# jaggedsoft/mythril

Measured on AMD Instinct MI355X. Metric: constraint-node evals/sec, higher is better.
Workload: dtype u32x8 (256-bit bit-vectors)

## Files before the change

### include/mythcc.h

```cpp
#ifndef MYTHCC_H
#define MYTHCC_H

#include <stdint.h>

#ifdef __cplusplus
extern "C" {
#endif

#define MGC_OK 0
#define MGC_UNSUPPORTED 1
#define MGC_ERROR 2

#define MGC_MAX_SOURCE_WIDTH 65536

#define MGC_SORT_BV 0
#define MGC_SORT_BOOL 1
#define MGC_SORT_ARRAY 2

#define MGC_REMAT_SPILL 0
#define MGC_REMAT_SCRATCH 1
#define MGC_REMAT_ALWAYS 2

typedef struct mgc_input {
    int32_t n_nodes;
    const int32_t* op;
    const int32_t* sort;
    const int32_t* width;
    const int32_t* dom;
    const int64_t* id;
    const int32_t* arg_off;
    const int32_t* args;
    const int64_t* p0;
    const int64_t* p1;
    const int32_t* str;
    const int32_t* cval_off;
    const uint32_t* cval;
    const char* strings;
    int32_t n_strings;
    int32_t n_cons;
    const int32_t* cons;
    int32_t n_probes;
    const int32_t* probes;
    int32_t n_tables;
    const int32_t* table_name;
    const int32_t* table_size;
    int32_t default_entries;
    int32_t nreg;
    int32_t n_extra;
    const uint32_t* extra;
    int32_t leaf_pools;
    int32_t const_keys;
    int32_t solve;
    int32_t remat_mode;
    int32_t remat_k;
    int32_t keep_clean;
    int32_t search_hints;
    int32_t abi_presets;
    int32_t n_cval;
    int32_t n_string_bytes;
} mgc_input;

typedef struct mgc_result mgc_result;

const char* mgc_source_ops(void);

int mgc_compile(const mgc_input* in, mgc_result** out);

const char* mgc_error(const mgc_result* r);
const uint32_t* mgc_code(const mgc_result* r, int32_t* n_ins);
const uint32_t* mgc_table(const mgc_result* r, int32_t* n_rows, int32_t* n_const_values);
const char* mgc_meta(const mgc_result* r);
void mgc_free(mgc_result* r);

#ifdef __cplusplus
}
#endif

#endif
```

### mythril_amd/ccompile.py

```python

from __future__ import annotations

import collections.abc as _abc
import ctypes
import json
import os
import threading
from array import array
from typing import Dict, List, Optional, Sequence

import numpy as np

from . import irdefs as I
from .smt.node import ARRAY, BOOL, topo_order

_lib = None
_lock = threading.Lock()
_OPS: Dict[str, int] = {}
_OTHER = 0

MGC_OK, MGC_UNSUPPORTED = 0, 1
_SORT = {"bv": 0, BOOL: 1, ARRAY: 2}
_REMAT = {"spill": 0, "always": 2}


class _Input(ctypes.Structure):
    _fields_ = [("n_nodes", ctypes.c_int32)] + \
        [(n, ctypes.c_void_p) for n in ("op", "sort", "width", "dom", "id", "arg_off", "args", "p0",
                                         "p1", "str", "cval_off", "cval")] + \
        [("strings", ctypes.c_char_p), ("n_strings", ctypes.c_int32),
         ("n_cons", ctypes.c_int32), ("cons", ctypes.c_void_p),
         ("n_probes", ctypes.c_int32), ("probes", ctypes.c_void_p),
         ("n_tables", ctypes.c_int32), ("table_name", ctypes.c_void_p),
         ("table_size", ctypes.c_void_p),
         ("default_entries", ctypes.c_int32), ("nreg", ctypes.c_int32),
         ("n_extra", ctypes.c_int32), ("extra", ctypes.c_void_p),
         ("leaf_pools", ctypes.c_int32), ("const_keys", ctypes.c_int32), ("solve", ctypes.c_int32),
         ("remat_mode", ctypes.c_int32), ("remat_k", ctypes.c_int32),
         ("keep_clean", ctypes.c_int32), ("search_hints", ctypes.c_int32),
         ("abi_presets", ctypes.c_int32), ("n_cval", ctypes.c_int32),
         ("n_string_bytes", ctypes.c_int32)]


def load():
    global _lib, _OTHER
    if _lib is not None:
        return _lib
    with _lock:
        if _lib is not None:
            return _lib
        from .build import build_compiler
        path = build_compiler()
        lib = ctypes.CDLL(path)
        lib.mgc_source_ops.restype = ctypes.c_char_p
        lib.mgc_compile.argtypes = [ctypes.POINTER(_Input), ctypes.POINTER(ctypes.c_void_p)]
        lib.mgc_compile.restype = ctypes.c_int
        lib.mgc_error.argtypes = [ctypes.c_void_p]
        lib.mgc_error.restype = ctypes.c_char_p
        lib.mgc_code.argtypes = [ctypes.c_void_p, ctypes.POINTER(ctypes.c_int32)]
        lib.mgc_code.restype = ctypes.c_void_p
        lib.mgc_table.argtypes = [ctypes.c_void_p, ctypes.POINTER(ctypes.c_int32),
                                  ctypes.POINTER(ctypes.c_int32)]
        lib.mgc_table.restype = ctypes.c_void_p
        lib.mgc_meta.argtypes = [ctypes.c_void_p]
        lib.mgc_meta.restype = ctypes.c_char_p
        lib.mgc_free.argtypes = [ctypes.c_void_p]
        names = lib.mgc_source_ops().decode().split("\n")
        _OPS.update({n: i for i, n in enumerate(names)})
        _OTHER = _OPS["?"]
        _lib = lib
    return _lib


def _ptr(a):
    return ctypes.addressof(ctypes.c_char.from_buffer(a)) if len(a) else None


_ext = None


def _load_ext():
    global _ext
    if _ext is None:
        import importlib.util
        from .build import cc_ext_path
        load()
        spec = importlib.util.spec_from_file_location("_mythcc", cc_ext_path())
        mod = importlib.util.module_from_spec(spec)
        spec.loader.exec_module(mod)
        _ext = mod
    return _ext


def compile_native(constraints: Sequence, probes: Sequence = (),
                   table_sizes: Optional[Dict[str, int]] = None, default_entries: int = 2,
                   nreg: int = I.NREG, extra_consts: Sequence[int] = (), leaf_pools: bool = False,
                   const_keys: bool = False, solve: bool = False, leaf_remat: Optional[str] = None,
                   keep_clean: Optional[bool] = None, search_hints: bool = False,
                   abi_presets: bool = False):
    from . import ir
    ext = _load_ext()
    M = (1 << 256) - 1
    extra = b"".join((v & M).to_bytes(32, "little") for v in extra_consts)
    remat = leaf_remat or ir.LEAF_REMAT
    mode = _REMAT.get(remat, 1)
    k = int(remat[7:]) if mode == 1 and remat[7:].isdigit() else 0
    rc, err, code_b, raw, ncv, meta = ext.compile(
        list(constraints), list(probes), _OPS, list((table_sizes or {}).items()), default_entries,
        nreg, extra, int(leaf_pools), int(const_keys), int(solve), mode, k,
        int(ir.KEEP_CLEAN if keep_clean is None else keep_clean), int(search_hints),
        int(abi_presets))
    if rc != MGC_OK:
        if rc == MGC_UNSUPPORTED:
            raise ir.Unsupported(err)
        raise RuntimeError("native compiler: " + err)
    prog = _program(np.frombuffer(code_b, dtype=np.uint32).reshape(-1, 4).copy(), raw, ncv,
                    json.loads(meta))
    prog.nreg = nreg
    return prog


def buckets(constraints: Sequence):
    return _load_ext().buckets(list(constraints))


def flatten(constraints: Sequence, probes: Sequence = (),
            table_sizes: Optional[Dict[str, int]] = None, extra_consts: Sequence[int] = ()):
    load()
    constraints, probes = list(constraints), list(probes)
    nodes = topo_order(constraints + probes)
    index = {n.id: i for i, n in enumerate(nodes)}
    ops, OTHER = _OPS, _OTHER
    f = {k: array("i") for k in ("op", "sort", "width", "dom", "str", "cval_off", "args")}
    f.update({k: array("q") for k in ("id", "p0", "p1")})
    f["arg_off"] = array("i", [0])
    cval = bytearray()
    strings: List[str] = []
    sidx: Dict[str, int] = {}

    def intern(s: str) -> int:
        k = sidx.get(s)
        if k is None:
            k = sidx[s] = len(strings)
            strings.append(s)
        return k
    for n in nodes:
        op = n.op
        code = ops.get(op, OTHER)
        f["op"].append(code)
        f["sort"].append(_SORT[n.sort])
        f["width"].append(n.width)
        f["dom"].append(n.dom or 0)
        f["id"].append(n.id)
        for a in n.args:
            f["args"].append(index[a.id])
        f["arg_off"].append(len(f["args"]))
        p0 = p1 = 0
        s = -1
        c = -1
        pr = n.params
        if op == "bvnum":
            c = len(cval) // 4
            cval += pr[0].to_bytes(4 * ((n.width + 31) // 32), "little")
        elif op in ("var", "array"):
            s = intern(pr[0])
        elif op == "apply":
            s = intern(pr[0])
            p0 = pr[1]
        elif op == "extract":
            p0, p1 = pr
        elif op in ("zero_extend", "sign_extend"):
            p0 = pr[0]
        elif code == OTHER:
            s = intern(op)
        f["p0"].append(p0)
        f["p1"].append(p1)
        f["str"].append(s)
        f["cval_off"].append(c)
    f["cons"] = array("i", [index[c.id] for c in constraints])
    f["probes"] = array("i", [index[p.id] for p in probes])
    tsz = table_sizes or {}
    f["table_name"] = array("i", [intern(k) for k in tsz])
    f["table_size"] = array("i", list(tsz.values()))
    M = (1 << 256) - 1
    f["extra"] = bytearray(b"".join((v & M).to_bytes(32, "little") for v in extra_consts))
    f["cval"] = bytearray(cval)
    f["strings"] = b"".join(s.encode() + b"\0" for s in strings)
    f["n_nodes"], f["n_strings"] = len(nodes), len(strings)
    return f


def compile_native_ctypes(constraints: Sequence, probes: Sequence = (),
                          table_sizes: Optional[Dict[str, int]] = None, default_entries: int = 2,
                          nreg: int = I.NREG, extra_consts: Sequence[int] = (),
                          leaf_pools: bool = False, const_keys: bool = False, solve: bool = False,
                          leaf_remat: Optional[str] = None, keep_clean: Optional[bool] = None,
                          search_hints: bool = False, abi_presets: bool = False):
    from . import ir
    lib = load()
    f = flatten(constraints, probes, table_sizes, extra_consts)
    remat = leaf_remat or ir.LEAF_REMAT
    mode = _REMAT.get(remat, 1)
    k = int(remat[7:]) if mode == 1 and remat[7:].isdigit() else 0
    P = {n: _ptr(f[n]) for n in ("op", "sort", "width", "dom", "id", "arg_off", "args", "p0", "p1",
                                  "str", "cval_off", "cval", "cons", "probes", "table_name",
                                  "table_size", "extra")}
    inp = _Input(f["n_nodes"], P["op"], P["sort"], P["width"], P["dom"], P["id"], P["arg_off"],
                 P["args"], P["p0"], P["p1"], P["str"], P["cval_off"], P["cval"], f["strings"],
                 f["n_strings"], len(f["cons"]), P["cons"], len(f["probes"]), P["probes"],
                 len(f["table_name"]), P["table_name"], P["table_size"], default_entries, nreg,
                 len(f["extra"]) // 32, P["extra"], int(leaf_pools), int(const_keys), int(solve),
                 mode, k, int(ir.KEEP_CLEAN if keep_clean is None else keep_clean),
                 int(search_hints), int(abi_presets), len(f["cval"]) // 4, len(f["strings"]))
    res = ctypes.c_void_p()
    rc = lib.mgc_compile(ctypes.byref(inp), ctypes.byref(res))
    try:
        if rc != MGC_OK:
            msg = lib.mgc_error(res).decode()
            if rc == MGC_UNSUPPORTED:
                raise ir.Unsupported(msg)
            raise RuntimeError("native compiler: " + msg)
        n = ctypes.c_int32()
        p = lib.mgc_code(res, ctypes.byref(n))
        code = np.frombuffer(ctypes.string_at(p, 16 * n.value), dtype=np.uint32).reshape(-1, 4).copy()
        rows, ncv = ctypes.c_int32(), ctypes.c_int32()
        p = lib.mgc_table(res, ctypes.byref(rows), ctypes.byref(ncv))
        raw = ctypes.string_at(p, 32 * rows.value) if rows.value else b""
        meta = json.loads(lib.mgc_meta(res))
    finally:
        lib.mgc_free(res)
    prog = _program(code, raw, ncv.value, meta)
    prog.nreg = nreg
    return prog


class LeafRecords(_abc.Sequence):

    __slots__ = ("_rs", "_items", "widths")

    def __init__(self, rs: str, widths: Sequence[int]):
        self._rs = rs
        self._items = None
        self.widths = list(widths)

    def _decode(self):
        from .ir import Leaf
        items = []
        if self.widths:
            for line in self._rs.split("\n"):
                name, w, kind, source, chunk, entry = line.split("\t")
                items.append(Leaf(name, int(w), kind, source, int(chunk), int(entry)))
        self._items = items
        self._rs = None
        return items

    def __len__(self):
        return len(self.widths)

    def __getitem__(self, i):
        return (self._items if self._items is not None else self._decode())[i]

    def __iter__(self):
        return iter(self._items if self._items is not None else self._decode())

    def __eq__(self, other):
        return list(self) == list(other)

    def __repr__(self):
        return repr(list(self))

    def __reduce__(self):
        return (list, (list(self),))


def _program(code, raw: bytes, ncv: int, meta):
    from . import ir
    consts = np.frombuffer(raw, dtype="<u4").reshape(-1, 8).astype(np.uint32)
    const_values = [int.from_bytes(raw[32 * i:32 * i + 32], "little") for i in range(ncv)]
    Leaf = ir.Leaf
    if meta.get("leaves_rs") is not None:
        leaves = LeafRecords(meta["leaves_rs"], meta["leaf_widths"])
    else:
        leaves = [Leaf(*row) for row in meta["leaves"]]
    hist_counts = dict(meta["hist"])
    stats = {"lnodes": meta["lnodes"], "n_ins": int(code.shape[0]), "spills": meta["spills"],
             "reloads": meta["reloads"],
             "hist": {I.OPNAME[op]: hist_counts[op] for op in meta["hist_order"]}}
    prog = ir.Program(code, consts, const_values, leaves, meta["n_lds"], meta["n_probes"],
                      meta["n_roots"], dict(meta["table_sizes"]), dict(meta["table_kinds"]),
                      {k: [int(h, 16) for h in v] for k, v in meta["table_ckeys"]}, stats,
                      [tuple(r) for r in meta["pool_ranges"]], dict(meta["derived"]),
                      {k: v for k, v in meta["entry_keys"]}, meta["n_user_probes"])
    prog.compile_us = meta.get("t_us")
    pre = meta.get("presets")
    if pre is not None:
        from .abi import Plan
        prog.presets = Plan(vars={k: int(v, 16) for k, v in pre["vars"]},
                            arrays={k: dict(cells) for k, cells in pre["arrays"]})
    return prog
```

### mythril_amd/csrc/mg_compile.cpp

```cpp

#include "mythcc.h"
#include "mythgpu_ir.h"

#include <algorithm>
#include <memory>
#include <cstdint>
#include <cstdio>
#include <cstring>
#include <chrono>
#include <stdexcept>
#include <string>
#include <unordered_map>
#include <unordered_set>
#include <tuple>
#include <utility>
#include <vector>

namespace {

struct U {
    static const int N = 6;
    uint64_t w[N];
    U() { std::memset(w, 0, sizeof w); }
    static U of(uint64_t x) { U r; r.w[0] = x; return r; }
    bool zero() const {
        for (int i = 0; i < N; i++) if (w[i]) return false;
        return true;
    }
    bool neg() const { return w[N - 1] >> 63; }
    int bitlen() const {
        for (int i = N - 1; i >= 0; i--)
            if (w[i]) return 64 * i + 64 - __builtin_clzll(w[i]);
        return 0;
    }
    int popcount() const {
        int c = 0;
        for (int i = 0; i < N; i++) c += __builtin_popcountll(w[i]);
        return c;
    }
    bool bit(int k) const { return k < 64 * N && ((w[k >> 6] >> (k & 63)) & 1); }
};

static U operator+(const U& a, const U& b) {
    U r; unsigned __int128 c = 0;
    for (int i = 0; i < U::N; i++) { c += (unsigned __int128)a.w[i] + b.w[i]; r.w[i] = (uint64_t)c; c >>= 64; }
    return r;
}
static U operator~(const U& a) { U r; for (int i = 0; i < U::N; i++) r.w[i] = ~a.w[i]; return r; }
static U operator-(const U& a, const U& b) { return a + ~b + U::of(1); }
static U operator&(const U& a, const U& b) { U r; for (int i = 0; i < U::N; i++) r.w[i] = a.w[i] & b.w[i]; return r; }
static U operator|(const U& a, const U& b) { U r; for (int i = 0; i < U::N; i++) r.w[i] = a.w[i] | b.w[i]; return r; }
static U operator^(const U& a, const U& b) { U r; for (int i = 0; i < U::N; i++) r.w[i] = a.w[i] ^ b.w[i]; return r; }
static U operator*(const U& a, const U& b) {
    U r;
    for (int i = 0; i < U::N; i++) {
        unsigned __int128 c = 0;
        for (int j = 0; i + j < U::N; j++) {
            c += (unsigned __int128)a.w[i] * b.w[j] + r.w[i + j];
            r.w[i + j] = (uint64_t)c; c >>= 64;
        }
    }
    return r;
}
struct BadShift : std::runtime_error { BadShift() : std::runtime_error("negative shift") {} };
static U shl(const U& a, int k) {
    if (k < 0) throw BadShift();
    U r; if (k >= 64 * U::N) return r;
    int q = k >> 6, s = k & 63;
    for (int i = U::N - 1; i >= q; i--) {
        uint64_t v = a.w[i - q] << s;
        if (s && i - q - 1 >= 0) v |= a.w[i - q - 1] >> (64 - s);
        r.w[i] = v;
    }
    return r;
}
static U shr(const U& a, int k) {
    if (k < 0) throw BadShift();
    U r; if (k >= 64 * U::N) return r;
    int q = k >> 6, s = k & 63;
    for (int i = 0; i + q < U::N; i++) {
        uint64_t v = a.w[i + q] >> s;
        if (s && i + q + 1 < U::N) v |= a.w[i + q + 1] << (64 - s);
        r.w[i] = v;
    }
    return r;
}
static U sar(const U& a, int k) {
    if (!a.neg()) return shr(a, k);
    return ~shr(~a, k);
}
static bool operator==(const U& a, const U& b) { return std::memcmp(a.w, b.w, sizeof a.w) == 0; }
static bool operator!=(const U& a, const U& b) { return !(a == b); }
static bool operator<(const U& a, const U& b) {
    for (int i = U::N - 1; i >= 0; i--) if (a.w[i] != b.w[i]) return a.w[i] < b.w[i];
    return false;
}
static bool operator>(const U& a, const U& b) { return b < a; }
static bool operator<=(const U& a, const U& b) { return !(b < a); }
static bool operator>=(const U& a, const U& b) { return !(a < b); }
static U umin(const U& a, const U& b) { return b < a ? b : a; }
static U umax(const U& a, const U& b) { return a < b ? b : a; }
static U mask_slow(int w) { return shl(U::of(1), w) - U::of(1); }
static const U* mask_table() {
    static const std::vector<U> t = [] {
        std::vector<U> v(64 * U::N + 1);
        for (int w = 0; w <= 64 * U::N; w++) v[w] = mask_slow(w);
        return v;
    }();
    return t.data();
}
static const U* const MASKS = mask_table();
static inline const U& mask(int w) { return MASKS[w < 0 ? 0 : (w > 64 * U::N ? 64 * U::N : w)]; }
static U U1(int k) { return shl(U::of(1), k); }
static bool nz(const U& a) { return !a.zero(); }

static std::string hex(const U& a) {
    char buf[8];
    std::string s;
    bool started = false;
    for (int i = U::N - 1; i >= 0; i--) {
        for (int nib = 15; nib >= 0; nib--) {
            int d = (a.w[i] >> (4 * nib)) & 15;
            if (!started && !d) continue;
            started = true;
            std::snprintf(buf, sizeof buf, "%x", d);
            s += buf;
        }
    }
    return started ? s : "0";
}

struct Big {
    std::vector<uint32_t> l;
    void norm() { while (!l.empty() && !l.back()) l.pop_back(); }
    bool operator==(const Big& o) const { return l == o.l; }
    bool operator<(const Big& o) const {
        if (l.size() != o.l.size()) return l.size() < o.l.size();
        for (size_t i = l.size(); i-- > 0;) if (l[i] != o.l[i]) return l[i] < o.l[i];
        return false;
    }
    U chunk(int k) const {
        U r;
        for (int j = 0; j < 8; j++) {
            size_t idx = (size_t)8 * k + j;
            if (idx < l.size()) r.w[j / 2] |= (uint64_t)l[idx] << (32 * (j & 1));
        }
        return r;
    }
    U low384() const {
        U r;
        for (size_t j = 0; j < l.size() && j < 12; j++) r.w[j / 2] |= (uint64_t)l[j] << (32 * (j & 1));
        return r;
    }
    std::string hexs() const {
        if (l.empty()) return "0";
        char buf[16];
        std::string s;
        std::snprintf(buf, sizeof buf, "%x", l.back());
        s += buf;
        for (size_t i = l.size() - 1; i-- > 0;) { std::snprintf(buf, sizeof buf, "%08x", l[i]); s += buf; }
        return s;
    }
};

static Big big_of(const U& u) {
    Big b;
    for (int j = 0; j < 2 * U::N; j++) b.l.push_back((uint32_t)(u.w[j / 2] >> (32 * (j & 1))));
    b.norm();
    return b;
}

struct Bits {
    std::vector<uint64_t> w;
    void set(int k) { if ((size_t)(k >> 6) >= w.size()) w.resize((k >> 6) + 1, 0); w[k >> 6] |= 1ull << (k & 63); }
    void orw(const Bits& o) { if (o.w.size() > w.size()) w.resize(o.w.size(), 0); for (size_t i = 0; i < o.w.size(); i++) w[i] |= o.w[i]; }
    bool meets(const Bits& o) const {
        size_t n = std::min(w.size(), o.w.size());
        for (size_t i = 0; i < n; i++) if (w[i] & o.w[i]) return true;
        return false;
    }
    bool any() const { for (auto x : w) if (x) return true; return false; }
    int count() const { int c = 0; for (auto x : w) c += __builtin_popcountll(x); return c; }
    template <class F> void each(F f) const {
        for (size_t i = 0; i < w.size(); i++) {
            uint64_t x = w[i];
            while (x) { int b = __builtin_ctzll(x); f((int)(64 * i + b)); x &= x - 1; }
        }
    }
    bool any_minus(const Bits& o) const {
        for (size_t i = 0; i < w.size(); i++) if (w[i] & ~(i < o.w.size() ? o.w[i] : 0)) return true;
        return false;
    }
    Bits minus(const Bits& o) const {
        Bits r; r.w = w;
        for (size_t i = 0; i < r.w.size() && i < o.w.size(); i++) r.w[i] &= ~o.w[i];
        return r;
    }
};

struct Unsupported : std::runtime_error { using std::runtime_error::runtime_error; };
struct MemoMiss {};

template <class K, class V, class H = std::hash<K>>
struct OMap {
    std::vector<std::pair<K, V>> items;
    std::unordered_map<K, size_t, H> idx;
    V* find(const K& k) { auto it = idx.find(k); return it == idx.end() ? nullptr : &items[it->second].second; }
    const V* find(const K& k) const { auto it = idx.find(k); return it == idx.end() ? nullptr : &items[it->second].second; }
    bool has(const K& k) const { return idx.count(k) != 0; }
    V& setdefault(const K& k, const V& d) {
        auto it = idx.find(k);
        if (it != idx.end()) return items[it->second].second;
        idx.emplace(k, items.size());
        items.emplace_back(k, d);
        return items.back().second;
    }
    void put(const K& k, const V& v) { setdefault(k, v) = v; }
    size_t size() const { return items.size(); }
    void truncate(size_t n) {
        while (items.size() > n) { idx.erase(items.back().first); items.pop_back(); }
    }
};

enum SOp {
    S_BVNUM, S_TRUE, S_FALSE, S_VAR, S_BVSUB, S_BVUDIV, S_BVUREM, S_BVSDIV, S_BVSREM, S_BVSMOD,
    S_BVSHL, S_BVLSHR, S_BVASHR, S_BVADD, S_BVMUL, S_BVAND, S_BVOR, S_BVXOR, S_AND, S_OR,
    S_BVNEG, S_BVNOT, S_NOT, S_XOR, S_IMPLIES, S_BVULT, S_BVULE, S_BVUGT, S_BVUGE, S_BVSLT,
    S_BVSLE, S_BVSGT, S_BVSGE, S_UMULNO, S_EQ, S_DISTINCT, S_ITE, S_CONCAT, S_EXTRACT, S_ZEXT,
    S_SEXT, S_SELECT, S_APPLY, S_STORE, S_K, S_ARRAY, S_OTHER
};
static const char* const SOP_NAMES =
    "bvnum\ntrue\nfalse\nvar\nbvsub\nbvudiv\nbvurem\nbvsdiv\nbvsrem\nbvsmod\n"
    "bvshl\nbvlshr\nbvashr\nbvadd\nbvmul\nbvand\nbvor\nbvxor\nand\nor\n"
    "bvneg\nbvnot\nnot\nxor\n=>\nbvult\nbvule\nbvugt\nbvuge\nbvslt\n"
    "bvsle\nbvsgt\nbvsge\nbvumul_noovfl\n=\ndistinct\nite\nconcat\nextract\nzero_extend\n"
    "sign_extend\nselect\napply\nstore\nK\narray\n?";

struct Src {
    int op, sort, width, dom;
    int64_t id;
    std::vector<int> args;
    int64_t p0, p1;
    std::string str;
    Big val;
    bool is_array() const { return sort == MGC_SORT_ARRAY; }
    bool is_bool() const { return sort == MGC_SORT_BOOL; }
};

static const int CHUNK = 256;
static const int MAX_SPILL = MG_MAX_LDS + MG_MAX_PSLOTS;
static const int LDS_TIER = 6;
static const int POOL_CAP = 128;
static const int ARG_ENTRIES_CAP = 64;

static std::vector<int> topo(const std::vector<Src>& S, const std::vector<int>& roots) {
    std::vector<char> seen(S.size(), 0);
    std::vector<int> out;
    std::vector<std::pair<int, bool>> stack;
    for (int r : roots) {
        if (seen[r]) continue;
        stack.assign(1, {r, false});
        while (!stack.empty()) {
            auto [n, done] = stack.back();
            stack.pop_back();
            if (done) { out.push_back(n); continue; }
            if (seen[n]) continue;
            seen[n] = 1;
            stack.push_back({n, true});
            const auto& a = S[n].args;
            for (size_t i = a.size(); i-- > 0;)
                if (!seen[a[i]]) stack.push_back({a[i], false});
        }
    }
    return out;
}

struct Args {
    int n = 0;
    int a[3] = {0, 0, 0};
    std::vector<int> more;
    Args() {}
    Args(std::initializer_list<int> il) { assign(il.begin(), il.end()); }
    Args(const std::vector<int>& v) { assign(v.data(), v.data() + v.size()); }
    template <class It> void assign(It b, It e) {
        n = (int)(e - b);
        if (n <= 3) { std::copy(b, e, a); more.clear(); }
        else more.assign(b, e);
    }
    const int* begin() const { return n <= 3 ? a : more.data(); }
    const int* end() const { return begin() + n; }
    int* begin() { return n <= 3 ? a : more.data(); }
    int* end() { return begin() + n; }
    size_t size() const { return (size_t)n; }
    bool empty() const { return n == 0; }
    int operator[](size_t i) const { return begin()[i]; }
    int& operator[](size_t i) { return begin()[i]; }
    int back() const { return begin()[n - 1]; }
    bool operator==(const Args& o) const { return n == o.n && std::equal(begin(), end(), o.begin()); }
    bool operator!=(const Args& o) const { return !(*this == o); }
};

struct LN {
    int op, width;
    Args args;
    bool has_imm;
    U imm;
    int64_t birth;
};

enum LeafKind { K_VAR, K_KEY, K_VAL, K_ELSE, K_CVAL, K_AUX };
static const char* KIND_NAMES[] = {"var", "key", "val", "else", "cval", "aux"};

struct Leaf {
    std::string name;
    int width;
    int kind;
    std::string source;
    int chunk, entry;
};

static bool is_pred(int op) {
    return op == MG_EQ || op == MG_ULT || op == MG_ULE || op == MG_SLT || op == MG_SLE || op == MG_UMULNO;
}
static bool is_cmp(int op) {
    return op == MG_EQ || op == MG_ULT || op == MG_ULE || op == MG_SLT || op == MG_SLE;
}
static bool is_order(int op) { return op == MG_ULT || op == MG_ULE || op == MG_SLT || op == MG_SLE; }

typedef std::vector<int> Chunks;


struct Lowerer {
    const std::vector<Src>& S;
    std::vector<LN> ln;
    std::vector<int> slot_id;
    std::vector<uint64_t> slot_hash;
    size_t n_slots_used = 0;
    std::vector<Leaf> leaves;
    std::unordered_map<std::string, int> leaf_ids;
    std::vector<Chunks> memo;
    std::vector<char> has_memo;
    std::unordered_map<std::string, Chunks> sel_memo;
    OMap<std::string, int> table_sizes;
    OMap<std::string, std::string> table_kinds;
    int default_entries;
    int64_t birth = 0;
    OMap<std::string, std::vector<Big>> table_ckeys;
    bool solve = false;
    std::unordered_set<std::string> solve_tables;
    OMap<std::string, std::vector<std::pair<Chunks, Chunks>>> arg_entries;

    Lowerer(const std::vector<Src>& s, int de) : S(s), default_entries(de) {
        memo.resize(S.size());
        has_memo.assign(S.size(), 0);
    }

    static uint64_t key_hash(int op, int width, const Args& args, bool has_imm, const U& imm) {
        uint64_t h = (uint64_t)op * 0x9E3779B97F4A7C15ull ^ (uint64_t)width * 0xC2B2AE3D27D4EB4Full;
        for (int a : args) h = (h ^ (uint64_t)(uint32_t)a) * 0x100000001B3ull;
        if (has_imm) for (int i = 0; i < U::N; i++) h = (h ^ imm.w[i]) * 0x100000001B3ull;
        h ^= h >> 29;
        return h | 1;
    }
    void rehash(size_t n) {
        std::vector<int> ids(n, -1);
        std::vector<uint64_t> hs(n, 0);
        for (size_t i = 0; i < slot_id.size(); i++) {
            if (slot_id[i] < 0) continue;
            size_t j = slot_hash[i] & (n - 1);
            while (ids[j] >= 0) j = (j + 1) & (n - 1);
            ids[j] = slot_id[i];
            hs[j] = slot_hash[i];
        }
        slot_id.swap(ids);
        slot_hash.swap(hs);
    }
    int mk(int op, int width, Args args, bool has_imm = false, const U& imm = U()) {
        if (op == MG_CONCAT && width == MG_MAX_WIDTH && ln[args[0]].op == MG_EXTRACT &&
            ln[args[0]].imm.zero() && ln[ln[args[0]].args[0]].width == MG_MAX_WIDTH)
            args[0] = ln[args[0]].args[0];
        const U key_imm = has_imm ? imm : U();
        if (2 * (n_slots_used + 1) > slot_id.size()) rehash(slot_id.empty() ? 4096 : 2 * slot_id.size());
        uint64_t h = key_hash(op, width, args, has_imm, key_imm);
        size_t j = h & (slot_id.size() - 1);
        while (slot_id[j] >= 0) {
            if (slot_hash[j] == h) {
                const LN& o = ln[slot_id[j]];
                if (o.op == op && o.width == width && o.has_imm == has_imm && o.args == args &&
                    (!has_imm || o.imm == key_imm))
                    return slot_id[j];
            }
            j = (j + 1) & (slot_id.size() - 1);
        }
        int64_t b = birth;
        for (int a : args) if (ln[a].birth > b) b = ln[a].birth;
        int id = (int)ln.size();
        ln.push_back(LN{op, width, std::move(args), has_imm, key_imm, b});
        slot_id[j] = id;
        slot_hash[j] = h;
        n_slots_used++;
        return id;
    }
    int mki(int op, int width, Args args, int64_t imm) { return mk(op, width, std::move(args), true, U::of((uint64_t)imm)); }
    int cnst(const U& value, int width) { return mk(MG_CONST, width, {}, true, value & mask(width)); }
    int cnst(uint64_t value, int width) { return cnst(U::of(value), width); }
    int leaf(const std::string& name, int width, int kind, const std::string& source, int chunk = 0, int entry = 0) {
        auto it = leaf_ids.find(name);
        int idx;
        if (it == leaf_ids.end()) {
            idx = (int)leaves.size();
            leaf_ids.emplace(name, idx);
            leaves.push_back(Leaf{name, width, kind, source, chunk, entry});
        } else {
            idx = it->second;
        }
        return mki(MG_LEAF, width, {}, idx);
    }

    static int nchunks(int w) { return (w + CHUNK - 1) / CHUNK; }
    static int chunk_width(int w, int i) { return std::min(CHUNK, w - CHUNK * i); }

    int bits(const Chunks& chunks, int w, int lo, int hi) {
        int ci = lo / CHUNK, cj = hi / CHUNK;
        if (ci == cj) {
            int c = chunks.at(ci);
            int cw = chunk_width(w, ci);
            int l0 = lo - CHUNK * ci, h0 = hi - CHUNK * ci;
            if (l0 == 0 && h0 == cw - 1) return c;
            return mki(MG_EXTRACT, h0 - l0 + 1, {c}, l0);
        }
        int low_w = CHUNK * (ci + 1) - lo;
        int low = bits(chunks, w, lo, CHUNK * (ci + 1) - 1);
        int high = bits(chunks, w, CHUNK * cj, hi);
        return mki(MG_CONCAT, hi - lo + 1, {high, low}, low_w);
    }

    Chunks assemble(const std::vector<std::pair<Chunks, int>>& pieces) {
        int total = 0;
        for (auto& p : pieces) total += p.second;
        struct Seg { const Chunks* ch; int w, off; };
        std::vector<Seg> segs;
        int off = 0;
        for (size_t i = pieces.size(); i-- > 0;) {
            segs.push_back({&pieces[i].first, pieces[i].second, off});
            off += pieces[i].second;
        }
        Chunks out;
        for (int k = 0; k < nchunks(total); k++) {
            int lo_k = CHUNK * k, hi_k = std::min(total, CHUNK * (k + 1)) - 1;
            int acc = -1, acc_w = 0;
            for (auto& s : segs) {
                int a = std::max(lo_k, s.off), b = std::min(hi_k, s.off + s.w - 1);
                if (a > b) continue;
                int part = bits(*s.ch, s.w, a - s.off, b - s.off);
                int pw = b - a + 1;
                if (acc < 0) { acc = part; acc_w = pw; }
                else { acc = mki(MG_CONCAT, acc_w + pw, {part, acc}, acc_w); acc_w += pw; }
            }
            out.push_back(acc);
        }
        return out;
    }

    const Chunks& M(int s) {
        if (!has_memo[s]) throw MemoMiss();
        return memo[s];
    }

    std::vector<char> pend_seen_;
    std::vector<int> pending(int n) {
        if (pend_seen_.size() < S.size()) pend_seen_.assign(S.size(), 0);
        std::vector<int> out, touched;
        std::vector<std::pair<int, bool>> stack{{n, false}};
        while (!stack.empty()) {
            auto [m, done] = stack.back();
            stack.pop_back();
            if (done) { out.push_back(m); continue; }
            if (pend_seen_[m] || has_memo[m]) continue;
            pend_seen_[m] = 1;
            touched.push_back(m);
            stack.push_back({m, true});
            const auto& a = S[m].args;
            for (size_t i = a.size(); i-- > 0;)
                if (!pend_seen_[a[i]] && !has_memo[a[i]]) stack.push_back({a[i], false});
        }
        for (int m : touched) pend_seen_[m] = 0;
        return out;
    }

    const Chunks& lower(int n) {
        if (has_memo[n]) return memo[n];
        std::vector<int> nodes = pending(n);
        std::unordered_set<int> skip;
        for (int m : nodes)
            if (S[m].op == S_EXTRACT && is_carry(m)) {
                int s = S[m].args[0];
                skip.insert(s); skip.insert(S[s].args[0]); skip.insert(S[s].args[1]);
            }
        int64_t saved = birth;
        for (int m : nodes) {
            if (has_memo[m] || S[m].is_array() || (skip.count(m) && m != n)) continue;
            birth = S[m].id;
            try {
                Chunks r = lower_one(m);
                memo[m] = std::move(r);
                has_memo[m] = 1;
            } catch (MemoMiss&) {
                throw Unsupported("operand lowered only as part of a pattern");
            }
            birth = S[m].id;
        }
        birth = saved ? std::max(saved, birth) : birth;
        if (!has_memo[n]) throw Unsupported("operand lowered only as part of a pattern");
        return memo[n];
    }

    int narrow(int s) {
        const Chunks& ch = M(s);
        if (ch.size() != 1)
            throw Unsupported(opname(s) + " on a " + std::to_string(S[s].width) + "-bit value");
        return ch[0];
    }

    std::string opname(int s) {
        static const std::vector<std::string> names = [] {
            std::vector<std::string> v;
            std::string all(SOP_NAMES);
            size_t p = 0;
            while (true) {
                size_t q = all.find('\n', p);
                v.push_back(all.substr(p, q == std::string::npos ? std::string::npos : q - p));
                if (q == std::string::npos) break;
                p = q + 1;
            }
            return v;
        }();
        return S[s].op == S_OTHER ? S[s].str : names[S[s].op];
    }

    int fold(int op, int width, const Chunks& args) {
        int acc = args[0];
        for (size_t i = 1; i < args.size(); i++) acc = mk(op, width, {acc, args[i]});
        return acc;
    }

    int by_constant(int op, int w, int n) {
        const Src& s = S[n];
        if (S[s.args[1]].op != S_BVNUM) return -1;
        const Big& cb = S[s.args[1]].val;
        int x = narrow(s.args[0]);
        bool huge = cb.l.size() > 2;
        uint64_t c = 0;
        for (size_t j = 0; j < cb.l.size() && j < 2; j++) c |= (uint64_t)cb.l[j] << (32 * j);
        if (op == S_BVUDIV || op == S_BVUREM) {
            bool pow2;
            int k = 0;
            if (huge) {
                int ones = 0, top = 0;
                for (size_t j = 0; j < cb.l.size(); j++) {
                    ones += __builtin_popcount(cb.l[j]);
                    if (cb.l[j]) top = (int)(32 * j + 31 - __builtin_clz(cb.l[j]));
                }
                pow2 = ones == 1;
                k = top;
            } else {
                pow2 = c && !(c & (c - 1));
                if (pow2) k = 63 - __builtin_clzll(c);
            }
            if (!pow2) return -1;
            if (op == S_BVUREM) return k == 0 ? cnst(0, w) : mki(MG_EXTRACT, k, {x}, 0);
            op = S_BVLSHR; c = (uint64_t)k; huge = false;
        }
        if (op != S_BVSHL && op != S_BVLSHR && op != S_BVASHR) return -1;
        if (!huge && c == 0) return x;
        bool ge = huge || c >= (uint64_t)w;
        if (op == S_BVASHR) {
            int cc = ge ? w - 1 : (int)std::min<uint64_t>(c, (uint64_t)(w - 1));
            int e = mki(MG_EXTRACT, w - cc, {x}, cc);
            return mki(MG_SEXT, w, {e}, w - cc);
        }
        if (ge) return cnst(0, w);
        int cc = (int)c;
        if (op == S_BVLSHR) return mki(MG_EXTRACT, w - cc, {x}, cc);
        int e = mki(MG_EXTRACT, w - cc, {x}, 0);
        int z = cnst(0, cc);
        return mki(MG_CONCAT, w, {e, z}, cc);
    }

    Chunks lower_one(int n) {
        const Src& s = S[n];
        int op = s.op, w = s.width;
        if (w > CHUNK) return lower_wide(n);
        auto A = [&](int i) { return narrow(s.args[i]); };
        switch (op) {
        case S_BVNUM: return {cnst(s.val.chunk(0), w)};
        case S_TRUE: return {cnst(1, 1)};
        case S_FALSE: return {cnst(0, 1)};
        case S_VAR: return {leaf(s.str, w, K_VAR, s.str)};
        default: break;
        }
        int simple = -1;
        switch (op) {
        case S_BVSUB: simple = MG_SUB; break;
        case S_BVUDIV: simple = MG_UDIV; break;
        case S_BVUREM: simple = MG_UREM; break;
        case S_BVSDIV: simple = MG_SDIV; break;
        case S_BVSREM: simple = MG_SREM; break;
        case S_BVSMOD: simple = MG_SMOD; break;
        case S_BVSHL: simple = MG_SHL; break;
        case S_BVLSHR: simple = MG_LSHR; break;
        case S_BVASHR: simple = MG_ASHR; break;
        default: break;
        }
        if (simple >= 0) {
            int red = by_constant(op, w, n);
            if (red >= 0) return {red};
            int a = A(0), b = A(1);
            return {mk(simple, w, {a, b})};
        }
        int nary = -1;
        switch (op) {
        case S_BVADD: nary = MG_ADD; break;
        case S_BVMUL: nary = MG_MUL; break;
        case S_BVAND: case S_AND: nary = MG_AND; break;
        case S_BVOR: case S_OR: nary = MG_OR; break;
        case S_BVXOR: nary = MG_XOR; break;
        default: break;
        }
        if (nary >= 0) {
            Chunks xs;
            for (size_t i = 0; i < s.args.size(); i++) xs.push_back(A((int)i));
            return {fold(nary, w, xs)};
        }
        if (op == S_BVNEG) return {mk(MG_NEG, w, {A(0)})};
        if (op == S_BVNOT || op == S_NOT) return {mk(MG_NOT, w, {A(0)})};
        if (op == S_XOR) { int a = A(0), b = A(1); return {mk(MG_XOR, 1, {a, b})}; }
        if (op == S_IMPLIES) {
            int a = A(0);
            int na = mk(MG_NOT, 1, {a});
            int b = A(1);
            return {mk(MG_OR, 1, {na, b})};
        }
        int kop = -1; bool swap = false;
        switch (op) {
        case S_BVULT: kop = MG_ULT; break;
        case S_BVULE: kop = MG_ULE; break;
        case S_BVUGT: kop = MG_ULT; swap = true; break;
        case S_BVUGE: kop = MG_ULE; swap = true; break;
        case S_BVSLT: kop = MG_SLT; break;
        case S_BVSLE: kop = MG_SLE; break;
        case S_BVSGT: kop = MG_SLT; swap = true; break;
        case S_BVSGE: kop = MG_SLE; swap = true; break;
        case S_UMULNO: kop = MG_UMULNO; break;
        default: break;
        }
        if (kop >= 0) {
            int a = A(0), b = A(1);
            if (swap) std::swap(a, b);
            return {mk(kop, S[s.args[0]].width, {a, b})};
        }
        if (op == S_EQ || op == S_DISTINCT) {
            for (int a : s.args) if (S[a].is_array()) throw Unsupported("array equality");
            return {eq_or_distinct(op, n)};
        }
        if (op == S_ITE) {
            if (s.is_array()) throw Unsupported("array-valued ite outside select");
            int c = A(0), a = A(1), b = A(2);
            return {mk(MG_ITE, w, {c, a, b})};
        }
        if (op == S_CONCAT) {
            int word = calldata_word(n);
            if (word >= 0) return {word};
            std::vector<std::pair<Chunks, int>> pieces;
            for (int a : s.args) pieces.push_back({M(a), S[a].width});
            return assemble(pieces);
        }
        if (op == S_EXTRACT) {
            int carry = carry_pattern(n);
            if (carry >= 0) return {carry};
            int src = s.args[0];
// ... 14 lines not shown

    int eq_parts(const Chunks& x, const Chunks& y, int w) {
        Chunks parts;
        for (size_t k = 0; k < x.size(); k++)
            parts.push_back(mk(MG_EQ, w > CHUNK ? chunk_width(w, (int)k) : w, {x[k], y.at(k)}));
        return fold(MG_AND, 1, parts);
    }

    int eq_or_distinct(int op, int n) {
        const Src& s = S[n];
        std::vector<const Chunks*> args;
        for (int a : s.args) args.push_back(&M(a));
        int w = S[s.args[0]].width;
        if (op == S_EQ) return eq_parts(*args[0], *args[1], w);
        Chunks terms;
        for (size_t i = 0; i < args.size(); i++)
            for (size_t j = i + 1; j < args.size(); j++) {
                int e = eq_parts(*args[i], *args[j], w);
                terms.push_back(mk(MG_NOT, 1, {e}));
            }
        return fold(MG_AND, 1, terms);
    }

    bool is_carry(int n) const {
        const Src& x = S[n];
        int64_t hi = x.p0, lo = x.p1;
        const Src& s = S[x.args[0]];
        if (hi != lo || s.op != S_BVADD || s.args.size() != 2 || hi != s.width - 1) return false;
        const Src& a = S[s.args[0]];
        const Src& b = S[s.args[1]];
        return a.op == S_ZEXT && b.op == S_ZEXT && a.p0 == 1 && b.p0 == 1 &&
               S[a.args[0]].width <= CHUNK;
    }

    int carry_pattern(int n) {
        if (!is_carry(n)) return -1;
        const Src& s = S[S[n].args[0]];
        int x = S[s.args[0]].args[0], y = S[s.args[1]].args[0];
        int lx = lower(x)[0];
        int ly = lower(y)[0];
        int sum = mk(MG_ADD, S[x].width, {lx, ly});
        return mk(MG_ULT, S[x].width, {sum, lx});
    }

    Chunks lower_wide(int n) {
        const Src& s = S[n];
        int op = s.op, w = s.width;
        if (op == S_BVNUM) {
            Chunks out;
            for (int k = 0; k < nchunks(w); k++) out.push_back(cnst(s.val.chunk(k), chunk_width(w, k)));
            return out;
        }
        if (op == S_VAR) {
            Chunks out;
            for (int k = 0; k < nchunks(w); k++)
                out.push_back(leaf(s.str + "#" + std::to_string(k), chunk_width(w, k), K_VAR, s.str, k));
            return out;
        }
        if (op == S_CONCAT) {
            std::vector<std::pair<Chunks, int>> pieces;
            for (int a : s.args) pieces.push_back({M(a), S[a].width});
            return assemble(pieces);
        }
        if (op == S_EXTRACT) {
            int src = s.args[0];
            int hi = (int)s.p0, lo = (int)s.p1;
            const Chunks& sc = M(src);
            std::vector<std::pair<Chunks, int>> pieces;
            for (int k = nchunks(w) - 1; k >= 0; k--) {
                int b = bits(sc, S[src].width, lo + CHUNK * k, std::min(hi, lo + CHUNK * k + CHUNK - 1));
                pieces.push_back({{b}, std::min(CHUNK, hi - lo + 1 - CHUNK * k)});
            }
            return assemble(pieces);
        }
        if (op == S_ZEXT) {
            int src = s.args[0];
            int pad = w - S[src].width;
            std::vector<std::pair<Chunks, int>> pieces;
            while (pad > 0) {
                int pw = std::min(CHUNK, pad);
                pieces.push_back({{cnst(0, pw)}, pw});
                pad -= pw;
            }
            pieces.push_back({M(src), S[src].width});
            return assemble(pieces);
        }
        if (op == S_ITE) {
            int c = narrow(s.args[0]);
            Chunks a = M(s.args[1]), b = M(s.args[2]);
            return ite_chunks(c, a, b);
        }
        if (op == S_SELECT) {
            Chunks idx = M(s.args[1]);
            return select(s.args[0], idx, S[s.args[1]].width, w);
        }
        if (op == S_APPLY) {
            Chunks key = M(s.args[0]);
            return table_lookup(s.str, key, (int)s.p0, w, "func");
        }
        throw Unsupported(opname(n) + " on a " + std::to_string(w) + "-bit value");
    }

    void index_parts(int x, int& base, U& c) const {
        c = U();
        while (true) {
            const Src& s = S[x];
            if (s.op == S_BVNUM) { base = -1; c = (c + s.val.chunk(0)) & mask(256); return; }
            if (s.op != S_BVADD || s.args.size() != 2) { base = x; return; }
            int a = s.args[0], b = s.args[1];
            if (S[b].op == S_BVNUM && S[a].op != S_BVNUM) { c = (c + S[b].val.chunk(0)) & mask(256); x = a; }
            else if (S[a].op == S_BVNUM && S[b].op != S_BVNUM) { c = (c + S[a].val.chunk(0)) & mask(256); x = b; }
            else { base = x; return; }
        }
    }

    int calldata_word(int n) {
        const Src& s = S[n];
        if (s.width != 256 || s.args.size() != 32) return -1;
        int size = -1, arr = -1, base = -1, off = -1;
        U c0;
        for (int i = 0; i < 32; i++) {
            const Src& x = S[s.args[i]];
            if (x.op != S_ITE || x.width != 8) return -1;
            const Src& cond = S[x.args[0]];
            const Src& sel = S[x.args[1]];
            const Src& zero = S[x.args[2]];
            if (zero.op != S_BVNUM || !zero.val.l.empty() || cond.op != S_BVSLT || sel.op != S_SELECT)
                return -1;
            int idx = sel.args[1];
            if (cond.args[0] != idx || S[idx].width != 256) return -1;
            if (i == 0) {
                size = cond.args[1];
                arr = sel.args[0];
                if (S[arr].op != S_ARRAY) return -1;
                index_parts(idx, base, c0);
                off = idx;
            } else if (cond.args[1] != size || sel.args[0] != arr) {
                return -1;
            } else {
                int b;
                U c;
                index_parts(idx, b, c);
                if (b != base || !(c == ((c0 + U::of((uint64_t)i)) & mask(256)))) return -1;
            }
        }
        const std::string& name = S[arr].str;
        const std::vector<Big>* ck = table_ckeys.find(name);
        if ((ck && !ck->empty()) || (solve && solve_tables.count(name))) return -1;
        table_kinds.put(name, "array");
        int entries = table_sizes.setdefault(name, default_entries);
        int o = narrow(off), sz = narrow(size);
        int acc = mk(MG_BCAST, 256, {cell(name, K_ELSE, 0, 8)[0]});
        for (int e = entries - 1; e >= 0; e--) {
            int key = cell(name, K_KEY, e, 256)[0];
            int delta = mk(MG_SUB, 256, {key, o});
            int val = cell(name, K_VAL, e, 8)[0];
            acc = mk(MG_CDWE, 256, {acc, delta, val});
        }
        return mk(MG_CDWX, 256, {acc, o, sz});
    }

    int chunk_eq(const Chunks& x, const Chunks& y, int w) {
        Chunks parts;
        for (size_t k = 0; k < x.size(); k++) parts.push_back(mk(MG_EQ, chunk_width(w, (int)k), {x[k], y.at(k)}));
        return fold(MG_AND, 1, parts);
    }

    Chunks ite_chunks(int c, const Chunks& a, const Chunks& b) {
        Chunks out;
        for (size_t i = 0; i < a.size() && i < b.size(); i++)
            out.push_back(mk(MG_ITE, std::max(ln[a[i]].width, ln[b[i]].width), {c, a[i], b[i]}));
        return out;
    }

    Chunks cell(const std::string& name, int kind, int e, int width) {
        std::string tag;
        switch (kind) {
        case K_KEY: tag = "k" + std::to_string(e); break;
        case K_VAL: tag = "v" + std::to_string(e); break;
        case K_ELSE: tag = "else"; break;
        default: tag = "c" + std::to_string(e); break;
        }
        Chunks out;
        for (int k = 0; k < nchunks(width); k++)
            out.push_back(leaf(name + "#" + tag + "#" + std::to_string(k), chunk_width(width, k), kind, name, k, e));
        return out;
    }

    Chunks const_key(const Big& v, int kw) {
        Chunks c;
        for (int k = 0; k < nchunks(kw); k++) c.push_back(cnst(v.chunk(k), chunk_width(kw, k)));
        return c;
    }

    Chunks table_lookup(const std::string& name, const Chunks& key, int kw, int vw, const char* kind) {
        table_kinds.put(name, kind);
        std::string mkey = "T" + name;
        mkey.push_back('\0');
        mkey.append((const char*)key.data(), 4 * key.size());
        auto hit = sel_memo.find(mkey);
        if (hit != sel_memo.end()) return hit->second;
        int entries = table_sizes.setdefault(name, default_entries);
        static const std::vector<Big> none;
        const std::vector<Big>* ckp = table_ckeys.find(name);
        const std::vector<Big>& ckeys = ckp ? *ckp : none;
        bool has_kval = true;
        for (int k : key) if (ln[k].op != MG_CONST) { has_kval = false; break; }
        Big kval;
        if (has_kval) {
            for (size_t i = 0; i < key.size(); i++) {
                Big part = big_of(ln[key[i]].imm);
                if (kval.l.size() < 8 * i + part.l.size()) kval.l.resize(8 * i + part.l.size(), 0);
                for (size_t j = 0; j < part.l.size(); j++) kval.l[8 * i + j] |= part.l[j];
            }
            kval.norm();
        }
        int kidx = -1;
        if (has_kval)
            for (size_t i = 0; i < ckeys.size(); i++) if (ckeys[i] == kval) { kidx = (int)i; break; }
        Chunks acc;
        if (kidx >= 0) {
            acc = cell(name, K_CVAL, kidx, vw);
        } else if (solve && solve_tables.count(name)) {
            auto& ents = arg_entries.setdefault(name, {});
            Chunks val = cell(name, K_VAL, (int)ents.size(), vw);
            acc = val;
            for (size_t i = ents.size(); i-- > 0;) {
                int e = chunk_eq(key, ents[i].first, kw);
                acc = ite_chunks(e, ents[i].second, acc);
            }
            ents.push_back({key, val});
            table_sizes.put(name, (int)ents.size());
            if (!has_kval)
                for (size_t i = ckeys.size(); i-- > 0;) {
                    Chunks c = const_key(ckeys[i], kw);
                    int e = chunk_eq(key, c, kw);
                    Chunks cv = cell(name, K_CVAL, (int)i, vw);
                    acc = ite_chunks(e, cv, acc);
                }
        } else {
            acc = cell(name, K_ELSE, 0, vw);
            for (int e = entries - 1; e >= 0; e--) {
                Chunks kc = cell(name, K_KEY, e, kw);
                int q = chunk_eq(key, kc, kw);
                Chunks vc = cell(name, K_VAL, e, vw);
                acc = ite_chunks(q, vc, acc);
            }
            if (!has_kval)
                for (size_t i = ckeys.size(); i-- > 0;) {
                    Chunks c = const_key(ckeys[i], kw);
                    int q = chunk_eq(key, c, kw);
                    Chunks cv = cell(name, K_CVAL, (int)i, vw);
                    acc = ite_chunks(q, cv, acc);
                }
        }
        sel_memo[mkey] = acc;
        return acc;
    }

    Chunks select(int arr, const Chunks& idx, int iw, int vw) {
        std::string mkey = "A" + std::to_string(arr);
        mkey.push_back('\0');
        mkey.append((const char*)idx.data(), 4 * idx.size());
        auto hit = sel_memo.find(mkey);
        if (hit != sel_memo.end()) return hit->second;
        std::vector<int> chain;
        int a = arr;
        while (S[a].op == S_STORE) { chain.push_back(a); a = S[a].args[0]; }
        Chunks base;
        if (S[a].op == S_K) {
            base = lower(S[a].args[0]);
        } else if (S[a].op == S_ARRAY) {
            base = table_lookup(S[a].str, idx, iw, vw, "array");
        } else if (S[a].op == S_ITE) {
            int c = narrow_node(S[a].args[0]);
            Chunks x = select(S[a].args[1], idx, iw, vw);
            Chunks y = select(S[a].args[2], idx, iw, vw);
            base = ite_chunks(c, x, y);
        } else {
            throw Unsupported("array term " + opname(a));
        }
        Chunks acc = base;
        for (size_t i = chain.size(); i-- > 0;) {
            int st = chain[i];
            Chunks j = lower(S[st].args[1]);
            Chunks v = lower(S[st].args[2]);
            int e = chunk_eq(idx, j, iw);
            acc = ite_chunks(e, v, acc);
        }
        sel_memo[mkey] = acc;
        return acc;
    }

    int narrow_node(int n) {
        const Chunks& ch = lower(n);
        if (ch.size() != 1) throw Unsupported("wide condition");
        return ch[0];
    }
};

static const int PASSES = 6;
static const int MAX_REFUSALS = 4;
static const int SCHEDULE_MIN_SCRATCH = 10;
static const int MAX_DOMAIN = 16;
static const int MAX_BRANCHES = 4;
static const int MAX_OR = 64;
static const int BRANCH_DEPTH = 2;
static const int SELECTOR_WIDTH = 8;

struct OverlayTable {
    std::vector<int> val, gen;
    int next_gen = 0;
};
struct Memo {
    std::vector<int> dense;
    const Memo* parent = nullptr;
    OverlayTable* ov = nullptr;
    int gen = 0;
    int get(int k) const {
        if (!parent) return (size_t)k < dense.size() ? dense[k] : -1;
        if ((size_t)k < ov->gen.size() && ov->gen[k] == gen) return ov->val[k];
        return parent->get(k);
    }
    void put(int k, int v) {
        if (parent) {
            if ((size_t)k >= ov->gen.size()) {
                size_t sz = std::max<size_t>(k + 1, 2 * ov->gen.size());
                ov->gen.resize(sz, 0);
                ov->val.resize(sz, -1);
            }
            ov->gen[k] = gen;
            ov->val[k] = v;
            return;
        }
        if ((size_t)k >= dense.size()) dense.resize(std::max<size_t>(k + 1, 2 * dense.size()), -1);
        dense[k] = v;
    }
    void overlay_on(const Memo* p, OverlayTable* t) {
        parent = p;
        ov = t;
        gen = ++t->next_gen;
    }
};

struct Interval { U lo, hi; };
struct Bound { int e; U lo, hi; int w; };

struct Solver {
    Lowerer& lw;
    std::vector<LN>& ln;
    OMap<int, int> repl;
    std::vector<int> repl_of_;
    const int* repl_find(int x) const {
        return (size_t)x < repl_of_.size() && repl_of_[x] >= 0 ? &repl_of_[x] : nullptr;
    }
    void repl_put(int k, int v) {
        repl.put(k, v);
        if ((size_t)k >= repl_of_.size()) repl_of_.resize(std::max<size_t>(k + 1, 2 * repl_of_.size()), -1);
        repl_of_[k] = v;
    }
    void repl_truncate(size_t n) {
        for (size_t i = n; i < repl.items.size(); i++) repl_of_[repl.items[i].first] = -1;
        repl.truncate(n);
    }
    int one, zero;
    int n_aux = 0, n_branch = 0;
    std::unordered_set<int> selectors, or_seen;
    std::vector<char> clean_;
    bool is_clean(int x) const { return (size_t)x < clean_.size() && clean_[x]; }
    void set_clean(int x) { if ((size_t)x >= clean_.size()) clean_.resize(std::max<size_t>(x + 1, 2 * clean_.size()), 0); clean_[x] = 1; }
    std::vector<int> stamp_;
    int stamp_gen_ = 0;
    int new_stamp() { return ++stamp_gen_; }
    bool stamped(int x, int g) { if ((size_t)x >= stamp_.size()) stamp_.resize(std::max<size_t>(x + 1, 2 * stamp_.size()), 0); if (stamp_[x] == g) return true; stamp_[x] = g; return false; }
    int dep_w = 0;
    std::vector<uint64_t> dep;
    std::vector<char> has_dep;
    struct DepRow {
        const uint64_t* p;
        int w;
        bool meets(const Bits& o) const {
            int n = std::min(w, (int)o.w.size());
            for (int i = 0; i < n; i++) if (p[i] & o.w[i]) return true;
            return false;
        }
        template <class F> void each(F f) const {
            for (int i = 0; i < w; i++) {
                uint64_t x = p[i];
                while (x) { int b = __builtin_ctzll(x); f(64 * i + b); x &= x - 1; }
            }
        }
    };
    std::vector<Interval> ivl_;
    std::vector<char> has_ivl_;
    std::unordered_set<std::string> joint_done;
    std::unordered_map<int, int> leaf_imm, leaf_node;
    bool dm_valid = false;
    Bits dm;
    Memo base_memo;
    Memo* run_memo = &base_memo;
    std::unordered_map<int, int> depth;
    bool unsat = false;
    bool dead = false;
    std::unordered_map<int, int> aux_seq;
    std::unordered_set<int> refused;
    bool wrap_ctx = false;
    std::unordered_set<int> wrap_defs;

    std::vector<std::pair<int, bool>> rw_stack_;

    explicit Solver(Lowerer& l) : lw(l), ln(l.ln) {
        one = lw.cnst(1, 1);
        zero = lw.cnst(0, 1);
    }

    const LN& N(int i) const { return ln[i]; }

    Interval interval(int n) {
        if ((size_t)n < has_ivl_.size() && has_ivl_[n]) return ivl_[n];
        U top = mask(ln[n].width);
        Interval r;
        int op = ln[n].op;
        if (op == MG_CONST) {
            r = {ln[n].imm, ln[n].imm};
        } else if (op == MG_ADD) {
            Interval a = interval(ln[n].args[0]), b = interval(ln[n].args[1]);
            U hs = a.hi + b.hi;
            r = hs <= top ? Interval{a.lo + b.lo, hs} : Interval{U(), top};
        } else if (op == MG_ITE) {
            Interval a = interval(ln[n].args[1]), b = interval(ln[n].args[2]);
            r = {umin(a.lo, b.lo), umax(a.hi, b.hi)};
        } else if (is_pred(op)) {
            r = {U(), U::of(1)};
        } else {
            r = {U(), top};
        }
        if ((size_t)n >= has_ivl_.size()) { size_t sz = std::max<size_t>(n + 1, 2 * has_ivl_.size()); has_ivl_.resize(sz, 0); ivl_.resize(sz); }
        ivl_[n] = r;
        has_ivl_[n] = 1;
        return r;
    }

    int cmp_fold(int op, int w, int a, int b) {
        Interval A = interval(a), B = interval(b);
        if (op == MG_SLT || op == MG_SLE) {
            U half = U1(w - 1);
            if (A.hi >= half || B.hi >= half) return -1;
        }
        if (op == MG_ULT || op == MG_SLT) {
            if (A.hi < B.lo) return one;
            if (A.lo >= B.hi) return zero;
        } else {
            if (A.hi <= B.lo) return one;
            if (A.lo > B.hi) return zero;
        }
        return -1;
    }

    bool const_fold(int x, const Args& args, U& out) {
        int w = ln[x].width, op = ln[x].op;
        U m = mask(w);
        auto v = [&](int i) { return ln[args[i]].imm; };
        switch (op) {
        case MG_CONCAT: out = (shl(v(0), (int)ln[x].imm.w[0]) | v(1)) & m; return true;
        case MG_EXTRACT: out = shr(v(0), (int)ln[x].imm.w[0]) & m; return true;
        case MG_AND: out = v(0) & v(1) & m; return true;
        case MG_OR: out = (v(0) | v(1)) & m; return true;
        case MG_XOR: out = (v(0) ^ v(1)) & m; return true;
        case MG_SUB: out = (v(0) - v(1)) & m; return true;
        case MG_MUL: out = (v(0) * v(1)) & m; return true;
        case MG_NOT: out = ~v(0) & m; return true;
        default: return false;
        }
    }

    bool all_const(const Args& args) const {
        for (int a : args) if (ln[a].op != MG_CONST) return false;
        return true;
    }

    int fold(int x, const Args& args) {
        int op = ln[x].op;
        if ((op == MG_CONCAT || op == MG_EXTRACT || op == MG_AND || op == MG_OR || op == MG_XOR ||
             op == MG_SUB || op == MG_MUL || op == MG_NOT) && all_const(args)) {
            U c;
            if (const_fold(x, args, c)) return lw.cnst(c, ln[x].width);
        }
        if (is_order(op) && !all_const(args)) {
            int r = cmp_fold(op, ln[x].width, args[0], args[1]);
            if (r >= 0) return r;
        }
        if (op == MG_EQ) {
            int a = args[0], b = args[1];
            if (a == b) return one;
            if (ln[a].op == MG_CONST && ln[b].op == MG_CONST) return ln[a].imm == ln[b].imm ? one : zero;
            int ya = a, yb = b;
            U ca, cb;
            if (ln[a].op == MG_ADD && ln[ln[a].args[1]].op == MG_CONST) { ya = ln[a].args[0]; ca = ln[ln[a].args[1]].imm; }
            if (ln[b].op == MG_ADD && ln[ln[b].args[1]].op == MG_CONST) { yb = ln[b].args[0]; cb = ln[ln[b].args[1]].imm; }
            if (ya == yb && ln[a].width == ln[b].width && ln[ya].op != MG_CONST) return ca == cb ? one : zero;
            Interval A = interval(a), B = interval(b);
            if (A.hi < B.lo || B.hi < A.lo) return zero;
        } else if (op == MG_ADD) {
            int a = args[0], b = args[1];
            if (ln[a].op == MG_CONST && ln[b].op != MG_CONST) std::swap(a, b);
            if (ln[b].op == MG_CONST) {
                int w = ln[x].width;
                if (ln[a].op == MG_CONST) return lw.cnst((ln[a].imm + ln[b].imm) & mask(w), w);
                if (ln[b].imm.zero() && ln[a].width <= w) return a;
                if (ln[a].op == MG_ADD && ln[a].width == w && ln[ln[a].args[1]].op == MG_CONST) {
                    int y = ln[a].args[0];
                    int c = lw.cnst((ln[ln[a].args[1]].imm + ln[b].imm) & mask(w), w);
                    return lw.mk(MG_ADD, w, {y, c});
                }
                if (!(a == args[0] && b == args[1])) return lw.mk(MG_ADD, w, {a, b});
            }
        } else if (is_order(op) && all_const(args)) {
            U a = ln[args[0]].imm, b = ln[args[1]].imm;
            if (op == MG_SLT || op == MG_SLE) {
                U half = U1(ln[x].width - 1);
                a = a ^ half; b = b ^ half;
            }
            bool r = (op == MG_ULT || op == MG_SLT) ? a < b : a <= b;
            return r ? one : zero;
        } else if (op == MG_ITE) {
            int c = args[0];
            if (ln[c].op == MG_CONST) return (ln[c].imm.w[0] & 1) ? args[1] : args[2];
            if (args[1] == args[2]) return args[1];
        } else if ((op == MG_AND || op == MG_OR) && ln[x].width == 1) {
            uint64_t absorb = op == MG_AND ? 0 : 1;
            Chunks rest;
            for (int a : args) {
                if (ln[a].op == MG_CONST) {
                    if ((ln[a].imm.w[0] & 1) == absorb) return ln[a].width == 1 ? a : lw.cnst(absorb, 1);
                    continue;
                }
                rest.push_back(a);
            }
            if (rest.empty()) return lw.cnst(1 - absorb, 1);
            if (rest.size() == 1) return rest[0];
            if (rest[0] == rest[1]) return rest[0];
        } else if (op == MG_NOT && ln[x].width == 1) {
            int a = args[0];
            if (ln[a].op == MG_CONST) return lw.cnst(1 - (ln[a].imm.w[0] & 1), 1);
            if (ln[a].op == MG_NOT && ln[a].width == 1) return ln[a].args[0];
        }
        bool same = true;
        for (size_t i = 0; i < args.size(); i++) if (args[i] != ln[x].args[i]) { same = false; break; }
        if (same) return x;
        return lw.mk(op, ln[x].width, args, ln[x].has_imm, ln[x].imm);
    }

    void dep_layout(size_t rows, int w) {
        if (w != dep_w) {
            std::vector<uint64_t> d(rows * (size_t)w, 0);
            for (size_t r = 0; r < has_dep.size(); r++)
                if (has_dep[r]) std::copy(dep.begin() + r * dep_w, dep.begin() + r * dep_w + dep_w, d.begin() + r * w);
            dep.swap(d);
            dep_w = w;
        } else {
            dep.resize(rows * (size_t)w, 0);
        }
        has_dep.resize(rows, 0);
    }

    DepRow depof(int n) {
        if ((size_t)n < has_dep.size() && has_dep[n]) return DepRow{dep.data() + (size_t)n * dep_w, dep_w};
        int need_w = (int)(lw.leaves.size() + 63) / 64 + 1;
        if (has_dep.size() < ln.size() || need_w > dep_w)
            dep_layout(std::max(ln.size(), 2 * has_dep.size()), std::max(dep_w, need_w));
        dep_stack_.clear();
        dep_stack_.push_back(n);
        while (!dep_stack_.empty()) {
            int x = dep_stack_.back();
            if (has_dep[x]) { dep_stack_.pop_back(); continue; }
            bool pend = false;
            for (int a : ln[x].args) if (!has_dep[a]) { dep_stack_.push_back(a); pend = true; }
            if (pend) continue;
            dep_stack_.pop_back();
            uint64_t* row = dep.data() + (size_t)x * dep_w;
            if (ln[x].op == MG_LEAF) {
                int li = (int)ln[x].imm.w[0];
                row[li >> 6] |= 1ull << (li & 63);
            } else {
                for (int a : ln[x].args) {
                    const uint64_t* src = dep.data() + (size_t)a * dep_w;
                    for (int i = 0; i < dep_w; i++) row[i] |= src[i];
                }
            }
            has_dep[x] = 1;
        }
        return DepRow{dep.data() + (size_t)n * dep_w, dep_w};
    }
    std::vector<int> dep_stack_;

    const Bits& defmask() {
        if (!dm_valid) {
            dm = Bits();
            for (auto& kv : repl.items) dm.set(leaf_imm[kv.first]);
            dm_valid = true;
        }
        return dm;
    }

    int rewrite(int n, Memo& memo) {
        const Bits& dmask = defmask();
// ... 1312 lines not shown
                if (S[x].op == S_STORE) stack.push_back(S[x].args[0]);
                else if (S[x].op == S_ITE) { stack.push_back(S[x].args[1]); stack.push_back(S[x].args[2]); }
                else if (S[x].op == S_ARRAY) note(S[x].str, S[n].args[1]);
            }
        } else if (S[n].op == S_APPLY) {
            note(S[n].str, S[n].args[0]);
        }
    }
    OMap<std::string, std::vector<Big>> ck;
    for (auto& kv : out.items) {
        const auto* s = sym.find(kv.first);
        size_t ns = s ? s->size() : 0;
        if (!kv.second.empty() && (long long)ns * (long long)kv.second.size() <= max_links) {
            std::vector<Big> v = kv.second;
            std::sort(v.begin(), v.end());
            ck.put(kv.first, v);
        }
    }
    for (auto& kv : sym.items) sym_counts[kv.first] = (int)kv.second.size();
    return ck;
}

static void harvest_hints(const std::vector<Src>& S, const std::vector<int>& order, std::vector<U>& out) {
    U M256 = mask(256), low6 = ~U::of(63);
    for (int n : order) {
        if (S[n].op != S_BVNUM || S[n].width < 8) continue;
        U v = S[n].val.chunk(0);
        out.push_back((v + U::of(63)) & M256 & low6);
        const Big& b = S[n].val;
        if (!b.l.empty() && b.l.size() == 1) out.push_back(shl(U::of(b.l[0]), 224));
    }
}

struct Presets {
    std::vector<std::pair<std::string, U>> vars;
    std::vector<std::pair<std::string, std::vector<std::pair<int64_t, int>>>> arrays;
    std::vector<std::pair<int, U>> subst;
};

static bool split_add(const std::vector<Src>& S, int k, int& base, U& c) {
    base = -1;
    c = U();
    std::vector<int> stack{k};
    while (!stack.empty()) {
        int x = stack.back();
        stack.pop_back();
        if (S[x].op == S_BVNUM) c = c + S[x].val.low384();
        else if (S[x].op == S_BVADD) for (int a : S[x].args) stack.push_back(a);
        else if (base < 0) base = x;
        else return false;
    }
    if (base < 0) return false;
    c = c & mask(S[k].width);
    return true;
}

static bool byte_cell(const std::vector<Src>& S, int x, int arr, int64_t& off, int& size) {
    size = -1;
    if (S[x].op == S_ITE && S[S[x].args[2]].op == S_BVNUM && S[S[x].args[2]].val.l.empty()) {
        int c = S[x].args[0];
        if (S[c].op != S_BVSLT || S[S[c].args[0]].op != S_BVNUM || S[S[c].args[1]].op != S_VAR) return false;
        size = S[c].args[1];
        x = S[x].args[1];
    }
    if (S[x].op == S_SELECT && S[x].args[0] == arr && S[S[x].args[1]].op == S_BVNUM) {
        const Big& v = S[S[x].args[1]].val;
        if (v.l.size() > 2) return false;
        off = (int64_t)(v.l.empty() ? 0 : v.l[0]) | (v.l.size() > 1 ? (int64_t)v.l[1] << 32 : 0);
        return true;
    }
    return false;
}

static bool word_of(const std::vector<Src>& S, int base, int arr, int64_t& first, int& size) {
    std::vector<int> parts, stack{base};
    while (!stack.empty()) {
        int x = stack.back();
        stack.pop_back();
        if (S[x].op == S_CONCAT) for (size_t i = S[x].args.size(); i-- > 0;) stack.push_back(S[x].args[i]);
        else parts.push_back(x);
    }
    if (parts.size() != 32) return false;
    size = -1;
    std::vector<int64_t> offs;
    for (int p : parts) {
        int64_t o;
        int s;
        if (!byte_cell(S, p, arr, o, s) || (s >= 0 && size >= 0 && s != size)) return false;
        if (s >= 0) size = s;
        offs.push_back(o);
    }
    for (size_t i = 0; i < offs.size(); i++) if (offs[i] != offs[0] + (int64_t)i) return false;
    first = offs[0];
    return true;
}

static bool abi_plan(const std::vector<Src>& S, const std::vector<int>& nodes, Presets& out) {
    struct Arr { int arr; std::vector<Big> consts; std::vector<int> sym; };
    OMap<int, Arr> by_arr;
    for (int n : nodes) {
        if (S[n].op != S_SELECT || S[S[n].args[0]].op != S_ARRAY) continue;
        int arr = S[n].args[0], k = S[n].args[1];
        Arr& d = by_arr.setdefault(arr, Arr{arr, {}, {}});
        if (S[k].op == S_BVNUM) {
            if (std::find(d.consts.begin(), d.consts.end(), S[k].val) == d.consts.end()) d.consts.push_back(S[k].val);
        } else {
            d.sym.push_back(k);
        }
    }
    for (auto& kv : by_arr.items) {
        const Arr& d = kv.second;
        if (d.sym.empty() || d.consts.empty()) continue;
        struct Base { int base; U lo, hi; int64_t off; std::vector<std::pair<int, U>> keys; int size; };
        OMap<int, Base> bases;
        bool ok = true;
        for (int k : d.sym) {
            int base;
            U c;
            if (!split_add(S, k, base, c) || nz(shr(c, 32))) { ok = false; break; }
            Base* r = bases.find(base);
            if (!r) {
                int64_t off = 0;
                int size = -1;
                if (!word_of(S, base, d.arr, off, size)) { ok = false; break; }
                r = &bases.setdefault(base, Base{base, c, c, off, {}, size});
            }
            r->lo = umin(r->lo, c);
            r->hi = umax(r->hi, c);
            r->keys.push_back({k, c});
        }
        if (!ok) continue;
        int size_var = -1;
        U nxt = std::max_element(d.consts.begin(), d.consts.end())->low384() + U::of(1);
        std::vector<std::pair<int64_t, int>> cells;
        auto set_cell = [&](int64_t o, int b) {
            for (auto& c : cells) if (c.first == o) { c.second = b; return; }
            cells.push_back({o, b});
        };
        for (auto& bv : bases.items) {
            const Base& b = bv.second;
            U val = shl(sar(nxt - b.lo + U::of(31), 5), 5);
            for (int i = 0; i < 32; i++) set_cell(b.off + i, (int)(sar(val, 8 * (31 - i)).w[0] & 0xFF));
            for (auto& kc : b.keys) out.subst.push_back({kc.first, (val + kc.second) & mask(S[kc.first].width)});
            nxt = val + b.hi + U::of(1);
            if (size_var < 0) size_var = b.size;
        }
        if (size_var >= 0) {
            out.vars.push_back({S[size_var].str, nxt});
            out.subst.push_back({size_var, nxt & mask(S[size_var].width)});
        }
        out.arrays.push_back({S[d.arr].str, cells});
        for (int n : nodes) {
            if (S[n].op != S_SELECT || S[n].args[0] != d.arr || S[S[n].args[1]].op != S_BVNUM) continue;
            const Big& v = S[S[n].args[1]].val;
            if (v.l.size() > 2) continue;
            int64_t o = (int64_t)(v.l.empty() ? 0 : v.l[0]) | (v.l.size() > 1 ? (int64_t)v.l[1] << 32 : 0);
            for (auto& c : cells)
                if (c.first == o) { out.subst.push_back({n, U::of((uint64_t)c.second) & mask(S[n].width)}); break; }
        }
    }
    return !out.arrays.empty();
}

static void jstr(std::string& o, const std::string& s) {
    o.push_back('"');
    for (unsigned char ch : s) {
        if (ch == '"' || ch == '\\') { o.push_back('\\'); o.push_back((char)ch); }
        else if (ch == '\n') o += "\\n";
        else if (ch == '\t') o += "\\t";
        else if (ch < 0x20) { char b[8]; std::snprintf(b, sizeof b, "\\u%04x", ch); o += b; }
        else o.push_back((char)ch);
    }
    o.push_back('"');
}

}

struct mgc_result {
    std::string error;
    std::vector<uint32_t> code;
    std::vector<uint32_t> table;
    int32_t n_rows = 0, n_const_values = 0;
    std::string meta;
};

namespace {

static double now_us() {
    return std::chrono::duration<double, std::micro>(
        std::chrono::steady_clock::now().time_since_epoch()).count();
}

static void compile(const mgc_input* in, mgc_result* res) {
    double tp[9];
    tp[0] = now_us();
    auto bad = [](const char* what) { throw std::runtime_error(what); };
    if (in->n_nodes < 0 || in->n_cons < 0 || in->n_probes < 0 || in->n_strings < 0 ||
        in->n_tables < 0 || in->n_extra < 0 || in->n_cval < 0 || in->n_string_bytes < 0)
        bad("negative count");
    if (in->n_nodes && (!in->op || !in->sort || !in->width || !in->dom || !in->id || !in->arg_off ||
                        !in->p0 || !in->p1 || !in->str || !in->cval_off))
        bad("missing node array");
    if ((in->n_cons && !in->cons) || (in->n_probes && !in->probes) ||
        (in->n_tables && (!in->table_name || !in->table_size)) || (in->n_extra && !in->extra) ||
        (in->n_cval && !in->cval) || (in->n_string_bytes && !in->strings))
        bad("missing array");
    if (in->nreg < 2 || in->nreg > 256 || in->default_entries < 0 || in->default_entries > 4096)
        bad("nreg / default_entries out of range");
    std::vector<std::string> strings;
    {
        const char* p = in->strings;
        const char* end = in->strings + in->n_string_bytes;
        for (int i = 0; i < in->n_strings; i++) {
            const char* z = p < end ? (const char*)std::memchr(p, 0, (size_t)(end - p)) : nullptr;
            if (!z) bad("string table overrun");
            strings.emplace_back(p, (size_t)(z - p));
            p = z + 1;
        }
    }
    if (in->n_nodes && in->arg_off[0] != 0) bad("arg_off[0] != 0");
    std::vector<Src> S(in->n_nodes);
    for (int i = 0; i < in->n_nodes; i++) {
        Src& s = S[i];
        s.op = in->op[i]; s.sort = in->sort[i]; s.width = in->width[i]; s.dom = in->dom[i];
        s.id = in->id[i];
        if (s.op < 0 || s.op > S_OTHER) bad("bad op code");
        if (s.sort < 0 || s.sort > MGC_SORT_ARRAY) bad("bad sort");
        if (s.width < 1 || s.width > MGC_MAX_SOURCE_WIDTH || s.dom < 0 || s.dom > MGC_MAX_SOURCE_WIDTH)
            bad("width out of range");
        if (in->arg_off[i + 1] < in->arg_off[i]) bad("arg_off not monotonic");
        if (in->arg_off[i + 1] > 0 && !in->args) bad("missing args array");
        for (int k = in->arg_off[i]; k < in->arg_off[i + 1]; k++) {
            int a = in->args[k];
            if (a < 0 || a >= i) bad("operand index out of order");
            s.args.push_back(a);
        }
        s.p0 = in->p0[i]; s.p1 = in->p1[i];
        if (in->str[i] >= 0) {
            if (in->str[i] >= in->n_strings) bad("string index out of range");
            s.str = strings[in->str[i]];
        }
        if (s.op == S_BVNUM) {
            int64_t nl = (s.width + 31) / 32;
            if (in->cval_off[i] < 0 || (int64_t)in->cval_off[i] + nl > in->n_cval) bad("numeral limbs out of range");
            s.val.l.assign(in->cval + in->cval_off[i], in->cval + in->cval_off[i] + nl);
            s.val.norm();
        }
        size_t na = s.args.size(), need_min = 0, need_max = (size_t)-1;
        switch (s.op) {
        case S_BVNUM: case S_TRUE: case S_FALSE: case S_VAR: case S_ARRAY: need_max = 0; break;
        case S_BVNEG: case S_BVNOT: case S_NOT: case S_EXTRACT: case S_ZEXT: case S_SEXT: case S_K:
        case S_APPLY: need_min = need_max = 1; break;
        case S_BVSUB: case S_BVUDIV: case S_BVUREM: case S_BVSDIV: case S_BVSREM: case S_BVSMOD:
        case S_BVSHL: case S_BVLSHR: case S_BVASHR: case S_XOR: case S_IMPLIES: case S_BVULT:
        case S_BVULE: case S_BVUGT: case S_BVUGE: case S_BVSLT: case S_BVSLE: case S_BVSGT:
        case S_BVSGE: case S_UMULNO: case S_SELECT: need_min = need_max = 2; break;
        case S_ITE: case S_STORE: need_min = need_max = 3; break;
        case S_BVADD: case S_BVMUL: case S_BVAND: case S_BVOR: case S_BVXOR: case S_AND: case S_OR:
        case S_CONCAT: need_min = 1; break;
        case S_EQ: case S_DISTINCT: need_min = 2; break;
        default: break;
        }
        if (na < need_min || na > need_max) bad("operand count");
        if (s.op == S_EXTRACT && (s.p1 < 0 || s.p0 < s.p1 || s.p0 >= S[s.args[0]].width ||
                                  s.width != s.p0 - s.p1 + 1))
            bad("extract bounds");
        if ((s.op == S_ZEXT || s.op == S_SEXT) && (s.p0 < 0 || s.width != S[s.args[0]].width + s.p0))
            bad("extension width");
        if (s.op == S_APPLY && s.p0 != S[s.args[0]].width) bad("function domain");
    }
    std::vector<int> cons(in->cons, in->cons + in->n_cons);
    std::vector<int> probes(in->probes, in->probes + in->n_probes);
    for (int c : cons) if (c < 0 || c >= in->n_nodes) throw std::runtime_error("constraint index");
    for (int p : probes) if (p < 0 || p >= in->n_nodes) throw std::runtime_error("probe index");
    std::vector<int> all = cons;
    all.insert(all.end(), probes.begin(), probes.end());

    std::vector<U> hints;
    std::vector<int> cons_order;
    if (in->search_hints || in->abi_presets) cons_order = topo(S, cons);
    if (in->search_hints) harvest_hints(S, cons_order, hints);
    Presets presets;
    bool have_presets = in->abi_presets && abi_plan(S, cons_order, presets);
    if (have_presets) {
        for (auto& su : presets.subst) {
            Src& s = S[su.first];
            s.op = S_BVNUM;
            s.args.clear();
            s.str.clear();
            s.p0 = s.p1 = 0;
            s.val = big_of(su.second);
        }
    }

    tp[1] = now_us();
    Lowerer lw(S, in->default_entries);
    for (int t = 0; t < in->n_tables; t++) {
        if (in->table_name[t] < 0 || in->table_name[t] >= in->n_strings || in->table_size[t] < 0 ||
            in->table_size[t] > 4096)
            bad("table entry out of range");
        lw.table_sizes.put(strings[in->table_name[t]], in->table_size[t]);
    }
    lw.solve = in->solve != 0;
    if (in->const_keys || in->solve) {
        std::unordered_map<std::string, int> sym_counts;
        const std::vector<int> all_order = topo(S, all);
        auto ck = scan_const_keys(S, all_order, in->solve ? 256 : 128, in->solve ? 8192 : 2048, sym_counts);
        if (in->const_keys) lw.table_ckeys = ck;
        if (in->solve) {
            for (int n : all_order) {
                if (S[n].op == S_ARRAY || S[n].op == S_APPLY) {
                    auto it = sym_counts.find(S[n].str);
                    if ((it == sym_counts.end() ? 0 : it->second) <= ARG_ENTRIES_CAP) lw.solve_tables.insert(S[n].str);
                }
            }
        }
    }
    Chunks roots;
    std::vector<int64_t> births;
    for (int c : cons) {
        if (!S[c].is_bool()) throw Unsupported("constraint is not Bool");
        roots.push_back(lw.lower(c)[0]);
        births.push_back(S[c].id);
    }
    tp[2] = now_us();
    std::vector<std::pair<int, int>> derived_nodes;
    Solver* solver = nullptr;
    std::unique_ptr<Solver> solver_own;
    if (lw.solve) {
        solver_own.reset(new Solver(lw));
        solver = solver_own.get();
        solver->run(roots, derived_nodes);
        if (solver->dead) {
            births.resize(1);
            probes.clear();
        }
    }
    tp[3] = now_us();
    Memo probe_memo;
    Chunks sinks;
    for (size_t i = 0; i < roots.size(); i++) {
        lw.birth = births[i];
        sinks.push_back(lw.mk(MG_ROOT, 1, {roots[i]}));
    }
    int probe_chunks = 0;
    for (int p : probes) {
        if (S[p].is_array()) throw Unsupported("array probe");
        Chunks chs = lw.lower(p);
        for (int ch : chs) {
            if (solver) { lw.birth = 0; ch = solver->rewrite(ch, probe_memo); }
            lw.birth = S[p].id;
            sinks.push_back(lw.mki(MG_OUT, 1, {ch}, probe_chunks));
            probe_chunks++;
        }
    }
    int n_user_probes = probe_chunks;
    std::vector<std::pair<int, int>> derived;
    std::vector<std::pair<std::string, std::vector<std::vector<int>>>> entry_keys;
    if (solver) {
        auto out = [&](int n) {
            lw.birth = 0;
            sinks.push_back(lw.mki(MG_OUT, 1, {n}, probe_chunks));
            probe_chunks++;
            return probe_chunks - 1;
        };
        std::sort(derived_nodes.begin(), derived_nodes.end());
        for (auto& de : derived_nodes) derived.push_back({de.first, out(de.second)});
        Memo memo_e;
        lw.birth = 0;
        for (auto& te : lw.arg_entries.items) {
            if (solver->dead) break;
            std::vector<std::vector<int>> ks;
            for (auto& ent : te.second) {
                std::vector<int> row;
                for (int k : ent.first) row.push_back(out(solver->rewrite(k, memo_e)));
                ks.push_back(row);
            }
            entry_keys.push_back({te.first, ks});
        }
    }
    if (sinks.empty()) {
        int one = lw.cnst(1, 1);
        sinks.push_back(lw.mk(MG_ROOT, 1, {one}));
    }
    for (auto& n : lw.ln)
        if (is_pred(n.op)) { n.imm = U::of((uint64_t)n.width); n.has_imm = true; n.width = 1; }
    tp[4] = now_us();
    std::unordered_set<int> fused;
    std::vector<int> order = fuse_roots(lw.ln, schedule(lw.ln, sinks), fused);
    tp[5] = now_us();
    U M256 = mask(256);
    std::vector<U> const_values;
    for (int n : order) if (lw.ln[n].op == MG_CONST) const_values.push_back(lw.ln[n].imm & M256);
    for (int i = 0; i < in->n_extra; i++) {
        U v;
        for (int j = 0; j < 8; j++) v.w[j / 2] |= (uint64_t)in->extra[8 * i + j] << (32 * (j & 1));
        const_values.push_back(v);
    }
    for (auto& h : hints) const_values.push_back(h & M256);
    std::sort(const_values.begin(), const_values.end());
    const_values.erase(std::unique(const_values.begin(), const_values.end()), const_values.end());
    std::unordered_map<U, int, UHash> const_index;
    for (size_t i = 0; i < const_values.size(); i++) const_index[const_values[i]] = (int)i;
    Alloc al0(lw.ln, order, const_index, fused, in->nreg, in->remat_mode, in->remat_k,
              in->keep_clean != 0);
    al0.run();
    const Alloc* alp = &al0;
    std::unordered_set<int> fused2;
    std::vector<int> order2;
    std::unique_ptr<Alloc> al2;
    if (!in->solve && !in->leaf_pools && al0.n_lds - LDS_TIER >= SCHEDULE_MIN_SCRATCH) {
        order2 = fuse_roots(lw.ln, schedule_demand(lw.ln, sinks), fused2);
        try {
            al2.reset(new Alloc(lw.ln, order2, const_index, fused2, in->nreg, in->remat_mode,
                                in->remat_k, in->keep_clean != 0));
            al2->run();
        } catch (const Unsupported&) {
            al2.reset();
        }
        auto cost = [](const Alloc& a) {
            return std::make_tuple(std::max(0, a.n_lds - LDS_TIER), a.n_spill + a.n_reload,
                                   (int)a.ins.size());
        };
        if (al2 && cost(*al2) < cost(al0)) alp = al2.get();
    }
    const Alloc& al = *alp;
    const std::vector<int>& ord = alp == &al0 ? order : order2;
    tp[6] = now_us();
    res->code.resize(4 * al.ins.size());
    for (size_t k = 0; k < al.ins.size(); k++) {
        const Ins& x = al.ins[k];
        res->code[4 * k] = x.op | (x.width << 8) | x.flags;
        res->code[4 * k + 1] = x.d | (x.a << 8) | (x.b << 16) | (x.c << 24);
        res->code[4 * k + 2] = x.imm;
        res->code[4 * k + 3] = 0;
    }
    std::vector<std::pair<int, int>> pool_ranges;
    std::vector<std::vector<U>> pools;
    size_t n_rows = const_values.size();
    if (in->leaf_pools) {
        pools = leaf_pools(lw.ln, order, lw.leaves);
        for (size_t li = 0; li < pools.size(); li++) {
            if (!pools[li].empty()) {
                pool_ranges.push_back({(int)n_rows, (int)pools[li].size()});
                n_rows += pools[li].size();
            } else {
                pool_ranges.push_back({0, (int)const_values.size()});
            }
        }
    }
    res->n_rows = (int32_t)n_rows;
    res->n_const_values = (int32_t)const_values.size();
    res->table.resize(8 * n_rows);
    uint32_t* row = res->table.data();
    auto put = [&row](const U& u) {
        for (int j = 0; j < 8; j++) row[j] = (uint32_t)(u.w[j / 2] >> (32 * (j & 1)));
        row += 8;
    };
    for (const U& u : const_values) put(u);
    for (const auto& pl : pools)
        for (const U& u : pl) put(u);

    tp[7] = now_us();
    std::string& o = res->meta;
    bool plain = true;
    for (const Leaf& L : lw.leaves)
        plain = plain && L.name.find_first_of("\t\n") == std::string::npos &&
                L.source.find_first_of("\t\n") == std::string::npos;
    if (!plain) {
        o = "{\"leaves\":[";
        for (size_t i = 0; i < lw.leaves.size(); i++) {
            const Leaf& L = lw.leaves[i];
            if (i) o += ",";
            o += "[";
            jstr(o, L.name);
            o += "," + std::to_string(L.width) + ",";
            jstr(o, KIND_NAMES[L.kind]);
            o += ",";
            jstr(o, L.source);
            o += "," + std::to_string(L.chunk) + "," + std::to_string(L.entry) + "]";
        }
        o += "],\"leaves_rs\":null";
    } else {
        o = "{\"leaves_rs\":";
    }
    if (plain) {
        std::string rs;
        for (size_t i = 0; i < lw.leaves.size(); i++) {
            const Leaf& L = lw.leaves[i];
            if (i) rs += '\n';
            rs += L.name;
            rs += '\t';
            rs += std::to_string(L.width);
            rs += '\t';
            rs += KIND_NAMES[L.kind];
            rs += '\t';
            rs += L.source;
            rs += '\t';
            rs += std::to_string(L.chunk);
            rs += '\t';
            rs += std::to_string(L.entry);
        }
        jstr(o, rs);
    }
    o += ",\"leaf_widths\":[";
    for (size_t i = 0; i < lw.leaves.size(); i++) {
        if (i) o += ",";
        o += std::to_string(lw.leaves[i].width);
    }
    o += "],\"n_lds\":" + std::to_string(al.n_lds);
    o += ",\"n_probes\":" + std::to_string(probe_chunks);
    o += ",\"n_roots\":" + std::to_string(cons.size());
    o += ",\"table_sizes\":[";
    {
        bool first = true;
        for (auto& kv : lw.table_sizes.items) {
            int v = kv.second;
            if (lw.solve_tables.count(kv.first) && lw.table_kinds.has(kv.first)) {
                auto* ents = lw.arg_entries.find(kv.first);
                v = ents ? (int)ents->size() : 0;
            }
            if (!first) o += ",";
            first = false;
            o += "[";
            jstr(o, kv.first);
            o += "," + std::to_string(v) + "]";
        }
    }
    o += "],\"table_kinds\":[";
    for (size_t i = 0; i < lw.table_kinds.items.size(); i++) {
        if (i) o += ",";
        o += "[";
        jstr(o, lw.table_kinds.items[i].first);
        o += ",";
        jstr(o, lw.table_kinds.items[i].second);
        o += "]";
    }
    o += "],\"table_ckeys\":[";
    {
        bool first = true;
        for (auto& kv : lw.table_ckeys.items) {
            if (!lw.table_kinds.has(kv.first)) continue;
            if (!first) o += ",";
            first = false;
            o += "[";
            jstr(o, kv.first);
            o += ",[";
            for (size_t j = 0; j < kv.second.size(); j++) {
                if (j) o += ",";
                jstr(o, kv.second[j].hexs());
            }
            o += "]]";
        }
    }
    std::vector<int> hist(MG_NUM_OPS, 0);
    for (int n : ord) hist[lw.ln[n].op]++;
    o += "],\"lnodes\":" + std::to_string(ord.size());
    o += ",\"spills\":" + std::to_string(al.n_spill);
    o += ",\"reloads\":" + std::to_string(al.n_reload);
    o += ",\"hist\":[";
    {
        bool first = true;
        for (int op = 0; op < MG_NUM_OPS; op++) {
            if (!hist[op]) continue;
            if (!first) o += ",";
            first = false;
            o += "[" + std::to_string(op) + "," + std::to_string(hist[op]) + "]";
        }
    }
    o += "],\"hist_order\":[";
    {
        std::vector<char> seen(MG_NUM_OPS, 0);
        bool first = true;
        for (int n : ord) {
            int op = lw.ln[n].op;
            if (seen[op]) continue;
            seen[op] = 1;
            if (!first) o += ",";
            first = false;
            o += std::to_string(op);
        }
    }
    o += "],\"pool_ranges\":[";
    for (size_t i = 0; i < pool_ranges.size(); i++) {
        if (i) o += ",";
        o += "[" + std::to_string(pool_ranges[i].first) + "," + std::to_string(pool_ranges[i].second) + "]";
    }
    o += "],\"derived\":[";
    for (size_t i = 0; i < derived.size(); i++) {
        if (i) o += ",";
        o += "[" + std::to_string(derived[i].first) + "," + std::to_string(derived[i].second) + "]";
    }
    o += "],\"entry_keys\":[";
    for (size_t i = 0; i < entry_keys.size(); i++) {
        if (i) o += ",";
        o += "[";
        jstr(o, entry_keys[i].first);
        o += ",[";
        for (size_t j = 0; j < entry_keys[i].second.size(); j++) {
            if (j) o += ",";
            o += "[";
            for (size_t k = 0; k < entry_keys[i].second[j].size(); k++) {
                if (k) o += ",";
                o += std::to_string(entry_keys[i].second[j][k]);
            }
            o += "]";
        }
        o += "]]";
    }
    o += "],\"n_user_probes\":" + std::to_string(n_user_probes);
    tp[8] = now_us();
    o += ",\"t_us\":[";
    for (int k = 0; k < 8; k++) {
        char b[32];
        std::snprintf(b, sizeof b, "%s%.1f", k ? "," : "", tp[k + 1] - tp[k]);
        o += b;
    }
    o += "]";
    if (have_presets) {
        o += ",\"presets\":{\"vars\":[";
        for (size_t i = 0; i < presets.vars.size(); i++) {
            if (i) o += ",";
            o += "[";
            jstr(o, presets.vars[i].first);
            o += ",";
            jstr(o, (presets.vars[i].second.neg() ? "-" + hex(U() - presets.vars[i].second) : hex(presets.vars[i].second)));
            o += "]";
        }
        o += "],\"arrays\":[";
        for (size_t i = 0; i < presets.arrays.size(); i++) {
            if (i) o += ",";
            o += "[";
            jstr(o, presets.arrays[i].first);
            o += ",[";
            for (size_t j = 0; j < presets.arrays[i].second.size(); j++) {
                if (j) o += ",";
                o += "[" + std::to_string(presets.arrays[i].second[j].first) + "," +
                     std::to_string(presets.arrays[i].second[j].second) + "]";
            }
            o += "]]";
        }
        o += "]}";
    }
    o += "}";
}

}

extern "C" {

const char* mgc_source_ops(void) { return SOP_NAMES; }

int mgc_compile(const mgc_input* in, mgc_result** out) {
    mgc_result* r = new mgc_result();
    *out = r;
    try {
        compile(in, r);
        return MGC_OK;
    } catch (Unsupported& e) {
        r->error = e.what();
        return MGC_UNSUPPORTED;
    } catch (BadShift& e) {
        r->error = e.what();
        return MGC_ERROR;
    } catch (std::exception& e) {
        r->error = e.what();
        return MGC_ERROR;
    } catch (MemoMiss&) {
        r->error = "operand lowered only as part of a pattern";
        return MGC_UNSUPPORTED;
    }
}

const char* mgc_error(const mgc_result* r) { return r->error.c_str(); }

const uint32_t* mgc_code(const mgc_result* r, int32_t* n_ins) {
    *n_ins = (int32_t)(r->code.size() / 4);
    return r->code.data();
}

const uint32_t* mgc_table(const mgc_result* r, int32_t* n_rows, int32_t* n_const_values) {
    *n_rows = r->n_rows;
    *n_const_values = r->n_const_values;
    return r->table.data();
}

const char* mgc_meta(const mgc_result* r) { return r->meta.c_str(); }

void mgc_free(mgc_result* r) { delete r; }

}
```

### mythril_amd/csrc/mg_compile_py.cpp

```cpp

#define PY_SSIZE_T_CLEAN
#include <Python.h>

#include "mythcc.h"

#include <cstring>
#include <string>
#include <unordered_map>
#include <vector>

namespace {

PyObject *s_op, *s_sort, *s_width, *s_dom, *s_args, *s_params, *s_id, *s_enc;

struct Flat {
    std::vector<int32_t> op, sort, width, dom, arg_off{0}, args, str, cval_off;
    std::vector<int64_t> id, p0, p1;
    std::vector<uint32_t> cval;
    std::string strings;
    int32_t n_strings = 0;
    std::unordered_map<std::string, int32_t> sidx;
    std::unordered_map<PyObject*, int32_t> index;

    int32_t intern(const char* s, Py_ssize_t n) {
        std::string k(s, (size_t)n);
        auto it = sidx.find(k);
        if (it != sidx.end()) return it->second;
        strings.append(k);
        strings.push_back('\0');
        sidx.emplace(std::move(k), n_strings);
        return n_strings++;
    }
};

inline PyObject* attr(PyObject* o, PyObject* name) { return PyObject_GetAttr(o, name); }

bool as_long(PyObject* o, PyObject* name, long long& out) {
    PyObject* v = attr(o, name);
    if (!v) return false;
    out = v == Py_None ? 0 : PyLong_AsLongLong(v);
    Py_DECREF(v);
    return !PyErr_Occurred();
}

bool str_of(PyObject* v, Flat& f, int32_t& out) {
    Py_ssize_t n;
    const char* s = PyUnicode_AsUTF8AndSize(v, &n);
    if (!s) return false;
    out = f.intern(s, n);
    return true;
}

PyObject* encode(PyObject* node, PyObject* ops, int other) {
    PyObject* op = attr(node, s_op);
    if (!op) return nullptr;
    PyObject* code = PyDict_GetItemWithError(ops, op);
    int c = code ? (int)PyLong_AsLong(code) : other;
    if (PyErr_Occurred()) { Py_DECREF(op); return nullptr; }
    Py_ssize_t oplen;
    const char* opname = PyUnicode_AsUTF8AndSize(op, &oplen);
    if (!opname) { Py_DECREF(op); return nullptr; }
    std::string name(opname, (size_t)oplen);

    PyObject* sort = attr(node, s_sort);
    if (!sort) { Py_DECREF(op); return nullptr; }
    int sc;
    if (PyUnicode_CompareWithASCIIString(sort, "bv") == 0) sc = MGC_SORT_BV;
    else if (PyUnicode_CompareWithASCIIString(sort, "bool") == 0) sc = MGC_SORT_BOOL;
    else sc = MGC_SORT_ARRAY;
    Py_DECREF(sort);
    long long width, dom, id;
    if (!as_long(node, s_width, width) || !as_long(node, s_dom, dom) || !as_long(node, s_id, id)) {
        Py_DECREF(op);
        return nullptr;
    }
    PyObject* params = attr(node, s_params);
    if (!params) { Py_DECREF(op); return nullptr; }
    PyObject* ps = PySequence_Fast(params, "params");
    Py_DECREF(params);
    if (!ps) { Py_DECREF(op); return nullptr; }
    Py_ssize_t np_ = PySequence_Fast_GET_SIZE(ps);
    PyObject** pv = PySequence_Fast_ITEMS(ps);
    long long p0 = 0, p1 = 0;
    PyObject* str = Py_None;
    PyObject* cval = Py_None;
    Py_INCREF(Py_None);
    Py_INCREF(Py_None);
    bool ok = true;
    if (name == "bvnum" && np_ >= 1) {
        size_t nl = (size_t)(width + 31) / 32;
        std::vector<unsigned char> buf(4 * nl, 0);
        ok = _PyLong_AsByteArray((PyLongObject*)pv[0], buf.data(), buf.size(), 1, 0) == 0;
        if (ok) {
            Py_DECREF(cval);
            cval = PyBytes_FromStringAndSize((const char*)buf.data(), (Py_ssize_t)buf.size());
            ok = cval != nullptr;
        }
    } else if ((name == "var" || name == "array") && np_ >= 1) {
        Py_DECREF(str); str = pv[0]; Py_INCREF(str);
    } else if (name == "apply" && np_ >= 2) {
        Py_DECREF(str); str = pv[0]; Py_INCREF(str);
        p0 = PyLong_AsLongLong(pv[1]);
        ok = !PyErr_Occurred();
    } else if (name == "extract" && np_ >= 2) {
        p0 = PyLong_AsLongLong(pv[0]);
        p1 = PyLong_AsLongLong(pv[1]);
        ok = !PyErr_Occurred();
    } else if ((name == "zero_extend" || name == "sign_extend") && np_ >= 1) {
        p0 = PyLong_AsLongLong(pv[0]);
        ok = !PyErr_Occurred();
    } else if (c == other) {
        Py_DECREF(str); str = op; Py_INCREF(str);
    }
    Py_DECREF(ps);
    Py_DECREF(op);
    if (!ok) { Py_XDECREF(str); Py_XDECREF(cval); return nullptr; }
    PyObject* t = Py_BuildValue("(iiLLLLLNN)", c, sc, width, dom, id, p0, p1, str, cval);
    if (t && PyObject_SetAttr(node, s_enc, t) < 0) PyErr_Clear();
    return t;
}

bool add_node(PyObject* node, PyObject* seq, PyObject* ops, int other, Flat& f) {
    PyObject* t = PyObject_GetAttr(node, s_enc);
    if (!t) {
        PyErr_Clear();
        t = encode(node, ops, other);
        if (!t) return false;
    }
    if (!PyTuple_Check(t) || PyTuple_GET_SIZE(t) != 9) {
        Py_DECREF(t);
        PyErr_SetString(PyExc_TypeError, "Node._enc is not a walk record");
        return false;
    }
    const int c = (int)PyLong_AsLong(PyTuple_GET_ITEM(t, 0));
    const int sc = (int)PyLong_AsLong(PyTuple_GET_ITEM(t, 1));
    const long long width = PyLong_AsLongLong(PyTuple_GET_ITEM(t, 2));
    const long long dom = PyLong_AsLongLong(PyTuple_GET_ITEM(t, 3));
    const long long id = PyLong_AsLongLong(PyTuple_GET_ITEM(t, 4));
    const long long p0 = PyLong_AsLongLong(PyTuple_GET_ITEM(t, 5));
    const long long p1 = PyLong_AsLongLong(PyTuple_GET_ITEM(t, 6));
    PyObject* so = PyTuple_GET_ITEM(t, 7);
    PyObject* co = PyTuple_GET_ITEM(t, 8);
    if (PyErr_Occurred()) { Py_DECREF(t); return false; }
    Py_ssize_t na = PySequence_Fast_GET_SIZE(seq);
    for (Py_ssize_t i = 0; i < na; i++) {
        auto it = f.index.find(PySequence_Fast_GET_ITEM(seq, i));
        if (it == f.index.end()) {
            Py_DECREF(t);
            PyErr_SetString(PyExc_RuntimeError, "operand visited after its user");
            return false;
        }
        f.args.push_back(it->second);
    }
    int32_t str = -1, cv = -1;
    if (so != Py_None && !str_of(so, f, str)) { Py_DECREF(t); return false; }
    if (co != Py_None) {
        const Py_ssize_t nb = PyBytes_GET_SIZE(co);
        cv = (int32_t)f.cval.size();
        f.cval.resize(f.cval.size() + (size_t)nb / 4, 0);
        std::memcpy(f.cval.data() + cv, PyBytes_AS_STRING(co), (size_t)nb);
    }
    Py_DECREF(t);
    f.op.push_back(c);
    f.sort.push_back(sc);
    f.width.push_back((int32_t)width);
    f.dom.push_back((int32_t)dom);
    f.id.push_back(id);
    f.arg_off.push_back((int32_t)f.args.size());
    f.p0.push_back(p0);
    f.p1.push_back(p1);
    f.str.push_back(str);
    f.cval_off.push_back(cv);
    f.index.emplace(node, (int32_t)(f.op.size() - 1));
    return true;
}

bool walk(PyObject* root, PyObject* ops, int other, Flat& f) {
    if (f.index.count(root)) return true;
    struct It { PyObject* node; PyObject* seq; Py_ssize_t next; };
    std::vector<It> stack;
    auto push = [&](PyObject* n) -> bool {
        PyObject* args = attr(n, s_args);
        if (!args) return false;
        PyObject* seq = PySequence_Fast(args, "args");
        Py_DECREF(args);
        if (!seq) return false;
        stack.push_back({n, seq, 0});
        return true;
    };
    if (!push(root)) return false;
    std::unordered_map<PyObject*, char> open;
    open[root] = 1;
    while (!stack.empty()) {
        It& it = stack.back();
        if (it.next < PySequence_Fast_GET_SIZE(it.seq)) {
            PyObject* a = PySequence_Fast_GET_ITEM(it.seq, it.next++);
            if (f.index.count(a) || open.count(a)) continue;
            open[a] = 1;
            if (!push(a)) goto fail;
            continue;
        }
        {
            PyObject* n = it.node;
            PyObject* seq = it.seq;
            stack.pop_back();
            const bool ok = add_node(n, seq, ops, other, f);
            Py_DECREF(seq);
            if (!ok) goto fail;
        }
    }
    return true;
fail:
    for (auto& it : stack) Py_DECREF(it.seq);
    return false;
}

PyObject* py_compile(PyObject*, PyObject* a) {
    PyObject *cons, *probes, *ops, *tables, *extra;
    int default_entries, nreg, leaf_pools, const_keys, solve, remat_mode, remat_k, keep_clean;
    int search_hints, abi_presets;
    if (!PyArg_ParseTuple(a, "OOO!OiiSiiiiiiii", &cons, &probes, &PyDict_Type, &ops, &tables,
                          &default_entries, &nreg, &extra, &leaf_pools, &const_keys, &solve,
                          &remat_mode, &remat_k, &keep_clean, &search_hints, &abi_presets))
        return nullptr;
    PyObject* oth = PyDict_GetItemString(ops, "?");
    if (!oth) { PyErr_SetString(PyExc_KeyError, "ops has no '?'"); return nullptr; }
    int other = (int)PyLong_AsLong(oth);
    Flat f;
    std::vector<int32_t> ci, pi;
    for (PyObject* lst : {cons, probes}) {
        PyObject* seq = PySequence_Fast(lst, "constraints / probes");
        if (!seq) return nullptr;
        Py_ssize_t n = PySequence_Fast_GET_SIZE(seq);
        for (Py_ssize_t i = 0; i < n; i++)
            if (!walk(PySequence_Fast_GET_ITEM(seq, i), ops, other, f)) { Py_DECREF(seq); return nullptr; }
        for (Py_ssize_t i = 0; i < n; i++)
            (lst == cons ? ci : pi).push_back(f.index.at(PySequence_Fast_GET_ITEM(seq, i)));
        Py_DECREF(seq);
    }
    std::vector<int32_t> tname, tsize;
    PyObject* tseq = PySequence_Fast(tables, "tables");
    if (!tseq) return nullptr;
    for (Py_ssize_t i = 0; i < PySequence_Fast_GET_SIZE(tseq); i++) {
        PyObject* t = PySequence_Fast_GET_ITEM(tseq, i);
        int32_t s;
        if (!PyTuple_Check(t) || PyTuple_GET_SIZE(t) != 2 || !str_of(PyTuple_GET_ITEM(t, 0), f, s)) {
            Py_DECREF(tseq);
            if (!PyErr_Occurred()) PyErr_SetString(PyExc_TypeError, "tables: (name, size) pairs");
            return nullptr;
        }
        tname.push_back(s);
        tsize.push_back((int32_t)PyLong_AsLong(PyTuple_GET_ITEM(t, 1)));
    }
    Py_DECREF(tseq);
    if (PyErr_Occurred()) return nullptr;
    mgc_input in;
    std::memset(&in, 0, sizeof in);
    in.n_nodes = (int32_t)f.op.size();
    in.op = f.op.data(); in.sort = f.sort.data(); in.width = f.width.data(); in.dom = f.dom.data();
    in.id = f.id.data(); in.arg_off = f.arg_off.data(); in.args = f.args.data();
    in.p0 = f.p0.data(); in.p1 = f.p1.data(); in.str = f.str.data(); in.cval_off = f.cval_off.data();
    in.cval = f.cval.data(); in.strings = f.strings.data(); in.n_strings = f.n_strings;
    in.n_cons = (int32_t)ci.size(); in.cons = ci.data();
    in.n_probes = (int32_t)pi.size(); in.probes = pi.data();
    in.n_tables = (int32_t)tname.size(); in.table_name = tname.data(); in.table_size = tsize.data();
    in.default_entries = default_entries; in.nreg = nreg;
    in.n_extra = (int32_t)(PyBytes_GET_SIZE(extra) / 32);
    in.extra = (const uint32_t*)PyBytes_AS_STRING(extra);
    in.leaf_pools = leaf_pools; in.const_keys = const_keys; in.solve = solve;
    in.remat_mode = remat_mode; in.remat_k = remat_k; in.keep_clean = keep_clean;
    in.search_hints = search_hints; in.abi_presets = abi_presets;
    in.n_cval = (int32_t)f.cval.size(); in.n_string_bytes = (int32_t)f.strings.size();
    mgc_result* res = nullptr;
    int rc;
    Py_BEGIN_ALLOW_THREADS
    rc = mgc_compile(&in, &res);
    Py_END_ALLOW_THREADS
    PyObject* out;
    if (rc != MGC_OK) {
        out = Py_BuildValue("(isOOiO)", rc, mgc_error(res), Py_None, Py_None, 0, Py_None);
    } else {
        int32_t n_ins, rows, ncv;
        const uint32_t* code = mgc_code(res, &n_ins);
        const uint32_t* table = mgc_table(res, &rows, &ncv);
        static const char empty[1] = {0};
        out = Py_BuildValue("(iOy#y#is)", rc, Py_None, code ? (const char*)code : empty,
                            (Py_ssize_t)(16 * n_ins), table ? (const char*)table : empty,
                            (Py_ssize_t)(32 * rows), ncv, mgc_meta(res));
    }
    mgc_free(res);
    return out;
}

struct UF {
    std::vector<int> p;
    int add() { p.push_back((int)p.size()); return (int)p.size() - 1; }
    int find(int x) { while (p[x] != x) { p[x] = p[p[x]]; x = p[x]; } return x; }
    void join(int a, int b) { a = find(a); b = find(b); if (a != b) p[b] = a; }
};

PyObject* py_buckets(PyObject*, PyObject* a) {
    PyObject* cons;
    if (!PyArg_ParseTuple(a, "O", &cons)) return nullptr;
    PyObject* seq = PySequence_Fast(cons, "constraints");
    if (!seq) return nullptr;
    std::unordered_map<PyObject*, int> idx;
    std::vector<char> has_sym;
    std::unordered_map<std::string, int> sym;
    UF uf;
    struct It { PyObject* node; PyObject* args; Py_ssize_t next; };
    std::vector<It> stack;
    auto fail = [&]() -> PyObject* {
        for (auto& it : stack) Py_DECREF(it.args);
        Py_DECREF(seq);
        return nullptr;
    };
    auto open = [&](PyObject* n) -> bool {
        PyObject* args = attr(n, s_args);
        if (!args) return false;
        PyObject* fs = PySequence_Fast(args, "args");
        Py_DECREF(args);
        if (!fs) return false;
        stack.push_back({n, fs, 0});
        return true;
    };
    auto close = [&](PyObject* n, PyObject* args) -> bool {
        int me = uf.add();
        has_sym.push_back(0);
        PyObject* op = attr(n, s_op);
        if (!op) return false;
        bool is_var = PyUnicode_CompareWithASCIIString(op, "var") == 0;
        bool is_tab = !is_var && (PyUnicode_CompareWithASCIIString(op, "array") == 0 ||
                                  PyUnicode_CompareWithASCIIString(op, "apply") == 0);
        Py_DECREF(op);
        if (is_var || is_tab) {
            PyObject* params = attr(n, s_params);
            if (!params) return false;
            PyObject* name = PyTuple_Check(params) && PyTuple_GET_SIZE(params) ? PyTuple_GET_ITEM(params, 0) : nullptr;
            Py_ssize_t len;
            const char* s = name ? PyUnicode_AsUTF8AndSize(name, &len) : nullptr;
            if (!s) { Py_DECREF(params); if (!PyErr_Occurred()) PyErr_SetString(PyExc_TypeError, "symbol name"); return false; }
            std::string key = std::string(is_var ? "v:" : "t:") + std::string(s, (size_t)len);
            Py_DECREF(params);
            auto it = sym.find(key);
            int se;
            if (it == sym.end()) {
                se = uf.add();
                has_sym.push_back(1);
                sym.emplace(key, se);
            } else {
                se = it->second;
            }
            uf.join(se, me);
            has_sym[me] = 1;
        }
        for (Py_ssize_t i = 0; i < PySequence_Fast_GET_SIZE(args); i++) {
            int c = idx.at(PySequence_Fast_GET_ITEM(args, i));
            if (has_sym[c]) { uf.join(me, c); has_sym[me] = 1; }
        }
        idx.emplace(n, me);
        return true;
    };
    Py_ssize_t nc = PySequence_Fast_GET_SIZE(seq);
    for (Py_ssize_t i = 0; i < nc; i++) {
        PyObject* r = PySequence_Fast_GET_ITEM(seq, i);
        if (idx.count(r)) continue;
        if (!open(r)) return fail();
        while (!stack.empty()) {
            It& it = stack.back();
            if (it.next < PySequence_Fast_GET_SIZE(it.args)) {
                PyObject* c = PySequence_Fast_GET_ITEM(it.args, it.next++);
                if (idx.count(c)) continue;
                if (!open(c)) return fail();
                continue;
            }
            PyObject* n = it.node;
            PyObject* args = it.args;
            stack.pop_back();
            bool ok = close(n, args);
            Py_DECREF(args);
            if (!ok) return fail();
        }
    }
    PyObject* out = PyList_New(nc);
    std::unordered_map<int, long> label;
    std::unordered_map<int, long> per_root;
    for (auto& kv : idx) if (has_sym[kv.second]) per_root[uf.find(kv.second)]++;
    std::vector<long> sizes;
    for (Py_ssize_t i = 0; i < nc; i++) {
        int e = idx.at(PySequence_Fast_GET_ITEM(seq, i));
        long l;
        if (!has_sym[e]) {
            l = (long)label.size();
            label[-1 - (int)i] = l;
            sizes.push_back(1);
        } else {
            int root = uf.find(e);
            auto it = label.find(root);
            if (it == label.end()) {
                l = label[root] = (long)label.size();
                sizes.push_back(per_root[root]);
            } else {
                l = it->second;
            }
        }
        PyList_SET_ITEM(out, i, PyLong_FromLong(l));
    }
    Py_DECREF(seq);
    PyObject* sz = PyList_New((Py_ssize_t)sizes.size());
    for (size_t g = 0; g < sizes.size(); g++) PyList_SET_ITEM(sz, (Py_ssize_t)g, PyLong_FromLong(sizes[g]));
    return Py_BuildValue("(NN)", out, sz);
}

PyMethodDef methods[] = {
    {"compile", py_compile, METH_VARARGS, "Flatten a constraint DAG and compile it (include/mythcc.h)."},
    {"buckets", py_buckets, METH_VARARGS, "Independent-group label of each constraint."},
    {nullptr, nullptr, 0, nullptr}};

PyModuleDef module = {PyModuleDef_HEAD_INIT, "_mythcc", "native host compiler front-end", -1, methods};

}

PyMODINIT_FUNC PyInit__mythcc(void) {
    s_op = PyUnicode_InternFromString("op");
    s_sort = PyUnicode_InternFromString("sort");
    s_width = PyUnicode_InternFromString("width");
    s_dom = PyUnicode_InternFromString("dom");
    s_args = PyUnicode_InternFromString("args");
    s_params = PyUnicode_InternFromString("params");
    s_id = PyUnicode_InternFromString("id");
    s_enc = PyUnicode_InternFromString("_enc");
    return PyModule_Create(&module);
}
```

### mythril_amd/ir.py

```python

from __future__ import annotations

from dataclasses import dataclass, field
from typing import Dict, List, Optional, Sequence, Tuple

import numpy as np

from . import irdefs as I
from .smt.node import Node, topo_order

CHUNK = 256
MAX_SPILL = I.MAX_LDS + I.MAX_PSLOTS
LDS_TIER = 6
import os as _os
LEAF_REMAT = _os.environ.get("MYTHRIL_GPU_LEAF_REMAT", "scratch2")


class Unsupported(Exception):
    """The DAG uses something the GPU path does not evaluate (→ z3)."""


class LNode:
    __slots__ = ("op", "width", "args", "imm", "id", "birth")

    def __init__(self, op, width, args, imm, nid, birth):
        self.op = op
        self.width = width
        self.args = args
        self.imm = imm
        self.id = nid
        self.birth = birth

    def __repr__(self):
        return "L%d:%s/%d%s" % (self.id, I.OPNAME.get(self.op, self.op), self.width,
                                 "" if self.imm is None else "[%s]" % (self.imm,))


@dataclass
class Leaf:
    name: str
    width: int
    kind: str
    source: str
    chunk: int = 0
    entry: int = 0


@dataclass
class Program:
    code: np.ndarray
    consts: np.ndarray
    const_values: List[int]
    leaves: List[Leaf]
    n_lds: int
    n_probes: int
    n_roots: int
    table_sizes: Dict[str, int]
    table_kinds: Dict[str, str] = field(default_factory=dict)
    table_ckeys: Dict[str, List[int]] = field(default_factory=dict)
    stats: Dict[str, object] = field(default_factory=dict)
    pool_ranges: List[Tuple[int, int]] = field(default_factory=list)
    derived: Dict[int, int] = field(default_factory=dict)
    entry_keys: Dict[str, List[List[int]]] = field(default_factory=dict)
    n_user_probes: int = 0
    presets: object = None
    group_key: object = None
    nreg: int = 16

    @property
    def solved(self) -> bool:
        return bool(self.derived or self.entry_keys or self.presets)

    @property
    def n_ins(self) -> int:
        return int(self.code.shape[0])

    def leaf_index(self) -> Dict[str, int]:
        return {l.name: i for i, l in enumerate(self.leaves)}



def _limbs(value: int) -> List[int]:
    return [(value >> (32 * j)) & 0xFFFFFFFF for j in range(8)]


class _Lowerer:
    def __init__(self, table_sizes: Dict[str, int], default_entries: int):
        self.table = {}
        self.nid = 0
        self.leaves: List[Leaf] = []
        self.leaf_ids: Dict[str, int] = {}
        self.memo: Dict[int, List[LNode]] = {}
        self.sel_memo: Dict[Tuple[int, Tuple[int, ...]], List[LNode]] = {}
        self.table_sizes = dict(table_sizes)
        self.table_kinds: Dict[str, str] = {}
        self.default_entries = default_entries
        self.consts_seen: set = set()
        self.birth = 0
        self.table_ckeys: Dict[str, List[int]] = {}
        self.solve = False
        self.solve_tables: set = set()
        self.arg_entries: Dict[str, List[Tuple[List[LNode], List[LNode]]]] = {}

    def mk(self, op: int, width: int, args=(), imm=None) -> LNode:
        if op == I.CONCAT and width == I.MAX_WIDTH and args[0].op == I.EXTRACT and \
                args[0].imm == 0 and args[0].args[0].width == I.MAX_WIDTH:
            args = (args[0].args[0],) + tuple(args[1:])
        key = (op, width, tuple(a.id for a in args), imm)
        n = self.table.get(key)
        if n is None:
            self.nid += 1
            birth = self.birth
            for a in args:
                if a.birth > birth:
                    birth = a.birth
            n = LNode(op, width, tuple(args), imm, self.nid, birth)
            self.table[key] = n
        return n

    def const(self, value: int, width: int) -> LNode:
        value &= (1 << width) - 1
        self.consts_seen.add(value)
        return self.mk(I.CONST, width, (), value)

    def leaf(self, name: str, width: int, kind: str, source: str, chunk=0, entry=0) -> LNode:
        idx = self.leaf_ids.get(name)
        if idx is None:
            idx = len(self.leaves)
            self.leaf_ids[name] = idx
            self.leaves.append(Leaf(name, width, kind, source, chunk, entry))
        return self.mk(I.LEAF, width, (), idx)

    @staticmethod
    def nchunks(w: int) -> int:
        return (w + CHUNK - 1) // CHUNK

    @staticmethod
    def chunk_width(w: int, i: int) -> int:
        return min(CHUNK, w - CHUNK * i)

    def bits(self, chunks: Sequence[LNode], w: int, lo: int, hi: int) -> LNode:
        ci, cj = lo // CHUNK, hi // CHUNK
        if ci == cj:
            c = chunks[ci]
            cw = self.chunk_width(w, ci)
            l0, h0 = lo - CHUNK * ci, hi - CHUNK * ci
            if l0 == 0 and h0 == cw - 1:
                return c
            return self.mk(I.EXTRACT, h0 - l0 + 1, (c,), l0)
        low_w = CHUNK * (ci + 1) - lo
        low = self.bits(chunks, w, lo, CHUNK * (ci + 1) - 1)
        high = self.bits(chunks, w, CHUNK * cj, hi)
        return self.mk(I.CONCAT, hi - lo + 1, (high, low), low_w)

    def assemble(self, pieces: List[Tuple[List[LNode], int]]) -> List[LNode]:
        total = sum(w for _, w in pieces)
        segs, off = [], 0
        for ch, w in reversed(pieces):
            segs.append((ch, w, off))
            off += w
        out = []
        for k in range(self.nchunks(total)):
            lo_k, hi_k = CHUNK * k, min(total, CHUNK * (k + 1)) - 1
            acc: Optional[LNode] = None
            acc_w = 0
            for ch, w, o in segs:
                a, b = max(lo_k, o), min(hi_k, o + w - 1)
                if a > b:
                    continue
                part = self.bits(ch, w, a - o, b - o)
                pw = b - a + 1
                if acc is None:
                    acc, acc_w = part, pw
                else:
                    acc = self.mk(I.CONCAT, acc_w + pw, (part, acc), acc_w)
                    acc_w += pw
            out.append(acc)
        return out

    def lower(self, n: Node) -> List[LNode]:
        r = self.memo.get(n.id)
        if r is not None:
            return r
        nodes = self._pending(n)
        skip = set()
        for m in nodes:
            if m.op == "extract" and self._is_carry(m):
                s = m.args[0]
                skip.update((s.id, s.args[0].id, s.args[1].id))
        saved = self.birth
        for m in nodes:
            if m.id in self.memo or m.is_array() or (m.id in skip and m is not n):
                continue
            try:
                self.birth = m.id
                self.memo[m.id] = self._lower_one(m)
            except KeyError as e:
                raise Unsupported("operand lowered only as part of a pattern") from e
            finally:
                self.birth = m.id
        self.birth = max(saved, self.birth) if saved else self.birth
        return self.memo[n.id]

    def _pending(self, n: Node) -> List[Node]:
        memo, seen, out = self.memo, set(), []
        stack = [(n, False)]
        while stack:
            m, done = stack.pop()
            if done:
                out.append(m)
                continue
            if m.id in seen or m.id in memo:
                continue
            seen.add(m.id)
            stack.append((m, True))
            for a in reversed(m.args):
                if a.id not in seen and a.id not in memo:
                    stack.append((a, False))
        return out

    def _narrow(self, n: Node) -> LNode:
        ch = self.memo[n.id]
        if len(ch) != 1:
            raise Unsupported("%s on a %d-bit value" % (n.op, n.width))
        return ch[0]

    def _fold(self, op: int, width: int, args: List[LNode]) -> LNode:
        acc = args[0]
        for a in args[1:]:
            acc = self.mk(op, width, (acc, a))
        return acc

    def _by_constant(self, op: str, w: int, n: Node) -> Optional[LNode]:
        if n.args[1].op != "bvnum":
            return None
        c = n.args[1].params[0]
        x = self._narrow(n.args[0])
        if op in ("bvudiv", "bvurem"):
            if c <= 0 or c & (c - 1):
                return None
            k = c.bit_length() - 1
            if op == "bvurem":
                return self.const(0, w) if k == 0 else self.mk(I.EXTRACT, k, (x,), 0)
            op, c = "bvlshr", k
        if op not in ("bvshl", "bvlshr", "bvashr"):
            return None
        if c == 0:
            return x
        if op == "bvashr":
            c = min(c, w - 1)
            return self.mk(I.SEXT, w, (self.mk(I.EXTRACT, w - c, (x,), c),), w - c)
        if c >= w:
            return self.const(0, w)
        if op == "bvlshr":
            return self.mk(I.EXTRACT, w - c, (x,), c)
        return self.mk(I.CONCAT, w, (self.mk(I.EXTRACT, w - c, (x,), 0), self.const(0, c)), c)

    def _lower_one(self, n: Node) -> List[LNode]:
        op, w = n.op, n.width
        if w > CHUNK:
            return self._lower_wide(n)
        A = lambda i: self._narrow(n.args[i])
        if op == "bvnum":
            return [self.const(n.params[0], w)]
        if op == "true":
            return [self.const(1, 1)]
        if op == "false":
            return [self.const(0, 1)]
        if op == "var":
            return [self.leaf(n.params[0], w, "var", n.params[0])]
        simple = {"bvsub": I.SUB, "bvudiv": I.UDIV, "bvurem": I.UREM, "bvsdiv": I.SDIV,
                  "bvsrem": I.SREM, "bvsmod": I.SMOD, "bvshl": I.SHL, "bvlshr": I.LSHR,
                  "bvashr": I.ASHR}
        if op in simple:
            red = self._by_constant(op, w, n)
            if red is not None:
                return [red]
            return [self.mk(simple[op], w, (A(0), A(1)))]
        nary = {"bvadd": I.ADD, "bvmul": I.MUL, "bvand": I.AND, "bvor": I.OR, "bvxor": I.XOR,
                "and": I.AND, "or": I.OR}
        if op in nary:
            return [self._fold(nary[op], w, [A(i) for i in range(len(n.args))])]
        if op in ("bvneg",):
            return [self.mk(I.NEG, w, (A(0),))]
        if op in ("bvnot", "not"):
            return [self.mk(I.NOT, w, (A(0),))]
        if op == "xor":
            return [self.mk(I.XOR, 1, (A(0), A(1)))]
        if op == "=>":
            return [self.mk(I.OR, 1, (self.mk(I.NOT, 1, (A(0),)), A(1)))]
        cmp = {"bvult": (I.ULT, False), "bvule": (I.ULE, False), "bvugt": (I.ULT, True),
               "bvuge": (I.ULE, True), "bvslt": (I.SLT, False), "bvsle": (I.SLE, False),
               "bvsgt": (I.SLT, True), "bvsge": (I.SLE, True), "bvumul_noovfl": (I.UMULNO, False)}
        if op in cmp:
            kop, swap = cmp[op]
            a, b = A(0), A(1)
            if swap:
                a, b = b, a
            return [self.mk(kop, n.args[0].width, (a, b))]
        if op in ("=", "distinct"):
            if any(x.is_array() for x in n.args):
                raise Unsupported("array equality")
            return [self._eq_or_distinct(op, n)]
        if op == "ite":
            if n.is_array():
                raise Unsupported("array-valued ite outside select")
            return [self.mk(I.ITE, w, (A(0), A(1), A(2)))]
        if op == "concat":
            word = self._calldata_word(n)
            if word is not None:
                return [word]
            return self.assemble([(self.memo[a.id], a.width) for a in n.args])
        if op == "extract":
            hi, lo = n.params
            src = n.args[0]
            carry = self._carry_pattern(n)
            if carry is not None:
                return [carry]
            return [self.bits(self.memo[src.id], src.width, lo, hi)]
        if op == "zero_extend":
            return [self._narrow(n.args[0])]
        if op == "sign_extend":
            return [self.mk(I.SEXT, w, (A(0),), n.args[0].width)]
        if op == "select":
            return self._select(n.args[0], self.memo[n.args[1].id], n.args[1].width, w)
        if op == "apply":
            fname, dom = n.params
            return self._table(fname, self.memo[n.args[0].id], dom, w, "func")
        raise Unsupported("operator %s" % op)

    def _eq_or_distinct(self, op: str, n: Node) -> LNode:
        args = [self.memo[a.id] for a in n.args]
        w = n.args[0].width

        def eq(x, y):
            parts = [self.mk(I.EQ, self.chunk_width(w, k) if w > CHUNK else w, (x[k], y[k]))
                     for k in range(len(x))]
            return self._fold(I.AND, 1, parts)
        if op == "=":
            return eq(args[0], args[1])
        terms = []
        for i in range(len(args)):
            for j in range(i + 1, len(args)):
                terms.append(self.mk(I.NOT, 1, (eq(args[i], args[j]),)))
        return self._fold(I.AND, 1, terms)

    @staticmethod
    def _is_carry(n: Node) -> bool:
        hi, lo = n.params
        s = n.args[0]
        if hi != lo or s.op != "bvadd" or len(s.args) != 2 or hi != s.width - 1:
            return False
        a, b = s.args
        return (a.op == "zero_extend" and b.op == "zero_extend" and a.params == (1,) and
                b.params == (1,) and a.args[0].width <= CHUNK)

    def _carry_pattern(self, n: Node) -> Optional[LNode]:
        if not self._is_carry(n):
            return None
        x, y = n.args[0].args[0].args[0], n.args[0].args[1].args[0]
        lx, ly = self.lower(x)[0], self.lower(y)[0]
        return self.mk(I.ULT, x.width, (self.mk(I.ADD, x.width, (lx, ly)), lx))

    def _lower_wide(self, n: Node) -> List[LNode]:
        op, w = n.op, n.width
        if op == "bvnum":
            v = n.params[0]
            return [self.const(v >> (CHUNK * k), self.chunk_width(w, k)) for k in range(self.nchunks(w))]
        if op == "var":
            return [self.leaf("%s#%d" % (n.params[0], k), self.chunk_width(w, k), "var",
                              n.params[0], chunk=k) for k in range(self.nchunks(w))]
        if op == "concat":
            return self.assemble([(self.memo[a.id], a.width) for a in n.args])
        if op == "extract":
            src = n.args[0]
            hi, lo = n.params
            return self.assemble([([self.bits(self.memo[src.id], src.width, lo + CHUNK * k,
                                              min(hi, lo + CHUNK * k + CHUNK - 1))],
                                   min(CHUNK, hi - lo + 1 - CHUNK * k))
                                  for k in reversed(range(self.nchunks(w)))])
        if op == "zero_extend":
            src = n.args[0]
            pad = w - src.width
            pieces = []
            while pad > 0:
                pw = min(CHUNK, pad)
                pieces.append(([self.const(0, pw)], pw))
                pad -= pw
            return self.assemble(pieces + [(self.memo[src.id], src.width)])
        if op == "ite":
            c = self._narrow(n.args[0])
            a, b = self.memo[n.args[1].id], self.memo[n.args[2].id]
            return self._ite_chunks(c, a, b)
        if op == "select":
            return self._select(n.args[0], self.memo[n.args[1].id], n.args[1].width, w)
        if op == "apply":
            fname, dom = n.params
            return self._table(fname, self.memo[n.args[0].id], dom, w, "func")
        raise Unsupported("%s on a %d-bit value" % (op, w))

    @staticmethod
    def _index_parts(x: Node) -> Tuple[Optional[Node], int]:
        c = 0
        while True:
            if x.op == "bvnum":
                return None, (c + x.params[0]) % (1 << 256)
            if x.op != "bvadd" or len(x.args) != 2:
# ... 213 lines not shown
    for i, n in enumerate(order):
        for a in n.args:
            uses.setdefault(a.id, []).append(i)
    ptr: Dict[int, int] = {}
    reg_of: Dict[int, int] = {}
    lds_of: Dict[int, int] = {}
    holder: Dict[int, LNode] = {}
    free_regs = list(range(nreg))[::-1]
    reg_clean: Dict[int, bool] = {}
    free_lds: List[int] = []
    n_lds = 0
    ins: List[Tuple[int, int, int, int, int, int, int]] = []
    n_spill = n_reload = 0

    def next_use(v: LNode, i: int) -> int:
        u = uses.get(v.id, [])
        p = ptr.get(v.id, 0)
        while p < len(u) and u[p] < i:
            p += 1
        ptr[v.id] = p
        return u[p] if p < len(u) else 1 << 60

    def free_to_drop(v: LNode) -> bool:
        return v.op == I.CONST or v.id in lds_of

    def droppable_when_full(v: LNode) -> bool:
        return free_to_drop(v) or v.op == I.LEAF

    def alloc_reg(i: int, protect: set, oldest: bool = False) -> int:
        nonlocal n_lds, n_spill
        if free_regs:
            return free_regs.pop(0 if oldest else -1)
        victim, far = None, -1
        for r, v in holder.items():
            if v.id in protect:
                continue
            nu = next_use(v, i)
            if nu > far:
                victim, far = v, nu
        if victim is None:
            raise Unsupported("register pressure")
        if not free_to_drop(victim) and not free_lds and n_lds >= MAX_SPILL:
            victim, far = None, -1
            for r, v in holder.items():
                if v.id in protect or not droppable_when_full(v):
                    continue
                nu = next_use(v, i)
                if nu > far:
                    victim, far = v, nu
            if victim is None:
                raise Unsupported("spill budget exceeded")
        r = reg_of.pop(victim.id)
        del holder[r]
        slots_left = bool(free_lds) or n_lds < MAX_SPILL
        if victim.op == I.LEAF and victim.id not in lds_of and leaf_remat != "spill":
            tier = LDS_TIER + (int(leaf_remat[7:]) if leaf_remat[7:].isdigit() else 0)
            cheap_free = (free_lds and min(free_lds) < tier) or n_lds < tier
            if leaf_remat == "always" or not cheap_free:
                slots_left = False
        if not free_to_drop(victim) and slots_left:
            if free_lds:
                s = min(free_lds)
                free_lds.remove(s)
            else:
                s = n_lds
                n_lds += 1
            lds_of[victim.id] = s
            ins.append((I.SPILL, 1, trash, r, 0, 0, s))
            n_spill += 1
        return r

    def materialise(v: LNode, r: int):
        nonlocal n_reload
        reg_clean[r] = v.width <= 32
        if v.op == I.CONST:
            ins.append((I.CONST, v.width, r, 0, 0, 0, const_index[v.imm]))
        elif v.id in lds_of:
            ins.append((I.RELOAD, v.width, r, 0, 0, 0, lds_of[v.id]))
            n_reload += 1
        else:
            ins.append((I.LEAF, v.width, r, 0, 0, 0, v.imm))

    def release(v: LNode, i: int):
        if next_use(v, i + 1) >= (1 << 60):
            r = reg_of.pop(v.id, None)
            if r is not None:
                del holder[r]
                free_regs.append(r)
            s = lds_of.pop(v.id, None)
            if s is not None:
                free_lds.append(s)

    for i, n in enumerate(order):
        protect = {a.id for a in n.args}
        for a in n.args:
            if a.id not in reg_of:
                r = alloc_reg(i, protect, oldest=a.op != I.CONST)
                materialise(a, r)
                reg_of[a.id] = r
                holder[r] = a
        slots = [reg_of[a.id] for a in n.args]
        for a in dict.fromkeys(n.args):
            release(a, i)
        if n.op in (I.ROOT, I.OUT):
            ins.append((n.op, 1, trash, slots[0], 0, 0, n.imm or 0))
            continue
        flags = I.ROOT_FLAG if n.id in fused else 0
        if not uses.get(n.id):
            if free_regs:
                d = free_regs[-1]
            else:
                d = alloc_reg(i, set())
                free_regs.append(d)
            if not (n.id in fused and (n.op in _CMP_OPS or
                                       (n.op in (I.AND, I.OR, I.XOR) and n.width <= 32))):
                reg_clean[d] = n.width <= 32
        else:
            d = None
            if n.op in _INPLACE and n.width > 32:
                cand = slots[1:3] if n.op == I.ITE else \
                    slots[:1] if n.op in (I.CDWE, I.CDWX) else slots[:2]
                for r in cand:
                    if r in free_regs:
                        free_regs.remove(r)
                        d = r
                        break
            if d is None and n.width <= 32:
                for r in reversed(free_regs):
                    if reg_clean.get(r):
                        free_regs.remove(r)
                        d = r
                        break
            if d is None and n.width > 32 and KEEP_CLEAN:
                for r in reversed(free_regs):
                    if not reg_clean.get(r):
                        free_regs.remove(r)
                        d = r
                        break
            if d is None:
                d = alloc_reg(i, set())
            reg_clean[d] = n.width <= 32
            reg_of[n.id] = d
            holder[d] = n
        op = n.op
        a = slots[0] if len(slots) > 0 else 0
        b = slots[1] if len(slots) > 1 else 0
        c = 0
        imm = 0
        width = n.width
        if op == I.CONST:
            imm = const_index[n.imm]
        elif op == I.LEAF:
            imm = n.imm
        elif op in (I.EXTRACT, I.CONCAT, I.SEXT):
            imm = n.imm
        elif op in (I.EQ, I.ULT, I.ULE, I.SLT, I.SLE, I.UMULNO):
            width = n.imm
        elif op == I.ITE:
            c, a, b = slots[0], slots[1], slots[2]
        elif op in (I.CDWE, I.CDWX):
            c = slots[2]
        ins.append((op, width, d, a, b, c, imm, flags))
    return ins, n_lds, n_spill, n_reload


_CMP_OPS = (I.EQ, I.ULT, I.ULE, I.SLT, I.SLE)
KEEP_CLEAN = True
POOL_CAP = 128


def _pool_values(c: int, w: int) -> List[int]:
    out = [c, (c + 63) & ((1 << 256) - 1) & ~63]
    if w < 256:
        for k in range(0, max(8, c.bit_length()), 8):
            out.append((c >> k) & ((1 << w) - 1))
    return out


def _bits(x: int):
    while x:
        low = x & -x
        yield low.bit_length() - 1
        x ^= low


def _leaf_pools(order: List[LNode], leaves: List["Leaf"]) -> List[List[int]]:
    values = sorted({n.imm for n in order if n.op == I.CONST})
    cidx = {v: i for i, v in enumerate(values)}
    under_l: Dict[int, int] = {}
    under_c: Dict[int, int] = {}
    pools: List[Dict[int, None]] = [dict() for _ in leaves]
    done: List[int] = [0] * len(leaves)
    pv: Dict[Tuple[int, int], List[int]] = {}
    M256 = (1 << 256) - 1
    for n in order:
        if n.op == I.LEAF:
            under_l[n.id], under_c[n.id] = 1 << n.imm, 0
            continue
        if n.op == I.CONST:
            under_l[n.id], under_c[n.id] = 0, 1 << cidx[n.imm]
            continue
        ls = cs = 0
        for a in n.args:
            ls |= under_l.get(a.id, 0)
            cs |= under_c.get(a.id, 0)
        if cs.bit_count() > POOL_CAP:
            keep = 0
            for k, ci in enumerate(_bits(cs)):
                if k == POOL_CAP:
                    break
                keep |= 1 << ci
            cs = keep
        under_l[n.id], under_c[n.id] = ls, cs
        if n.op in _CMP_OPS and cs:
            for li in _bits(ls):
                p = pools[li]
                if len(p) >= POOL_CAP:
                    continue
                new = cs & ~done[li]
                if not new:
                    continue
                done[li] |= new
                w = leaves[li].width
                for ci in _bits(new):
                    c = values[ci]
                    vals = pv.get((c, w))
                    if vals is None:
                        vals = pv[(c, w)] = [v & M256 for v in _pool_values(c, w)]
                    for v in vals:
                        p.setdefault(v)
                        if len(p) >= POOL_CAP:
                            break
                    if len(p) >= POOL_CAP:
                        break
    return [list(p) for p in pools]


CKEY_CAP = 128
CKEY_LINKS = 2048
ARG_ENTRIES_CAP = 64


def scan_const_keys(nodes: Sequence[Node], cap: int = CKEY_CAP,
                    max_links: int = CKEY_LINKS,
                    sym_counts: Optional[Dict[str, int]] = None) -> Dict[str, List[int]]:
    out: Dict[str, Dict[int, None]] = {}
    sym: Dict[str, set] = {}

    def bases(a: Node):
        stack, seen = [a], set()
        while stack:
            x = stack.pop()
            if x.id in seen:
                continue
            seen.add(x.id)
            if x.op == "store":
                stack.append(x.args[0])
            elif x.op == "ite":
                stack.extend(x.args[1:])
            elif x.op == "array":
                yield x.params[0]

    def note(name: str, key: Node):
        if key.op == "bvnum":
            d = out.setdefault(name, {})
            if len(d) < cap:
                d.setdefault(key.params[0])
        else:
            sym.setdefault(name, set()).add(key.id)

    for n in topo_order(list(nodes)):
        if n.op == "select":
            for name in bases(n.args[0]):
                note(name, n.args[1])
        elif n.op == "apply":
            note(n.params[0], n.args[0])
    ck = {k: sorted(v) for k, v in out.items() if v and len(sym.get(k, ())) * len(v) <= max_links}
    if sym_counts is not None:
        sym_counts.update({k: len(v) for k, v in sym.items()})
    return ck


def harvest_hints(nodes: Sequence[Node]) -> List[int]:
    out = set()
    for n in topo_order(list(nodes)):
        if n.op == "bvnum" and n.width >= 8:
            v = n.params[0]
            out.add((v + 63) & ~63)
            if 0 < v < (1 << 32):
                out.add(v << 224)
    return sorted(out)


def lw_tables(constraints, probes) -> set:
    out = set()
    for n in topo_order(list(constraints) + list(probes)):
        if n.op == "array":
            out.add(n.params[0])
        elif n.op == "apply":
            out.add(n.params[0])
    return out


COMPILER = _os.environ.get("MYTHRIL_GPU_COMPILER", "native")


AUTO_SCRATCH_SHARE = 0.02
AUTO_ALWAYS_HEAVY = 0.01
_HEAVY = (I.MUL, I.UDIV, I.UREM, I.SDIV, I.SREM, I.SMOD, I.UMULNO)


def heavy_share(p: Program) -> float:
    if not len(p.code):
        return 0.0
    op = p.code[:, 0] & 0xFF
    return float(np.isin(op, _HEAVY).sum()) / len(p.code)


def scratch_reload_share(p: Program, lds_tier: int = LDS_TIER) -> float:
    code = p.code
    if not len(code):
        return 0.0
    op = code[:, 0] & 0xFF
    width = (code[:, 0] >> 8) & 0x3FF
    hit = (op == I.RELOAD) & (width > 32) & (code[:, 2] >= lds_tier)
    return float(hit.sum()) / len(code)


def compile_constraints(constraints: Sequence[Node], probes: Sequence[Node] = (),
                        table_sizes: Optional[Dict[str, int]] = None,
                        default_entries: int = 2, nreg: int = I.NREG,
                        extra_consts: Sequence[int] = (), leaf_pools: bool = False,
                        const_keys: bool = False, solve: bool = False, search_hints: bool = False,
                        abi_presets: bool = False, leaf_remat: Optional[str] = None) -> Program:
    global LEAF_REMAT
    policy = leaf_remat or LEAF_REMAT
    if policy == "auto":
        args = (constraints, probes, table_sizes, default_entries, nreg, extra_consts,
                leaf_pools, const_keys, solve, search_hints, abi_presets)
        p = compile_constraints(*args, leaf_remat="scratch2")
        if heavy_share(p) < AUTO_ALWAYS_HEAVY:
            p = compile_constraints(*args, leaf_remat="always")
        elif scratch_reload_share(p) > AUTO_SCRATCH_SHARE:
            p = compile_constraints(*args, leaf_remat="scratch")
        return p
    if COMPILER == "py":
        saved, LEAF_REMAT = LEAF_REMAT, policy
        try:
            return compile_constraints_py(constraints, probes, table_sizes, default_entries, nreg,
                                          extra_consts, leaf_pools, const_keys, solve, search_hints,
                                          abi_presets)
        finally:
            LEAF_REMAT = saved
    from .ccompile import compile_native
    return compile_native(constraints, probes, table_sizes, default_entries, nreg, extra_consts,
                          leaf_pools, const_keys, solve, leaf_remat=policy,
                          search_hints=search_hints, abi_presets=abi_presets)


def compile_constraints_py(constraints: Sequence[Node], probes: Sequence[Node] = (),
                           table_sizes: Optional[Dict[str, int]] = None,
                           default_entries: int = 2, nreg: int = I.NREG,
                           extra_consts: Sequence[int] = (), leaf_pools: bool = False,
                           const_keys: bool = False, solve: bool = False,
                           search_hints: bool = False, abi_presets: bool = False) -> Program:
    constraints, probes = list(constraints), list(probes)
    if search_hints:
        extra_consts = list(extra_consts) + harvest_hints(constraints)
    plan = None
    if abi_presets:
        from . import abi
        plan = abi.plan(constraints)
        if plan is not None:
            constraints, probes = plan.view(constraints), plan.view(probes)
    lw = _Lowerer(table_sizes or {}, default_entries)
    lw.solve = solve
    if const_keys or solve:
        sym_counts: Dict[str, int] = {}
        ck = scan_const_keys(list(constraints) + list(probes), sym_counts=sym_counts,
                             cap=256 if solve else CKEY_CAP,
                             max_links=8192 if solve else CKEY_LINKS)
        if const_keys:
            lw.table_ckeys = ck
        lw.solve_tables = {k for k in lw_tables(constraints, probes)
                           if sym_counts.get(k, 0) <= ARG_ENTRIES_CAP} if solve else set()
    roots: List[LNode] = []
    births: List[int] = []
    for c in constraints:
        if not c.is_bool():
            raise Unsupported("constraint is not Bool")
        roots.append(lw.lower(c)[0])
        births.append(c.id)
    derived_nodes: Dict[int, LNode] = {}
    solver = None
    if solve:
        from .solve import Solver
        solver = Solver(lw)
        roots, derived_nodes = solver.run(roots)
        probe_memo: Dict[int, LNode] = {}
        if solver.dead:
            births, probes = births[:1], ()
    sinks: List[LNode] = []
    for r, b in zip(roots, births):
        lw.birth = b
        sinks.append(lw.mk(I.ROOT, 1, (r,), None))
    probe_chunks = 0
    for p in probes:
        if p.is_array():
            raise Unsupported("array probe")
        for ch in lw.lower(p):
            if solver is not None:
                lw.birth = 0
                ch = solver.rewrite(ch, probe_memo)
            lw.birth = p.id
            sinks.append(lw.mk(I.OUT, 1, (ch,), probe_chunks))
            probe_chunks += 1
    n_user_probes = probe_chunks
    derived: Dict[int, int] = {}
    entry_keys: Dict[str, List[List[int]]] = {}
    if solve:
        def out(n: LNode) -> int:
            nonlocal probe_chunks
            lw.birth = 0
            sinks.append(lw.mk(I.OUT, 1, (n,), probe_chunks))
            probe_chunks += 1
            return probe_chunks - 1
        for li, e in sorted(derived_nodes.items()):
            derived[li] = out(e)
        memo_e: Dict[int, LNode] = {}
        lw.birth = 0
        for name, ents in (lw.arg_entries.items() if not solver.dead else ()):
            entry_keys[name] = [[out(solver.rewrite(k, memo_e)) for k in key]
                                for key, _ in ents]
    if not sinks:
        sinks.append(lw.mk(I.ROOT, 1, (lw.const(1, 1),), None))
    for n in list(lw.table.values()):
        if n.op in (I.EQ, I.ULT, I.ULE, I.SLT, I.SLE, I.UMULNO):
            n.imm = n.width
            n.width = 1
    order, fused = _fuse_roots(_schedule(sinks))
    const_values = sorted({n.imm & ((1 << 256) - 1) for n in order if n.op == I.CONST} |
                          {v & ((1 << 256) - 1) for v in extra_consts})
    const_index = {v: i for i, v in enumerate(const_values)}
    ins, n_lds, n_spill, n_reload = _allocate(order, const_index, fused, nreg)
    if not solve and not leaf_pools and SCHEDULE_CHOICE and \
            n_lds - LDS_TIER >= SCHEDULE_MIN_SCRATCH:
        order2, fused2 = _fuse_roots(_schedule_demand(sinks))
        try:
            alt = _allocate(order2, const_index, fused2, nreg)
        except Unsupported:
            alt = None
        if alt is not None and _alloc_cost(alt[1], alt[2], alt[3], len(alt[0])) < \
                _alloc_cost(n_lds, n_spill, n_reload, len(ins)):
            ins, n_lds, n_spill, n_reload = alt
            order, fused = order2, fused2
    code = np.zeros((len(ins), 4), dtype=np.uint32)
    for k, (op, width, d, a, b, c, imm, *fl) in enumerate(ins):
        code[k, 0] = op | (width << 8) | (fl[0] if fl else 0)
        code[k, 1] = I.w1(d, a, b, c)
        code[k, 2] = imm
    table = list(const_values)
    pool_ranges: List[Tuple[int, int]] = []
    if leaf_pools:
        for li, p in enumerate(_leaf_pools(order, lw.leaves)):
            if p:
                pool_ranges.append((len(table), len(p)))
                table.extend(p)
            else:
                pool_ranges.append((0, len(const_values)))
    consts = np.frombuffer(b"".join(v.to_bytes(32, "little") for v in table),
                           dtype="<u4").reshape(-1, 8).astype(np.uint32)
    hist: Dict[str, int] = {}
    for n in order:
        hist[I.OPNAME[n.op]] = hist.get(I.OPNAME[n.op], 0) + 1
    stats = {"lnodes": len(order), "n_ins": len(ins), "spills": n_spill, "reloads": n_reload,
             "hist": hist}
    ckeys = {k: v for k, v in lw.table_ckeys.items() if k in lw.table_kinds}
    tsizes = dict(lw.table_sizes)
    for name in lw.solve_tables & set(lw.table_kinds):
        tsizes[name] = len(lw.arg_entries.get(name, ()))
    prog = Program(code, consts, const_values, lw.leaves, n_lds, probe_chunks,
                   len(constraints), tsizes, lw.table_kinds, ckeys, stats, pool_ranges,
                   derived, entry_keys, n_user_probes)
    prog.nreg = nreg
    if plan is not None:
        prog.presets = plan
    return prog
```

### mythril_amd/roofline.py

```python

from __future__ import annotations

from typing import Dict, Iterable, Tuple

from .smt.node import Node, topo_order

VALU_PEAK_OPS = 256 * 4 * 64 / 2.019 * 2.4e9
HBM_PEAK_BPS = 8.0e12

_W8 = {"bvadd", "bvsub", "bvneg", "bvand", "bvor", "bvxor", "bvnot", "=", "distinct",
       "bvult", "bvule", "bvugt", "bvuge", "bvslt", "bvsle", "bvsgt", "bvsge", "ite",
       "concat", "extract", "zero_extend", "sign_extend"}
_BOOL = {"and", "or", "xor", "not", "=>"}
_LEAF = {"var", "bvnum", "true", "false", "array", "K"}


def _scale(w: int) -> float:
    return ((w + 31) // 32) / 8.0


def node_weight(n: Node, table_sizes: Dict[str, int]) -> float:
    op = n.op
    if op in _LEAF or op == "store":
        return 0.0
    if n.is_bool() and op in _BOOL:
        return float(max(1, len(n.args) - 1))
    w = n.args[0].width if n.args and n.args[0].is_bv() else n.width
    if op in ("ite", "=", "distinct") and n.args and n.args[-1].is_bool():
        return 1.0
    if op in _W8:
        return 8.0 * _scale(max(w, n.width))
    if op in ("bvshl", "bvlshr", "bvashr"):
        if n.args[1].op == "bvnum":
            return 8.0 * _scale(w)
        return 24.0 * _scale(w)
    if op == "bvmul":
        return 192.0 * _scale(w) * (len(n.args) - 1)
    if op == "bvumul_noovfl":
        return 320.0 * _scale(w)
    if op in ("bvudiv", "bvurem") and _pow2_divisor(n):
        return 8.0 * _scale(w)
    if op in ("bvudiv", "bvurem", "bvsdiv", "bvsrem", "bvsmod"):
        return 512.0 * _scale(w)
    if op == "select":
        s, a = 0, n.args[0]
        while a.op == "store":
            s, a = s + 1, a.args[0]
        extra = 8 * table_sizes.get(a.params[0], 2) + 8 if a.op == "array" else 0
        return 8.0 * s + 8.0 + extra
    if op == "apply":
        return 8.0 * table_sizes.get(n.params[0], 2) + 8.0
    return 8.0


def _pow2_divisor(n: Node) -> bool:
    d = n.args[1]
    return d.op == "bvnum" and d.params[0] > 0 and not d.params[0] & (d.params[0] - 1)


def _index_parts(x: Node):
    c = 0
    while True:
        if x.op == "bvnum":
            return None, (c + x.params[0]) % (1 << 256)
        if x.op != "bvadd" or len(x.args) != 2:
            return x, c
        a, b = x.args
        if b.op == "bvnum" and a.op != "bvnum":
            x, c = a, (c + b.params[0]) % (1 << 256)
        elif a.op == "bvnum" and b.op != "bvnum":
            x, c = b, (c + a.params[0]) % (1 << 256)
        else:
            return x, c


def calldata_word(n: Node):
    if n.op != "concat" or n.width != 256 or len(n.args) != 32:
        return None
    size = arr = base = None
    c0 = 0
    inner = []
    for i, x in enumerate(n.args):
        if x.op != "ite" or x.width != 8:
            return None
        cond, sel, zero = x.args
        if zero.op != "bvnum" or zero.params[0] != 0 or cond.op != "bvslt" or sel.op != "select":
            return None
        idx = sel.args[1]
        if cond.args[0] is not idx or idx.width != 256:
            return None
        if i == 0:
            size, arr = cond.args[1], sel.args[0]
            if arr.op != "array":
                return None
            base, c0 = _index_parts(idx)
        elif cond.args[1] is not size or sel.args[0] is not arr:
            return None
        else:
            b, c = _index_parts(idx)
            if b is not base or c != (c0 + i) % (1 << 256):
                return None
            inner.append(idx)
        inner.extend((x, cond, sel))
    return arr.params[0], inner


def dag_work(roots: Iterable[Node], table_sizes: Dict[str, int] = None) -> Tuple[int, float]:
    ts = table_sizes or {}
    order = topo_order(list(roots))
    users: Dict[int, list] = {}
    for n in order:
        for a in n.args:
            users.setdefault(a.id, []).append(n.id)
    words: Dict[int, float] = {}
    cand = set()
    for n in order:
        cw = calldata_word(n)
        if cw is not None:
            name, inner = cw
            words[n.id] = 16.0 * ts.get(name, 2) + 24.0
            cand.update(x.id for x in inner)
    absorbed = set()
    for n in reversed(order):
        if n.id in cand and all(u in words or u in absorbed for u in users.get(n.id, ())):
            absorbed.add(n.id)
    nodes = 0
    weight = 0.0
    for n in order:
        if n.op in _LEAF:
            continue
        nodes += 1
        if n.id in words:
            weight += words[n.id]
        elif n.id not in absorbed:
            weight += node_weight(n, ts)
    return nodes, weight
```

Measured before the change: 1844 billion.

## Add constant folding and algebraic peephole simplification to constraint lowering

```diff
diff --git a/include/mythcc.h b/include/mythcc.h
--- a/include/mythcc.h
+++ b/include/mythcc.h
@@ -58,6 +58,7 @@
     int32_t abi_presets;
     int32_t n_cval;
     int32_t n_string_bytes;
+    int32_t no_simplify;
 } mgc_input;
 
 typedef struct mgc_result mgc_result;
diff --git a/mythril_amd/ccompile.py b/mythril_amd/ccompile.py
--- a/mythril_amd/ccompile.py
+++ b/mythril_amd/ccompile.py
@@ -39,7 +39,7 @@
          ("remat_mode", ctypes.c_int32), ("remat_k", ctypes.c_int32),
          ("keep_clean", ctypes.c_int32), ("search_hints", ctypes.c_int32),
          ("abi_presets", ctypes.c_int32), ("n_cval", ctypes.c_int32),
-         ("n_string_bytes", ctypes.c_int32)]
+         ("n_string_bytes", ctypes.c_int32), ("no_simplify", ctypes.c_int32)]
 
 
 def load():
@@ -97,7 +97,7 @@
                    nreg: int = I.NREG, extra_consts: Sequence[int] = (), leaf_pools: bool = False,
                    const_keys: bool = False, solve: bool = False, leaf_remat: Optional[str] = None,
                    keep_clean: Optional[bool] = None, search_hints: bool = False,
-                   abi_presets: bool = False):
+                   abi_presets: bool = False, simplify: Optional[bool] = None):
     from . import ir
     ext = _load_ext()
     M = (1 << 256) - 1
@@ -109,7 +109,7 @@
         list(constraints), list(probes), _OPS, list((table_sizes or {}).items()), default_entries,
         nreg, extra, int(leaf_pools), int(const_keys), int(solve), mode, k,
         int(ir.KEEP_CLEAN if keep_clean is None else keep_clean), int(search_hints),
-        int(abi_presets))
+        int(abi_presets), int(not (ir.SIMPLIFY if simplify is None else simplify)))
     if rc != MGC_OK:
         if rc == MGC_UNSUPPORTED:
             raise ir.Unsupported(err)
@@ -195,7 +195,8 @@
                           nreg: int = I.NREG, extra_consts: Sequence[int] = (),
                           leaf_pools: bool = False, const_keys: bool = False, solve: bool = False,
                           leaf_remat: Optional[str] = None, keep_clean: Optional[bool] = None,
-                          search_hints: bool = False, abi_presets: bool = False):
+                          search_hints: bool = False, abi_presets: bool = False,
+                          simplify: Optional[bool] = None):
     from . import ir
     lib = load()
     f = flatten(constraints, probes, table_sizes, extra_consts)
@@ -211,7 +212,8 @@
                  len(f["table_name"]), P["table_name"], P["table_size"], default_entries, nreg,
                  len(f["extra"]) // 32, P["extra"], int(leaf_pools), int(const_keys), int(solve),
                  mode, k, int(ir.KEEP_CLEAN if keep_clean is None else keep_clean),
-                 int(search_hints), int(abi_presets), len(f["cval"]) // 4, len(f["strings"]))
+                 int(search_hints), int(abi_presets), len(f["cval"]) // 4, len(f["strings"]),
+                 int(not (ir.SIMPLIFY if simplify is None else simplify)))
     res = ctypes.c_void_p()
     rc = lib.mgc_compile(ctypes.byref(inp), ctypes.byref(res))
     try:
@@ -276,7 +278,8 @@
 def _program(code, raw: bytes, ncv: int, meta):
     from . import ir
     consts = np.frombuffer(raw, dtype="<u4").reshape(-1, 8).astype(np.uint32)
-    const_values = [int.from_bytes(raw[32 * i:32 * i + 32], "little") for i in range(ncv)]
+    rows = [int.from_bytes(raw[32 * i:32 * i + 32], "little") for i in range(len(raw) // 32)]
+    const_values = ir.ConstValues(rows[:ncv], rows[ncv:])
     Leaf = ir.Leaf
     if meta.get("leaves_rs") is not None:
         leaves = LeafRecords(meta["leaves_rs"], meta["leaf_widths"])
@@ -285,13 +288,15 @@
     hist_counts = dict(meta["hist"])
     stats = {"lnodes": meta["lnodes"], "n_ins": int(code.shape[0]), "spills": meta["spills"],
              "reloads": meta["reloads"],
-             "hist": {I.OPNAME[op]: hist_counts[op] for op in meta["hist_order"]}}
+             "hist": {I.OPNAME[op]: hist_counts[op] for op in meta["hist_order"]},
+             "folded": meta["folded"]}
     prog = ir.Program(code, consts, const_values, leaves, meta["n_lds"], meta["n_probes"],
                       meta["n_roots"], dict(meta["table_sizes"]), dict(meta["table_kinds"]),
                       {k: [int(h, 16) for h in v] for k, v in meta["table_ckeys"]}, stats,
                       [tuple(r) for r in meta["pool_ranges"]], dict(meta["derived"]),
                       {k: v for k, v in meta["entry_keys"]}, meta["n_user_probes"])
     prog.compile_us = meta.get("t_us")
+    prog.appended = meta["appended"]
     pre = meta.get("presets")
     if pre is not None:
         from .abi import Plan
diff --git a/mythril_amd/csrc/mg_compile.cpp b/mythril_amd/csrc/mg_compile.cpp
--- a/mythril_amd/csrc/mg_compile.cpp
+++ b/mythril_amd/csrc/mg_compile.cpp
@@ -114,6 +114,15 @@
 static U U1(int k) { return shl(U::of(1), k); }
 static bool nz(const U& a) { return !a.zero(); }
 
+static void udivmod(const U& a, const U& b, U& q, U& r) {
+    q = U(); r = U();
+    for (int i = a.bitlen() - 1; i >= 0; i--) {
+        r = shl(r, 1);
+        if (a.bit(i)) r.w[0] |= 1;
+        if (r >= b) { r = r - b; q.w[i >> 6] |= 1ull << (i & 63); }
+    }
+}
+
 static std::string hex(const U& a) {
     char buf[8];
     std::string s;
@@ -375,7 +384,196 @@
         slot_id.swap(ids);
         slot_hash.swap(hs);
     }
+    bool simplify = false;
+    int64_t folded = 0;
+
+    static bool simplify_op(int op) {
+        switch (op) {
+        case MG_ADD: case MG_SUB: case MG_MUL: case MG_NEG: case MG_AND: case MG_OR: case MG_XOR:
+        case MG_NOT: case MG_SHL: case MG_LSHR: case MG_ASHR: case MG_UDIV: case MG_UREM:
+        case MG_SDIV: case MG_SREM: case MG_SMOD: case MG_ITE: case MG_CONCAT: case MG_EXTRACT:
+        case MG_SEXT: case MG_EQ: case MG_ULT: case MG_ULE: case MG_SLT: case MG_SLE:
+        case MG_UMULNO: return true;
+        default: return false;
+        }
+    }
+
+    static U const_eval(int op, int w, const U* v, int imm) {
+        const U m = mask(w);
+        if (op == MG_CONCAT) return (shl(v[0], imm) | v[1]) & m;
+        if (op == MG_EXTRACT) return shr(v[0], imm) & m;
+        if (op == MG_SEXT) {
+            U x = v[0] & mask(imm);
+            if (x.bit(imm - 1)) x = x | ~mask(imm);
+            return x & m;
+        }
+        auto neg = [&m](const U& x) { return (U() - x) & m; };
+        const U a = v[0] & m;
+        if (op == MG_NEG) return neg(a);
+        if (op == MG_NOT) return ~a & m;
+        const U b = v[1] & m;
+        const U bit1 = U::of(1), none = U();
+        switch (op) {
+        case MG_ADD: return (a + b) & m;
+        case MG_SUB: return (a - b) & m;
+        case MG_MUL: return (a * b) & m;
+        case MG_AND: return a & b;
+        case MG_OR: return a | b;
+        case MG_XOR: return a ^ b;
+        case MG_SHL: return b >= U::of((uint64_t)w) ? none : shl(a, (int)b.w[0]) & m;
+        case MG_LSHR: return b >= U::of((uint64_t)w) ? none : shr(a, (int)b.w[0]);
+        case MG_ASHR: {
+            U sa = a.bit(w - 1) ? (a | ~m) : a;
+            int k = b >= U::of((uint64_t)(w - 1)) ? w - 1 : (int)b.w[0];
+            return sar(sa, k) & m;
+        }
+        case MG_UDIV: case MG_UREM: {
+            if (b.zero()) return op == MG_UDIV ? m : a;
+            U q, r;
+            udivmod(a, b, q, r);
+            return op == MG_UDIV ? q : r;
+        }
+        case MG_SDIV: case MG_SREM: case MG_SMOD: {
+            bool na = a.bit(w - 1), nb = b.bit(w - 1);
+            U ua = na ? neg(a) : a, ub = nb ? neg(b) : b;
+            U q = m, r = ua;
+            if (!ub.zero()) udivmod(ua, ub, q, r);
+            if (op == MG_SDIV) return na != nb ? neg(q) : q;
+            if (op == MG_SREM) return na ? neg(r) : r;
+            if (r.zero() || !(na || nb)) return r;
+            if (na && nb) return neg(r);
+            return (na ? b - r : r + b) & m;
+        }
+        case MG_EQ: return a == b ? bit1 : none;
+        case MG_ULT: return a < b ? bit1 : none;
+        case MG_ULE: return a <= b ? bit1 : none;
+        case MG_SLT: case MG_SLE: {
+            U h = U1(w - 1);
+            U x = a ^ h, y = b ^ h;
+            return (op == MG_SLT ? x < y : x <= y) ? bit1 : none;
+        }
+        case MG_UMULNO: {
+            if (a.zero() || b.zero()) return bit1;
+            if (a.bitlen() + b.bitlen() >= w + 2) return none;
+            return a * b <= m ? bit1 : none;
+        }
+        default: throw std::runtime_error("const_eval: op");
+        }
+    }
+
+    int shl_form(int x, int k, int w) {
+        if (k == 0) return x;
+        if (k >= w) return cnst(0, w);
+        int e = mki(MG_EXTRACT, w - k, {x}, 0);
+        int z = cnst(0, k);
+        return mki(MG_CONCAT, w, {e, z}, k);
+    }
+    int div_guard(int x, int w, uint64_t other) {
+        int z = cnst(0, w);
+        int e = mk(MG_EQ, w, {x, z});
+        int ones = cnst(mask(w), w);
+        int t = cnst(other, w);
+        return mk(MG_ITE, w, {e, ones, t});
+    }
+
+    int rule(int op, int w, const Args& args, const U& imm) {
+        const U m = mask(w);
+        auto isc = [this](int x) { return ln[x].op == MG_CONST; };
+        if (op == MG_ITE) {
+            int c = args[0], a = args[1], b = args[2];
+            if (isc(c)) return (ln[c].imm.w[0] & 1) ? a : b;
+            if (a == b) return a;
+            return -1;
+        }
+        bool all = true;
+        for (int x : args) if (!isc(x)) { all = false; break; }
+        if (all) {
+            U v[2];
+            for (size_t i = 0; i < args.size() && i < 2; i++) v[i] = ln[args[i]].imm;
+            return cnst(const_eval(op, w, v, (int)imm.w[0]), is_pred(op) ? 1 : w);
+        }
+        if (args.size() != 2 || op == MG_CONCAT) return -1;
+        int a = args[0], b = args[1];
+        if (a == b) {
+            switch (op) {
+            case MG_SUB: case MG_XOR: return cnst(0, w);
+            case MG_AND: case MG_OR: return ln[a].width <= w ? a : -1;
+            case MG_EQ: case MG_ULE: case MG_SLE: return cnst(1, 1);
+            case MG_ULT: case MG_SLT: return cnst(0, 1);
+            case MG_UREM: case MG_SREM: case MG_SMOD: return cnst(0, w);
+            case MG_UDIV: case MG_SDIV: return div_guard(a, w, 1);
+            default: return -1;
+            }
+        }
+        if (op == MG_ADD || op == MG_MUL || op == MG_AND || op == MG_OR || op == MG_XOR ||
+            op == MG_UMULNO) {
+            int x;
+            U c;
+            if (isc(a)) { x = b; c = ln[a].imm & m; }
+            else if (isc(b)) { x = a; c = ln[b].imm & m; }
+            else return -1;
+            bool fits = ln[x].width <= w;
+            const U one = U::of(1);
+            switch (op) {
+            case MG_ADD:
+                if (c.zero() && fits) return x;
+                break;
+            case MG_MUL:
+                if (c.zero()) return cnst(0, w);
+                if (c == one && fits) return x;
+                if ((c & (c - one)).zero() && fits) return shl_form(x, c.bitlen() - 1, w);
+                if ((c & (c + one)).zero() && fits) {
+                    int s = shl_form(x, c.bitlen(), w);
+                    return mk(MG_SUB, w, {s, x});
+                }
+                break;
+            case MG_AND:
+                if (c.zero()) return cnst(0, w);
+                if (c == m && fits) return x;
+                break;
+            case MG_OR:
+                if (c.zero() && fits) return x;
+                if (c == m) return cnst(m, w);
+                break;
+            case MG_XOR:
+                if (c.zero() && fits) return x;
+                break;
+            default:
+                if (c <= one) return cnst(1, 1);
+                break;
+            }
+            return -1;
+        }
+        if (isc(b)) {
+            const U c = ln[b].imm & m;
+            bool fits = ln[a].width <= w;
+            if (c.zero()) {
+                if ((op == MG_SUB || op == MG_UREM || op == MG_SREM || op == MG_SHL ||
+                     op == MG_LSHR || op == MG_ASHR) && fits)
+                    return a;
+                if (op == MG_UDIV) return cnst(m, w);
+                if (op == MG_ULT) return cnst(0, 1);
+            }
+            if (c == U::of(1)) {
+                if ((op == MG_UDIV || op == MG_SDIV) && fits) return a;
+                if (op == MG_UREM || op == MG_SREM) return cnst(0, w);
+            }
+            if (c == m && op == MG_ULE) return cnst(1, 1);
+        } else if (isc(a) && (ln[a].imm & m).zero()) {
+            if (op == MG_UDIV || op == MG_SDIV) return div_guard(b, w, 0);
+            if (op == MG_UREM || op == MG_SREM || op == MG_SHL || op == MG_LSHR || op == MG_ASHR)
+                return cnst(0, w);
+            if (op == MG_ULE) return cnst(1, 1);
+        }
+        return -1;
+    }
+
     int mk(int op, int width, Args args, bool has_imm = false, const U& imm = U()) {
+        if (simplify && !args.empty() && simplify_op(op)) {
+            const U im = has_imm ? imm : U();
+            int r = rule(op, width, args, im);
+            if (r >= 0) { folded++; return r; }
+        }
         if (op == MG_CONCAT && width == MG_MAX_WIDTH && ln[args[0]].op == MG_EXTRACT &&
             ln[args[0]].imm.zero() && ln[ln[args[0]].args[0]].width == MG_MAX_WIDTH)
             args[0] = ln[args[0]].args[0];
@@ -996,6 +1194,7 @@
 static const int PASSES = 6;
 static const int MAX_REFUSALS = 4;
 static const int SCHEDULE_MIN_SCRATCH = 10;
+static const double SIMPLIFY_MIN_HEAVY = 0.01;
 static const int MAX_DOMAIN = 16;
 static const int MAX_BRANCHES = 4;
 static const int MAX_OR = 64;
@@ -2914,6 +3113,8 @@
         lw.table_sizes.put(strings[in->table_name[t]], in->table_size[t]);
     }
     lw.solve = in->solve != 0;
+    lw.simplify = !in->no_simplify && !in->solve;
+    const OMap<std::string, int> given_sizes = lw.table_sizes;
     if (in->const_keys || in->solve) {
         std::unordered_map<std::string, int> sym_counts;
         const std::vector<int> all_order = topo(S, all);
@@ -2951,9 +3152,17 @@
     tp[3] = now_us();
     Memo probe_memo;
     Chunks sinks;
+    std::unordered_set<int> rooted;
     for (size_t i = 0; i < roots.size(); i++) {
         lw.birth = births[i];
-        sinks.push_back(lw.mk(MG_ROOT, 1, {roots[i]}));
+        if (lw.simplify && rooted.count(roots[i])) {
+            lw.ln.push_back(LN{MG_ROOT, 1, Args{roots[i]}, false, U(),
+                               std::max(births[i], lw.ln[roots[i]].birth)});
+            sinks.push_back((int)lw.ln.size() - 1);
+        } else {
+            sinks.push_back(lw.mk(MG_ROOT, 1, {roots[i]}));
+        }
+        rooted.insert(roots[i]);
     }
     int probe_chunks = 0;
     for (int p : probes) {
@@ -3000,10 +3209,56 @@
     tp[4] = now_us();
     std::unordered_set<int> fused;
     std::vector<int> order = fuse_roots(lw.ln, schedule(lw.ln, sinks), fused);
+    std::vector<int> unread;
+    if (lw.folded) {
+        std::vector<char> have(lw.leaves.size(), 0);
+        for (int n : order) if (lw.ln[n].op == MG_LEAF) have[(size_t)lw.ln[n].imm.w[0]] = 1;
+        for (size_t i = 0; i < lw.leaves.size(); i++)
+            if (!have[i]) unread.push_back(lw.mki(MG_LEAF, lw.leaves[i].width, {}, (int64_t)i));
+        order.insert(order.end(), unread.begin(), unread.end());
+    }
     tp[5] = now_us();
     U M256 = mask(256);
-    std::vector<U> const_values;
-    for (int n : order) if (lw.ln[n].op == MG_CONST) const_values.push_back(lw.ln[n].imm & M256);
+    std::vector<U> used_consts, const_values;
+    for (int n : order) if (lw.ln[n].op == MG_CONST) used_consts.push_back(lw.ln[n].imm & M256);
+    if (lw.folded) {
+        Lowerer plain(S, in->default_entries);
+        plain.table_sizes = given_sizes;
+        plain.table_ckeys = lw.table_ckeys;
+        Chunks stack;
+        for (int c : cons) stack.push_back(plain.lower(c)[0]);
+        for (int p : probes) { Chunks chs = plain.lower(p); stack.insert(stack.end(), chs.begin(), chs.end()); }
+        if (stack.empty()) stack.push_back(plain.cnst(1, 1));
+        bool same = plain.leaves.size() == lw.leaves.size();
+        for (size_t i = 0; same && i < lw.leaves.size(); i++) {
+            const Leaf &x = plain.leaves[i], &y = lw.leaves[i];
+            same = x.name == y.name && x.width == y.width && x.kind == y.kind &&
+                   x.source == y.source && x.chunk == y.chunk && x.entry == y.entry;
+        }
+        std::vector<char> seen(plain.ln.size(), 0);
+        size_t reach = 0, heavy = 0;
+        while (!stack.empty()) {
+            int n = stack.back();
+            stack.pop_back();
+            if (seen[n]) continue;
+            seen[n] = 1;
+            reach++;
+            const LN& x = plain.ln[n];
+            if (x.op == MG_CONST) const_values.push_back(x.imm & M256);
+            heavy += x.op == MG_MUL || x.op == MG_UDIV || x.op == MG_UREM || x.op == MG_SDIV ||
+                     x.op == MG_SREM || x.op == MG_SMOD || x.op == MG_UMULNO;
+            for (int a : x.args) stack.push_back(a);
+        }
+        if (!same || (double)heavy < SIMPLIFY_MIN_HEAVY * (double)reach) {
+            mgc_input off = *in;
+            off.no_simplify = 1;
+            *res = mgc_result();
+            compile(&off, res);
+            return;
+        }
+    } else {
+        const_values = used_consts;
+    }
     for (int i = 0; i < in->n_extra; i++) {
         U v;
         for (int j = 0; j < 8; j++) v.w[j / 2] |= (uint64_t)in->extra[8 * i + j] << (32 * (j & 1));
@@ -3014,6 +3269,20 @@
     const_values.erase(std::unique(const_values.begin(), const_values.end()), const_values.end());
     std::unordered_map<U, int, UHash> const_index;
     for (size_t i = 0; i < const_values.size(); i++) const_index[const_values[i]] = (int)i;
+    std::vector<std::vector<U>> pools;
+    size_t n_pool_rows = 0;
+    if (in->leaf_pools) {
+        pools = leaf_pools(lw.ln, order, lw.leaves);
+        for (const auto& pl : pools) n_pool_rows += pl.size();
+    }
+    std::sort(used_consts.begin(), used_consts.end());
+    used_consts.erase(std::unique(used_consts.begin(), used_consts.end()), used_consts.end());
+    std::vector<U> appended;
+    for (const U& u : used_consts)
+        if (!const_index.count(u)) {
+            const_index[u] = (int)(const_values.size() + n_pool_rows + appended.size());
+            appended.push_back(u);
+        }
     Alloc al0(lw.ln, order, const_index, fused, in->nreg, in->remat_mode, in->remat_k,
               in->keep_clean != 0);
     al0.run();
@@ -3023,6 +3292,7 @@
     std::unique_ptr<Alloc> al2;
     if (!in->solve && !in->leaf_pools && al0.n_lds - LDS_TIER >= SCHEDULE_MIN_SCRATCH) {
         order2 = fuse_roots(lw.ln, schedule_demand(lw.ln, sinks), fused2);
+        order2.insert(order2.end(), unread.begin(), unread.end());
         try {
             al2.reset(new Alloc(lw.ln, order2, const_index, fused2, in->nreg, in->remat_mode,
                                 in->remat_k, in->keep_clean != 0));
@@ -3048,10 +3318,8 @@
         res->code[4 * k + 3] = 0;
     }
     std::vector<std::pair<int, int>> pool_ranges;
-    std::vector<std::vector<U>> pools;
     size_t n_rows = const_values.size();
     if (in->leaf_pools) {
-        pools = leaf_pools(lw.ln, order, lw.leaves);
         for (size_t li = 0; li < pools.size(); li++) {
             if (!pools[li].empty()) {
                 pool_ranges.push_back({(int)n_rows, (int)pools[li].size()});
@@ -3061,6 +3329,7 @@
             }
         }
     }
+    n_rows += appended.size();
     res->n_rows = (int32_t)n_rows;
     res->n_const_values = (int32_t)const_values.size();
     res->table.resize(8 * n_rows);
@@ -3072,6 +3341,7 @@
     for (const U& u : const_values) put(u);
     for (const auto& pl : pools)
         for (const U& u : pl) put(u);
+    for (const U& u : appended) put(u);
 
     tp[7] = now_us();
     std::string& o = res->meta;
@@ -3170,6 +3440,8 @@
     o += "],\"lnodes\":" + std::to_string(ord.size());
     o += ",\"spills\":" + std::to_string(al.n_spill);
     o += ",\"reloads\":" + std::to_string(al.n_reload);
+    o += ",\"folded\":" + std::to_string(lw.folded);
+    o += ",\"appended\":" + std::to_string(appended.size());
     o += ",\"hist\":[";
     {
         bool first = true;
diff --git a/mythril_amd/csrc/mg_compile_py.cpp b/mythril_amd/csrc/mg_compile_py.cpp
--- a/mythril_amd/csrc/mg_compile_py.cpp
+++ b/mythril_amd/csrc/mg_compile_py.cpp
@@ -218,10 +218,11 @@
 PyObject* py_compile(PyObject*, PyObject* a) {
     PyObject *cons, *probes, *ops, *tables, *extra;
     int default_entries, nreg, leaf_pools, const_keys, solve, remat_mode, remat_k, keep_clean;
-    int search_hints, abi_presets;
-    if (!PyArg_ParseTuple(a, "OOO!OiiSiiiiiiii", &cons, &probes, &PyDict_Type, &ops, &tables,
+    int search_hints, abi_presets, no_simplify = 0;
+    if (!PyArg_ParseTuple(a, "OOO!OiiSiiiiiiii|i", &cons, &probes, &PyDict_Type, &ops, &tables,
                           &default_entries, &nreg, &extra, &leaf_pools, &const_keys, &solve,
-                          &remat_mode, &remat_k, &keep_clean, &search_hints, &abi_presets))
+                          &remat_mode, &remat_k, &keep_clean, &search_hints, &abi_presets,
+                          &no_simplify))
         return nullptr;
     PyObject* oth = PyDict_GetItemString(ops, "?");
     if (!oth) { PyErr_SetString(PyExc_KeyError, "ops has no '?'"); return nullptr; }
@@ -270,6 +271,7 @@
     in.leaf_pools = leaf_pools; in.const_keys = const_keys; in.solve = solve;
     in.remat_mode = remat_mode; in.remat_k = remat_k; in.keep_clean = keep_clean;
     in.search_hints = search_hints; in.abi_presets = abi_presets;
+    in.no_simplify = no_simplify;
     in.n_cval = (int32_t)f.cval.size(); in.n_string_bytes = (int32_t)f.strings.size();
     mgc_result* res = nullptr;
     int rc;
diff --git a/mythril_amd/ir.py b/mythril_amd/ir.py
--- a/mythril_amd/ir.py
+++ b/mythril_amd/ir.py
@@ -44,6 +44,23 @@
     source: str
     chunk: int = 0
     entry: int = 0
+
+
+class ConstValues(list):
+
+    __slots__ = ("rest",)
+
+    def __init__(self, pool=(), rest=()):
+        super().__init__(pool)
+        self.rest = tuple(rest)
+
+    def __getitem__(self, i):
+        if isinstance(i, int) and i >= len(self):
+            return self.rest[i - len(self)]
+        return super().__getitem__(i)
+
+    def __reduce__(self):
+        return (ConstValues, (list(self), self.rest))
 
 
 @dataclass
@@ -66,6 +83,7 @@
     presets: object = None
     group_key: object = None
     nreg: int = 16
+    appended: int = 0
 
     @property
     def solved(self) -> bool:
@@ -82,6 +100,90 @@
 
 def _limbs(value: int) -> List[int]:
     return [(value >> (32 * j)) & 0xFFFFFFFF for j in range(8)]
+
+
+SIMPLIFY = _os.environ.get("MYTHRIL_GPU_SIMPLIFY", "1") != "0"
+SIMPLIFY_MIN_HEAVY = 0.01
+_PRED_OPS = (I.EQ, I.ULT, I.ULE, I.SLT, I.SLE, I.UMULNO)
+_SIMPLIFY_OPS = frozenset((I.ADD, I.SUB, I.MUL, I.NEG, I.AND, I.OR, I.XOR, I.NOT, I.SHL, I.LSHR,
+                           I.ASHR, I.UDIV, I.UREM, I.SDIV, I.SREM, I.SMOD, I.ITE, I.CONCAT,
+                           I.EXTRACT, I.SEXT) + _PRED_OPS)
+SIMPLIFY_RULES = tuple(
+    ["const:" + I.OPNAME[op] for op in sorted(_SIMPLIFY_OPS - {I.ITE})] +
+    ["same:" + I.OPNAME[op] for op in (I.SUB, I.XOR, I.AND, I.OR, I.EQ, I.ULE, I.SLE, I.ULT, I.SLT,
+                                       I.UREM, I.SREM, I.SMOD, I.UDIV, I.SDIV)] +
+    ["ITE:const", "ITE:same", "ADD:0", "MUL:0", "MUL:1", "MUL:pow2", "MUL:pow2m1", "AND:0",
+     "AND:ones", "OR:0", "OR:ones", "XOR:0", "UMULNO:01", "UDIV:x,0", "ULT:x,0", "ULE:x,ones",
+     "ULE:0,x"] +
+    [I.OPNAME[op] + ":x,0" for op in (I.SUB, I.UREM, I.SREM, I.SHL, I.LSHR, I.ASHR)] +
+    [I.OPNAME[op] + ":x,1" for op in (I.UDIV, I.SDIV, I.UREM, I.SREM)] +
+    [I.OPNAME[op] + ":0,x" for op in (I.UDIV, I.SDIV, I.UREM, I.SREM, I.SHL, I.LSHR, I.ASHR)])
+
+
+def const_eval(op: int, w: int, v: Sequence[int], imm) -> int:
+    m = (1 << w) - 1
+    if op == I.CONCAT:
+        return ((v[0] << imm) | v[1]) & m
+    if op == I.EXTRACT:
+        return (v[0] >> imm) & m
+    if op == I.SEXT:
+        x = v[0] & ((1 << imm) - 1)
+        return (x - (1 << imm) if x >> (imm - 1) else x) & m
+    a = v[0] & m
+    if op == I.NEG:
+        return -a & m
+    if op == I.NOT:
+        return ~a & m
+    b = v[1] & m
+    if op == I.ADD:
+        return (a + b) & m
+    if op == I.SUB:
+        return (a - b) & m
+    if op == I.MUL:
+        return (a * b) & m
+    if op == I.AND:
+        return a & b
+    if op == I.OR:
+        return a | b
+    if op == I.XOR:
+        return a ^ b
+    if op == I.SHL:
+        return 0 if b >= w else (a << b) & m
+    if op == I.LSHR:
+        return 0 if b >= w else a >> b
+    if op == I.ASHR:
+        sa = a - (1 << w) if a >> (w - 1) else a
+        return (sa >> min(b, w - 1)) & m
+    if op == I.UDIV:
+        return m if b == 0 else a // b
+    if op == I.UREM:
+        return a if b == 0 else a % b
+    if op in (I.SDIV, I.SREM, I.SMOD):
+        na, nb = a >> (w - 1), b >> (w - 1)
+        ua, ub = (-a & m if na else a), (-b & m if nb else b)
+        if op == I.SDIV:
+            q = m if ub == 0 else ua // ub
+            return -q & m if na != nb else q
+        r = ua if ub == 0 else ua % ub
+        if op == I.SREM:
+            return -r & m if na else r
+        if r == 0 or not (na or nb):
+            return r
+        if na and nb:
+            return -r & m
+        return (b - r if na else r + b) & m
+    if op == I.EQ:
+        return int(a == b)
+    if op == I.ULT:
+        return int(a < b)
+    if op == I.ULE:
+        return int(a <= b)
+    if op in (I.SLT, I.SLE):
+        h = 1 << (w - 1)
+        return int((a ^ h) < (b ^ h)) if op == I.SLT else int((a ^ h) <= (b ^ h))
+    if op == I.UMULNO:
+        return int(a * b <= m)
+    raise AssertionError("const_eval: op %d" % op)
 
 
 class _Lowerer:
@@ -101,8 +203,129 @@
         self.solve = False
         self.solve_tables: set = set()
         self.arg_entries: Dict[str, List[Tuple[List[LNode], List[LNode]]]] = {}
+        self.simplify = False
+        self.folded = 0
+        self.fired: Dict[str, int] = {}
+
+    def _hit(self, tag: str, n: LNode) -> LNode:
+        self.fired[tag] = self.fired.get(tag, 0) + 1
+        return n
+
+    def _shl_form(self, x: LNode, k: int, w: int) -> LNode:
+        if k == 0:
+            return x
+        if k >= w:
+            return self.const(0, w)
+        return self.mk(I.CONCAT, w, (self.mk(I.EXTRACT, w - k, (x,), 0), self.const(0, k)), k)
+
+    def _div_guard(self, x: LNode, w: int, other: int) -> LNode:
+        e = self.mk(I.EQ, w, (x, self.const(0, w)))
+        ones = self.const((1 << w) - 1, w)
+        return self.mk(I.ITE, w, (e, ones, self.const(other, w)))
+
+    def _rule(self, op: int, w: int, args, imm) -> Optional[LNode]:
+        C = I.CONST
+        m = (1 << w) - 1
+        hit, const = self._hit, self.const
+        if op == I.ITE:
+            c, a, b = args
+            if c.op == C:
+                return hit("ITE:const", a if c.imm & 1 else b)
+            if a is b:
+                return hit("ITE:same", a)
+            return None
+        for x in args:
+            if x.op != C:
+                break
+        else:
+            v = const_eval(op, w, [x.imm for x in args], imm)
+            return hit("const:" + I.OPNAME[op], const(v, 1 if op in _PRED_OPS else w))
+        if len(args) != 2 or op in (I.CONCAT,):
+            return None
+        a, b = args
+        if a is b:
+            if op in (I.SUB, I.XOR):
+                return hit("same:" + I.OPNAME[op], const(0, w))
+            if op in (I.AND, I.OR) and a.width <= w:
+                return hit("same:" + I.OPNAME[op], a)
+            if op in (I.EQ, I.ULE, I.SLE):
+                return hit("same:" + I.OPNAME[op], const(1, 1))
+            if op in (I.ULT, I.SLT):
+                return hit("same:" + I.OPNAME[op], const(0, 1))
+            if op in (I.UREM, I.SREM, I.SMOD):
+                return hit("same:" + I.OPNAME[op], const(0, w))
+            if op in (I.UDIV, I.SDIV):
+                return hit("same:" + I.OPNAME[op], self._div_guard(a, w, 1))
+            return None
+        if op in (I.ADD, I.MUL, I.AND, I.OR, I.XOR, I.UMULNO):
+            if a.op == C:
+                x, c = b, a.imm & m
+            elif b.op == C:
+                x, c = a, b.imm & m
+            else:
+                return None
+            fits = x.width <= w
+            if op == I.ADD:
+                if c == 0 and fits:
+                    return hit("ADD:0", x)
+            elif op == I.MUL:
+                if c == 0:
+                    return hit("MUL:0", const(0, w))
+                if c == 1 and fits:
+                    return hit("MUL:1", x)
+                if c & (c - 1) == 0 and fits:
+                    return hit("MUL:pow2", self._shl_form(x, c.bit_length() - 1, w))
+                if c & (c + 1) == 0 and fits:
+                    return hit("MUL:pow2m1",
+                               self.mk(I.SUB, w, (self._shl_form(x, c.bit_length(), w), x)))
+            elif op == I.AND:
+                if c == 0:
+                    return hit("AND:0", const(0, w))
+                if c == m and fits:
+                    return hit("AND:ones", x)
+            elif op == I.OR:
+                if c == 0 and fits:
+                    return hit("OR:0", x)
+                if c == m:
+                    return hit("OR:ones", const(m, w))
+            elif op == I.XOR:
+                if c == 0 and fits:
+                    return hit("XOR:0", x)
+            elif c <= 1:
+                return hit("UMULNO:01", const(1, 1))
+            return None
+        if b.op == C:
+            c = b.imm & m
+            fits = a.width <= w
+            if c == 0:
+                if op in (I.SUB, I.UREM, I.SREM, I.SHL, I.LSHR, I.ASHR) and fits:
+                    return hit(I.OPNAME[op] + ":x,0", a)
+                if op == I.UDIV:
+                    return hit("UDIV:x,0", const(m, w))
+                if op == I.ULT:
+                    return hit("ULT:x,0", const(0, 1))
+            if c == 1:
+                if op in (I.UDIV, I.SDIV) and fits:
+                    return hit(I.OPNAME[op] + ":x,1", a)
+                if op in (I.UREM, I.SREM):
+                    return hit(I.OPNAME[op] + ":x,1", const(0, w))
+            if c == m and op == I.ULE:
+                return hit("ULE:x,ones", const(1, 1))
+        elif a.op == C and a.imm & m == 0:
+            if op in (I.UDIV, I.SDIV):
+                return hit(I.OPNAME[op] + ":0,x", self._div_guard(b, w, 0))
+            if op in (I.UREM, I.SREM, I.SHL, I.LSHR, I.ASHR):
+                return hit(I.OPNAME[op] + ":0,x", const(0, w))
+            if op == I.ULE:
+                return hit("ULE:0,x", const(1, 1))
+        return None
 
     def mk(self, op: int, width: int, args=(), imm=None) -> LNode:
+        if self.simplify and args and op in _SIMPLIFY_OPS:
+            n = self._rule(op, width, args, imm)
+            if n is not None:
+                self.folded += 1
+                return n
         if op == I.CONCAT and width == I.MAX_WIDTH and args[0].op == I.EXTRACT and \
                 args[0].imm == 0 and args[0].args[0].width == I.MAX_WIDTH:
             args = (args[0].args[0],) + tuple(args[1:])
@@ -922,6 +1145,32 @@
     return out
 
 
+def _reach(stack: List[LNode]) -> Tuple[set, int, int]:
+    seen, values, heavy = set(), set(), 0
+    while stack:
+        n = stack.pop()
+        if n.id in seen:
+            continue
+        seen.add(n.id)
+        if n.op == I.CONST:
+            values.add(n.imm & ((1 << 256) - 1))
+        heavy += n.op in _HEAVY
+        stack.extend(n.args)
+    return values, heavy, len(seen)
+
+
+def _plain_lowering(constraints, probes, table_sizes, default_entries, table_ckeys):
+    lw = _Lowerer(table_sizes or {}, default_entries)
+    lw.table_ckeys = table_ckeys
+    stack = [lw.lower(c)[0] for c in constraints]
+    for p in probes:
+        stack.extend(lw.lower(p))
+    if not stack:
+        stack.append(lw.const(1, 1))
+    values, heavy, reach = _reach(stack)
+    return values, lw.leaves, heavy, reach
+
+
 COMPILER = _os.environ.get("MYTHRIL_GPU_COMPILER", "native")
 
 
@@ -983,8 +1232,12 @@
                            default_entries: int = 2, nreg: int = I.NREG,
                            extra_consts: Sequence[int] = (), leaf_pools: bool = False,
                            const_keys: bool = False, solve: bool = False,
-                           search_hints: bool = False, abi_presets: bool = False) -> Program:
+                           search_hints: bool = False, abi_presets: bool = False,
+                           simplify: Optional[bool] = None) -> Program:
     constraints, probes = list(constraints), list(probes)
+    simplify = (SIMPLIFY if simplify is None else simplify) and not solve
+    given = (constraints, probes, table_sizes, default_entries, nreg, extra_consts, leaf_pools,
+             const_keys, solve, search_hints, abi_presets)
     if search_hints:
         extra_consts = list(extra_consts) + harvest_hints(constraints)
     plan = None
@@ -995,6 +1248,7 @@
             constraints, probes = plan.view(constraints), plan.view(probes)
     lw = _Lowerer(table_sizes or {}, default_entries)
     lw.solve = solve
+    lw.simplify = simplify
     if const_keys or solve:
         sym_counts: Dict[str, int] = {}
         ck = scan_const_keys(list(constraints) + list(probes), sym_counts=sym_counts,
@@ -1021,9 +1275,15 @@
         if solver.dead:
             births, probes = births[:1], ()
     sinks: List[LNode] = []
+    rooted = set()
     for r, b in zip(roots, births):
         lw.birth = b
-        sinks.append(lw.mk(I.ROOT, 1, (r,), None))
+        if simplify and r.id in rooted:
+            lw.nid += 1
+            sinks.append(LNode(I.ROOT, 1, (r,), None, lw.nid, max(b, r.birth)))
+        else:
+            sinks.append(lw.mk(I.ROOT, 1, (r,), None))
+        rooted.add(r.id)
     probe_chunks = 0
     for p in probes:
         if p.is_array():
@@ -1059,13 +1319,30 @@
             n.imm = n.width
             n.width = 1
     order, fused = _fuse_roots(_schedule(sinks))
-    const_values = sorted({n.imm & ((1 << 256) - 1) for n in order if n.op == I.CONST} |
-                          {v & ((1 << 256) - 1) for v in extra_consts})
+    unread: List[LNode] = []
+    if lw.folded:
+        have = {n.imm for n in order if n.op == I.LEAF}
+        unread = [lw.mk(I.LEAF, l.width, (), i) for i, l in enumerate(lw.leaves) if i not in have]
+        order = order + unread
+    M256 = (1 << 256) - 1
+    used_consts = {n.imm & M256 for n in order if n.op == I.CONST}
+    pool_consts = used_consts
+    if lw.folded:
+        pool_consts, plain_leaves, heavy, reach = _plain_lowering(
+            constraints, probes, table_sizes, default_entries, lw.table_ckeys)
+        if plain_leaves != lw.leaves or heavy < SIMPLIFY_MIN_HEAVY * reach:
+            return compile_constraints_py(*given, simplify=False)
+    const_values = sorted(pool_consts | {v & M256 for v in extra_consts})
     const_index = {v: i for i, v in enumerate(const_values)}
+    pools = _leaf_pools(order, lw.leaves) if leaf_pools else []
+    appended = sorted(used_consts - set(const_values))
+    first = len(const_values) + sum(len(p) for p in pools)
+    const_index.update({v: first + i for i, v in enumerate(appended)})
     ins, n_lds, n_spill, n_reload = _allocate(order, const_index, fused, nreg)
     if not solve and not leaf_pools and SCHEDULE_CHOICE and \
             n_lds - LDS_TIER >= SCHEDULE_MIN_SCRATCH:
         order2, fused2 = _fuse_roots(_schedule_demand(sinks))
+        order2 = order2 + unread
         try:
             alt = _allocate(order2, const_index, fused2, nreg)
         except Unsupported:
@@ -1082,19 +1359,21 @@
     table = list(const_values)
     pool_ranges: List[Tuple[int, int]] = []
     if leaf_pools:
-        for li, p in enumerate(_leaf_pools(order, lw.leaves)):
+        for li, p in enumerate(pools):
             if p:
                 pool_ranges.append((len(table), len(p)))
                 table.extend(p)
             else:
                 pool_ranges.append((0, len(const_values)))
+    table.extend(appended)
     consts = np.frombuffer(b"".join(v.to_bytes(32, "little") for v in table),
                            dtype="<u4").reshape(-1, 8).astype(np.uint32)
+    const_values = ConstValues(const_values, table[len(const_values):])
     hist: Dict[str, int] = {}
     for n in order:
         hist[I.OPNAME[n.op]] = hist.get(I.OPNAME[n.op], 0) + 1
     stats = {"lnodes": len(order), "n_ins": len(ins), "spills": n_spill, "reloads": n_reload,
-             "hist": hist}
+             "hist": hist, "folded": lw.folded}
     ckeys = {k: v for k, v in lw.table_ckeys.items() if k in lw.table_kinds}
     tsizes = dict(lw.table_sizes)
     for name in lw.solve_tables & set(lw.table_kinds):
@@ -1103,6 +1382,7 @@
                    len(constraints), tsizes, lw.table_kinds, ckeys, stats, pool_ranges,
                    derived, entry_keys, n_user_probes)
     prog.nreg = nreg
+    prog.appended = len(appended)
     if plan is not None:
         prog.presets = plan
     return prog
diff --git a/mythril_amd/roofline.py b/mythril_amd/roofline.py
--- a/mythril_amd/roofline.py
+++ b/mythril_amd/roofline.py
@@ -105,9 +105,79 @@
     return arr.params[0], inner
 
 
+def _lowered(order, roots, ts, simplify):
+    from . import ir
+    lw = ir._Lowerer(ts, 2)
+    lw.simplify = simplify
+    for r in roots:
+        lw.lower(r)
+    return lw
+
+
+def simplified_weights(order, roots, ts: Dict[str, int]) -> Dict[int, float]:
+    from . import ir
+    from . import irdefs as I
+    if not ir.SIMPLIFY:
+        return {}
+    try:
+        on, off = _lowered(order, roots, ts, True), _lowered(order, roots, ts, False)
+    except ir.Unsupported:
+        return {}
+    if not on.folded:
+        return {}
+    _, heavy, reach = ir._reach([off.memo[r.id][0] for r in roots])
+    if heavy < ir.SIMPLIFY_MIN_HEAVY * reach:
+        return {}
+
+    def kind(lw, n):
+        ch = lw.memo.get(n.id)
+        if ch is None or len(ch) != 1:
+            return None
+        x = ch[0]
+        if x.op == I.CONST:
+            return "gone"
+        for a in n.args:
+            ca = lw.memo.get(a.id)
+            if ca is not None and len(ca) == 1 and ca[0] is x:
+                return "gone"
+        return x.op
+
+    out: Dict[int, float] = {}
+    for n in order:
+        if n.op in _LEAF or n.op in ("select", "apply", "store") or n.width > 256:
+            continue
+        k_on, k_off = kind(on, n), kind(off, n)
+        if k_on is None or k_off is None or k_off == "gone":
+            continue
+        w = n.args[0].width if n.args and n.args[0].is_bv() else n.width
+        if k_on == "gone":
+            out[n.id] = 0.0
+        elif n.op in ("bvudiv", "bvsdiv") and k_on == I.ITE and k_off in (I.UDIV, I.SDIV):
+            out[n.id] = 16.0 * _scale(w)
+        elif n.op == "bvmul":
+            acc, total = on.memo[n.args[0].id][0], 0.0
+            for a in n.args[1:]:
+                b = on.memo[a.id][0]
+                new = on.mk(I.MUL, n.width, (acc, b))
+                if new.op == I.MUL:
+                    total += 192.0 * _scale(w)
+                elif new is acc or new is b or new.op == I.CONST:
+                    pass
+                elif new.op == I.CONCAT:
+                    total += 8.0 * _scale(w)
+                else:
+                    total += 16.0 * _scale(w)
+                acc = new
+            if total < node_weight(n, ts):
+                out[n.id] = total
+    return out
+
+
 def dag_work(roots: Iterable[Node], table_sizes: Dict[str, int] = None) -> Tuple[int, float]:
     ts = table_sizes or {}
-    order = topo_order(list(roots))
+    roots = list(roots)
+    order = topo_order(roots)
+    cheaper = simplified_weights(order, roots, dict(ts))
     users: Dict[int, list] = {}
     for n in order:
         for a in n.args:
@@ -133,5 +203,5 @@
         if n.id in words:
             weight += words[n.id]
         elif n.id not in absorbed:
-            weight += node_weight(n, ts)
+            weight += cheaper[n.id] if n.id in cheaper else node_weight(n, ts)
     return nodes, weight
```

After: 2137 billion (median of 6 runs). +15.9%, better.
